# muhanzhang/IGMC

Measured on AMD Instinct MI355X. Metric: enclosing-subgraphs/sec (train step, batch=50) + test RMSE, higher is better.
Workload: dtype f32; 1 GPU; ml_1m, hop 1, max-nodes-per-hop 100, batch 50 per GPU, adj-dropout 0, dynamic-train, ARR 0.001, Adam; parallelism=dp1, global_batch=50, graphs_captured_before_timing=True, steps_per_graph_launch=100, group_steps=50

## Files before the change

igmc_amd/csrc/capi.hip:

```cpp
#include "launch.h"
#include "sortpool.h"
#include "g2_image.h"

#include <algorithm>
#include <climits>
#include <cmath>
#include <cstdio>
#include <cstring>
#include <map>
#include <string>
#include <vector>

static thread_local std::string g_err;
int g_igmc_prof_on = 0;

#define IGMC_FAIL(msg)                                                      \
  do {                                                                      \
    g_err = std::string(__func__) + ": " + (msg);                           \
    return 1;                                                               \
  } while (0)
#define HIPCHECK(expr)                                                      \
  do {                                                                      \
    hipError_t e_ = (expr);                                                 \
    if (e_ != hipSuccess) {                                                 \
// ... 706 lines not shown
      if (!told) fprintf(stderr, "[igmc] batches of more than 1024 subgraphs: no plane-exchange regions -- the dense-layer / per-layer kernels take the steps, not the subgraph kernel\n");
      told = true;
    }
  } else if (wide) {
    fail |= M.get(&d.g2_w, g2_w_words(d.R, d.L));
  }
  fail |= M.get(&d.gs_bar, 2 * Bc + 1);
  fail |= M.get(&d.gs_ts, 4);
  d.gs_err = d.gs_bar ? d.gs_bar + 2 * Bc : nullptr;
  fail |= M.get(&d.wg_part, (size_t)4 * IGMC_WG_BLOCKS * igmc_wg_stride()) |
          M.get(&d.gatt_part, (size_t)3 * IGMC_GATHER_BLOCKS * d.R * 4) |
          M.get(&d.l0_part, (size_t)IGMC_L0_BLOCKS * rows0 * 32) |
          M.get(&d.graw, (size_t)3 * igmc_wg_stride() + 3 * d.R * 4 + rows0 * 32) | M.get(&d.arr_part, 4);
  d.side = nullptr;
  d.ctrl = nullptr;
  d.dcat[0] = d.dcat[1] = d.dcat[2] = nullptr;
  fail |= M.get(&m->done_ctr, 8);
  if (fail) {
    M.release();
    delete m;
    IGMC_FAIL("hipMalloc failed (model workspace)");
  }
  {
    hipStream_t st1, st2;
    if (hipStreamCreateWithFlags(&st1, hipStreamNonBlocking) != hipSuccess ||
        hipStreamCreateWithFlags(&st2, hipStreamNonBlocking) != hipSuccess) {
      M.release();
      delete m;
      IGMC_FAIL("hipStreamCreate failed");
    }
    m->ax.s1 = st1;
    m->ax.s2 = st2;
    for (int i = 0; i < 8; ++i) {
      hipEvent_t e;
      if (hipEventCreateWithFlags(&e, hipEventDisableTiming) != hipSuccess) IGMC_FAIL("hipEventCreate failed");
      m->ax.ev[i] = e;
    }
  }
  HIPCHECK(hipMemset(m->done_ctr, 0, 8 * sizeof(int)));
  HIPCHECK(hipMemset(m->d.gs_bar, 0, (2 * (size_t)max_graphs + 1) * sizeof(int)));
  {
    const unsigned long long ts0[4] = {~0ull, 0ull, 0ull, 0ull};
    HIPCHECK(hipMemcpy(m->d.gs_ts, ts0, sizeof(ts0), hipMemcpyHostToDevice));
  }
  if (m->d.fold_w) HIPCHECK(hipMemset(m->d.fold_w, 0, (size_t)4 * 32 * IGMC_FOLD_NA * sizeof(unsigned long long)));
  if (m->d.g2_ex) {
    HIPCHECK(hipMemset(m->d.g2_ex, 0, 5 * m->d.g2_ex_stride * sizeof(unsigned long long)));
    HIPCHECK(hipMemset(m->d.g2_fx, 0, (size_t)max_graphs * 256 * sizeof(unsigned long long)));
    if (m->d.g2_px) HIPCHECK(hipMemset(m->d.g2_px, 0, 5 * m->d.g2_px_stride));
  }
  if (igmc_model_prepare(d)) {
    M.release();
    delete m;
    IGMC_FAIL("hipFuncSetAttribute failed");
  }
  *out = m;
  return 0;
}

extern "C" int igmc_debug_lin_mask(const igmc_model* m, uint8_t* h_out, int64_t n) {
  if (!m || !h_out) IGMC_FAIL("null argument");
  if (n < 0 || n > (int64_t)m->d.graph_cap * 128) IGMC_FAIL("mask size out of range");
  HIPCHECK(hipDeviceSynchronize());
  HIPCHECK(hipMemcpy(h_out, m->d.lmask, (size_t)n, hipMemcpyDeviceToHost));
  return 0;
}

extern "C" int igmc_debug_head_array(const igmc_model* m, int which, float* h_out, int64_t n) {
  if (!m || !h_out) IGMC_FAIL("null argument");
  if (which < 0 || which > 3) IGMC_FAIL("no such array");
  const float* src = which == 0 ? m->d.a1 : which == 1 ? m->d.dz : which == 2 ? m->d.feat : m->d.gfeat;
  if (n < 0 || n > (int64_t)m->d.graph_cap * (which < 2 ? 128 : m->d.D)) IGMC_FAIL("size out of range");
  HIPCHECK(hipDeviceSynchronize());
  HIPCHECK(hipMemcpy(h_out, src, (size_t)n * sizeof(float), hipMemcpyDeviceToHost));
  return 0;
}

extern "C" int igmc_debug_weight_images(const igmc_model* m, float* h_out, int64_t* n_words) {
  if (!m || !n_words) IGMC_FAIL("null argument");
  const int64_t n = m->d.g2_w ? (int64_t)g2_w_words(m->d.R, m->d.L) : 0;
  if (h_out) {
    if (*n_words < 0 || *n_words > n) IGMC_FAIL("size out of range");
    HIPCHECK(hipDeviceSynchronize());
    if (*n_words) HIPCHECK(hipMemcpy(h_out, m->d.g2_w, (size_t)*n_words * sizeof(float), hipMemcpyDeviceToHost));
  } else {
    *n_words = n;
  }
  return 0;
}

extern "C" void igmc_model_destroy(igmc_model* m) {
  if (!m) return;
  for (int i = 0; i < 8; ++i) hipEventDestroy((hipEvent_t)m->ax.ev[i]);
  hipStreamDestroy((hipStream_t)m->ax.s1);
  hipStreamDestroy((hipStream_t)m->ax.s2);
  m->mem.release();
  delete m;
}

extern "C" int64_t igmc_param_count(const igmc_model* m) { return m ? m->d.n_params : 0; }

extern "C" int64_t igmc_param_offset(const igmc_model* m, int layer, int which, int64_t* count) {
  if (!m) return -1;
  const ModelDev& d = m->d;
  const int fin = (layer == 0) ? d.L : 32;
  int64_t off = -1, n = 0;
  switch (which) {
    case IGMC_P_BASIS: off = d.off_basis[layer & 3]; n = (int64_t)4 * fin * 32; break;
    case IGMC_P_ROOT: off = d.off_root[layer & 3]; n = (int64_t)fin * 32; break;
    case IGMC_P_BIAS: off = d.off_bias[layer & 3]; n = 32; break;
    case IGMC_P_ATT: off = d.off_att[layer & 3]; n = (int64_t)d.R * 4; break;
    case IGMC_P_LIN1_W: off = d.off_l1w; n = (int64_t)128 * d.D; break;
    case IGMC_P_LIN1_B: off = d.off_l1b; n = 128; break;
    case IGMC_P_LIN2_W: off = d.off_l2w; n = 128; break;
    case IGMC_P_LIN2_B: off = d.off_l2b; n = 1; break;
  }
  if (count) *count = n;
  return off;
}

static StepPlan plan_query(const igmc_model* m, const igmc_batch* b, int B) {
  StepPlan sp;
  igmc_step_plan(m->d, b->d, B, IGMC_CALL_STEP, &sp);
  return sp;
}

extern "C" int igmc_model_dense_layers(const igmc_model* m, const igmc_batch* b, int B) {
  return (m && b) ? plan_query(m, b, B).dense_layers : 0;
}

extern "C" int igmc_model_dense_path(const igmc_model* m, const igmc_batch* b, int B) {
  return (m && b) ? plan_query(m, b, B).family == IGMC_FAM_G2 : 0;
}

extern "C" int igmc_model_step_form(const igmc_model* m, const igmc_batch* b, int B) {
  return (m && b) ? plan_query(m, b, B).step_form : 0;
}

extern "C" int igmc_model_step_geometry(const igmc_model* m, const igmc_batch* b, int B, int32_t* out, int n) {
  if (!m || !b || !out || n < 0) IGMC_FAIL("bad arguments");
  if (B < 1 || B > b->d.graph_cap) IGMC_FAIL("batch size outside the arena's capacity");
  const StepPlan sp = plan_query(m, b, B);
  const int g2 = sp.family == IGMC_FAM_G2, dense = sp.family == IGMC_FAM_DLF || sp.family == IGMC_FAM_DL;
  const int32_t v[IGMC_GEOM_N] = {sp.step_form,
                                  sp.family,
                                  g2 ? sp.cs : 0,
                                  g2 ? sp.grid : 0,
                                  sp.nqu,
                                  sp.nqv,
                                  sp.family == IGMC_FAM_ROWS ? 0 : sp.wide ? g2_groups(m->d.R, m->d.L) : 1,
                                  sp.wide && sp.gsplit,
                                  g2 || sp.dlts,
                                  g2 ? sp.lay.kp : 0,
                                  dense && sp.dlb};
  for (int i = 0; i < n && i < IGMC_GEOM_N; ++i) out[i] = v[i];
  return 0;
}

static int check_fit(igmc_model* m, const igmc_batch* b, std::string* why) {
  if (!m || !b) { *why = "null model or batch"; return 1; }
  if (b->last_B <= 0) { *why = "batch is empty (run igmc_extract_batch first)"; return 1; }
  if (b->d.node_cap > m->d.node_cap || b->d.graph_cap > m->d.graph_cap) { *why = "batch capacity exceeds the model workspace"; return 1; }
  if (b->d.num_labels != m->d.L) { *why = "num_labels mismatch (hop)"; return 1; }
  if (b->g->max_rel >= m->d.R) { *why = "graph has more relations than the model"; return 1; }
  if (m->d.S != b->n_side && m->d.S > 0) { *why = "side feature width mismatch"; return 1; }
  return 0;
}

static int check_call(igmc_model* m, const igmc_batch* b, bool buffers, std::string* why) {
  if (check_fit(m, b, why)) return 1;
  if (!buffers) { *why = "null buffer"; return 1; }
  return 0;
}
static StepPlan begin_call(igmc_model* m, const igmc_batch* b, int kind, void* stream) {
  m->d.side = b->side;
  StepPlan sp;
  igmc_step_plan(m->d, b->d, b->last_B, kind, &sp);
  if (b->lean && sp.needs_csr) ensure_csr(b, stream);
  return sp;
}
static void end_call(igmc_model* m, const igmc_batch* b, int training, int use_edge_flags) {
  m->last_B = b->last_B;
  m->last_training = training;
  m->last_flags = use_edge_flags;
}

struct AdamScalars {
  float step_size, inv_sqrt_bc2;
};
static AdamScalars adam_scalars(const int64_t* d_ctrl, int64_t t, float lr, float beta1, float beta2) {
  AdamScalars a = {0.f, 0.f};
  if (!d_ctrl) {
    const double bc1 = 1.0 - std::pow((double)beta1, (double)t);
    const double bc2 = 1.0 - std::pow((double)beta2, (double)t);
    a.step_size = (float)((double)lr / bc1);
    a.inv_sqrt_bc2 = (float)(1.0 / std::sqrt(bc2));
  }
  return a;
}

extern "C" int igmc_model_forward(igmc_model* m, const float* d_params, const igmc_batch* b, int training,
                                  int use_edge_flags, const uint8_t* d_lin_mask, uint64_t seed, uint64_t step,
                                  float multiply_by, float* d_out, void* stream) {
  std::string why;
  if (check_call(m, b, d_params && d_out, &why)) IGMC_FAIL(why);
  const StepPlan sp = begin_call(m, b, training ? IGMC_CALL_CONV : IGMC_CALL_EVAL, stream);
  ImgScope img(m, d_params);
  igmc_launch_forward(m->d, b->d, sp, d_params, b->last_B, training, use_edge_flags, d_lin_mask, seed, step, multiply_by,
                      d_out, stream);
  img.done_unchanged();
  HIPCHECK(hipGetLastError());
  end_call(m, b, training, use_edge_flags);
  return 0;
}

extern "C" int igmc_model_backward(igmc_model* m, const float* d_params, const igmc_batch* b, const float* d_gout,
                                   float multiply_by, float* d_grad, void* stream) {
  std::string why;
  if (check_fit(m, b, &why)) IGMC_FAIL(why);
  if (!m->last_training || m->last_B != b->last_B) IGMC_FAIL("backward needs a preceding training-mode forward on this batch");
  if (!d_params || !d_gout || !d_grad) IGMC_FAIL("null buffer");
  StepPlan sp;
  igmc_step_plan(m->d, b->d, b->last_B, IGMC_CALL_CONV, &sp);
  igmc_launch_backward(m->d, b->d, sp, d_params, b->last_B, m->last_flags, d_gout, 0, 0.f, multiply_by, 2.f, 0.f, d_grad,
                       stream);
  HIPCHECK(hipGetLastError());
  return 0;
}

extern "C" int igmc_model_loss_grad(igmc_model* m, const float* d_params, const igmc_batch* b, int use_edge_flags,
                                    const uint8_t* d_lin_mask, uint64_t seed, uint64_t step, float multiply_by,
                                    float ARR, float grad_scale, float arr_scale, float* d_out, float* d_grad,
                                    float* d_loss, void* stream) {
  std::string why;
  if (check_call(m, b, d_params && d_out && d_grad, &why)) IGMC_FAIL(why);
  const StepPlan sp = begin_call(m, b, IGMC_CALL_STEP, stream);
  ImgScope img(m, d_params);
  igmc_launch_loss_grad(m->d, b->d, sp, (float*)d_params, b->last_B, use_edge_flags, d_lin_mask, seed, step,
                        multiply_by, ARR, grad_scale, arr_scale, d_out, d_grad, d_loss, nullptr, stream);
  img.done_unchanged();
  HIPCHECK(hipGetLastError());
  end_call(m, b, 1, use_edge_flags);
  return 0;
}

extern "C" int igmc_adam_step(float* d_params, const float* d_grad, float* d_exp_avg, float* d_exp_avg_sq, int64_t n,
                              int64_t step, float lr, float beta1, float beta2, float eps, float weight_decay,
                              void* stream) {
  if (!d_params || !d_grad || !d_exp_avg || !d_exp_avg_sq || n <= 0 || step < 1) IGMC_FAIL("bad arguments");
  const AdamScalars as = adam_scalars(nullptr, step, lr, beta1, beta2);
  igmc_launch_adam(d_params, d_grad, d_exp_avg, d_exp_avg_sq, n, as.step_size, as.inv_sqrt_bc2, beta1, beta2, eps, weight_decay,
                   nullptr, 0, stream);
  HIPCHECK(hipGetLastError());
  return 0;
}

extern "C" int igmc_sse_accumulate(const float* d_out, const igmc_batch* b, double* d_acc, void* stream) {
  if (!d_out || !b || !d_acc) IGMC_FAIL("null argument");
  igmc_launch_sse(b->d, d_out, d_acc, nullptr, stream);
  HIPCHECK(hipGetLastError());
  return 0;
}
extern "C" int igmc_sse_accumulate_tick(const float* d_out, const igmc_batch* b, double* d_acc, int64_t* d_ctrl, void* stream) {
  if (!d_out || !b || !d_acc || !d_ctrl) IGMC_FAIL("null argument");
  igmc_launch_sse(b->d, d_out, d_acc, d_ctrl, stream);
  HIPCHECK(hipGetLastError());
  return 0;
}

extern "C" int igmc_scores_store(const float* d_out, const igmc_batch* b, double* d_acc, float* d_scores, float* d_labels,
                                 int64_t n, int64_t first_or_minus1, int64_t* d_ctrl, int32_t* d_err, void* stream) {
  if (!d_out || !b || !d_acc || !d_scores || !d_labels || !d_err) IGMC_FAIL("null argument");
  if (n < 1 || n > (int64_t)INT32_MAX) IGMC_FAIL("n must be in [1, 2^31)");
  if (first_or_minus1 < -1 || first_or_minus1 >= n) IGMC_FAIL("first must be -1 (the arena's stamp) or a position below n");
  igmc_launch_scores_store(b->d, d_out, d_acc, d_ctrl, d_scores, d_labels, n, first_or_minus1, d_err, stream);
  HIPCHECK(hipGetLastError());
  return 0;
}
static int select_grid(int64_t n, int num, int grid) {
  if (n < 1 || n > (int64_t)INT32_MAX || num < 1 || num > IGMC_SELECT_MAX_NUM || grid < 0 || grid > IGMC_SELECT_MAX_GRID) return -1;
  return grid > 0 ? grid : igmc_select_default_grid(n);
}
extern "C" int64_t igmc_select_scratch_bytes(int64_t n, int num, int grid) {
  const int g = select_grid(n, num, grid);
  if (g < 0) {
    g_err = std::string(__func__) + ": n must be in [1, 2^31), num in [1, 64], grid in [0, 1024]";
    return -1;
  }
  return (int64_t)2 * g * num * (int64_t)sizeof(uint64_t);
}
extern "C" int igmc_select_extremes(const float* d_keys, int64_t n, int num, int32_t* d_idx_low, int32_t* d_idx_high,
                                    float* d_key_low, float* d_key_high, int32_t* d_count, void* d_scratch,
                                    int64_t scratch_bytes, int grid, void* stream) {
  if (!d_keys || !d_idx_low || !d_idx_high || !d_scratch) IGMC_FAIL("null argument");
  const int g = select_grid(n, num, grid);
  if (g < 0) IGMC_FAIL("n must be in [1, 2^31), num in [1, 64], grid in [0, 1024]");
  if (scratch_bytes < (int64_t)2 * g * num * (int64_t)sizeof(uint64_t)) IGMC_FAIL("scratch too small (igmc_select_scratch_bytes)");
  if (((uintptr_t)d_scratch & 7) != 0) IGMC_FAIL("scratch must be 8-byte aligned");
  igmc_launch_select(d_keys, n, num, g, d_scratch, d_idx_low, d_idx_high, d_key_low, d_key_high, d_count, stream);
  HIPCHECK(hipGetLastError());
  return 0;
}

extern "C" int igmc_candidates_count(const igmc_graph* g, const int32_t* d_users, int nq, const uint8_t* d_item_ok,
                                     int exclude_seen, int64_t* d_counts, int32_t* d_err, void* stream) {
  if (!g || !d_users || !d_counts || !d_err) IGMC_FAIL("null argument");
  if (nq < 1) IGMC_FAIL("nq must be at least 1");
// ... 739 lines not shown
```

igmc_amd/csrc/g2_compose.h:

```cpp
#pragma once

__global__ __launch_bounds__(G2C_THREADS) void k_g2_compose(ModelDev m, const float* P, float* w) {
  __shared__ float s_att[4 * G2_NR * G2_NG_MAX];
  const int tid = threadIdx.x, R = m.R, L = m.L, RL = R * L, LF = L * 32;
  const int ng = g2_groups(R, L);
  const int tableb = 2 * 3 * ng * (G2_NR + 1);
  const int mi = (int)(blockIdx.x >> 1);
  const int l = ((int)blockIdx.x >= tableb) ? 0 : 1 + mi / (ng * (G2_NR + 1)), trans = blockIdx.x & 1;
  if ((int)blockIdx.x >= tableb) {
    const int c0 = 32 * ((int)blockIdx.x - tableb);
    const float attv = (tid < R * 4) ? P[m.off_att[0] + tid] : 0.f;
    float bv[4][4], rv[4];
#pragma unroll
    for (int q = 0; q < 4; ++q) {
      const int i = tid + q * G2C_THREADS, c = c0 + (i >> 5), f = i & 31;
      const int cf = (c < RL) ? (c % L) * 32 + f : 0;
#pragma unroll
      for (int bb = 0; bb < 4; ++bb) bv[q][bb] = (c < RL) ? P[m.off_basis[0] + bb * LF + cf] : 0.f;
      rv[q] = (c >= RL && c < RL + L) ? P[m.off_root[0] + (c - RL) * 32 + f] : ((c == RL + L) ? P[m.off_bias[0] + f] : 0.f);
    }
    if (tid < 4 * G2_NR * G2_NG_MAX) s_att[tid] = attv;
    __syncthreads();
#pragma unroll
    for (int q = 0; q < 4; ++q) {
// ... 1 lines not shown
      float sacc = rv[q];
      if (c < RL) {
        const int r = c / L;
        sacc = g2_wsum(s_att[r * 4], s_att[r * 4 + 1], s_att[r * 4 + 2], s_att[r * 4 + 3], bv[q][0], bv[q][1], bv[q][2], bv[q][3]);
      }
      w[g2_t0_off(ng) + (size_t)c0 * 32 + i] = sacc;
    }
    return;
  }
  const int grp = (mi / (G2_NR + 1)) % ng, blk = mi % (G2_NR + 1);
  uint16_t* img = (uint16_t*)(w + g2_img_off(ng, l, trans, grp));
  const int r = (blk == G2_NR) ? ((grp == 0) ? -1 : R) : G2_NR * grp + blk;
  const int n = tid & 31, kg = tid >> 5;
  float v[4] = {0.f, 0.f, 0.f, 0.f};
  if (r < 0) {
    const float* root = P + m.off_root[l];
    if (trans) {
      const float4 r4 = *(const float4*)(root + n * 32 + 4 * kg);
      v[0] = r4.x; v[1] = r4.y; v[2] = r4.z; v[3] = r4.w;
    } else {
#pragma unroll
      for (int q = 0; q < 4; ++q) v[q] = root[(4 * kg + q) * 32 + n];
    }
  } else if (r < R) {
    const float* basis = P + m.off_basis[l];
    float bq[4][4];
#pragma unroll
    for (int bb = 0; bb < 4; ++bb) {
      if (trans) {
        const float4 b4 = *(const float4*)(basis + bb * 1024 + n * 32 + 4 * kg);
        bq[bb][0] = b4.x; bq[bb][1] = b4.y; bq[bb][2] = b4.z; bq[bb][3] = b4.w;
      } else {
#pragma unroll
        for (int q = 0; q < 4; ++q) bq[bb][q] = basis[bb * 1024 + (4 * kg + q) * 32 + n];
      }
    }
    float at[4];
#pragma unroll
    for (int bb = 0; bb < 4; ++bb) at[bb] = P[m.off_att[l] + r * 4 + bb];
#pragma unroll
    for (int q = 0; q < 4; ++q) v[q] = g2_wsum(at[0], at[1], at[2], at[3], bq[0][q], bq[1][q], bq[2][q], bq[3][q]);
  }
  uint32_t h01, m01, l01, h23, m23, l23;
  g2_split2(v[0], v[1], h01, m01, l01);
  g2_split2(v[2], v[3], h23, m23, l23);
  const int lane = (kg & 3) * 16 + (n & 15), nt = n >> 4, e0 = 4 * (kg >> 2);
  const uint32_t t3[3][2] = {{h01, h23}, {m01, m23}, {l01, l23}};
#pragma unroll
  for (int t = 0; t < G2_NT; ++t)
    *(uint2*)(img + ((size_t)(((t * (G2_NR + 1) + blk) * 2 + nt) * 64 + lane)) * 8 + e0) = make_uint2(t3[t][0], t3[t][1]);
}

static int igmc_g2_layout(const ModelDev& m, const BatchDev& b, int cs, G2Layout* lay) {
  const int RL = m.R * m.L;
  if (m.S != 0 || m.D != 256 || m.R > G2_NR || m.L > 8 || RL + m.L + 1 > 32 || !m.ts_part || !m.g2_px || !m.g2_fx || !m.g2_w || !b.relm) return 0;
  const int half = 2 * cs;
  const int cmax = b.cap_u > b.cap_v ? b.cap_u : b.cap_v;
  if (cmax > 16 * half || cmax > 128) return 0;
  if (b.graph_cap > m.g2_graphs) return 0;
  const int kmax = ((cmax + 31) >> 5) << 5;
  lay->kp = kmax + 8;
  lay->nsides = (cs == 1) ? 2 : 1;
  lay->rmr = ((cmax + 15) >> 4) << 4;
  lay->rmc = kmax;
  int o = 0;
  lay->pside = ((G2_NT * 32 * lay->kp * 2 + 1023) & ~1023) >> 2;
  lay->planes = o; o += lay->nsides * lay->pside;
  lay->ohp = o; o += lay->nsides * (8 * lay->kp >> 1);
  lay->lab = o; o += 64;
  lay->xo = o; o += 2 * G2_NB * 16 * G2_XP;
  lay->hs = o; o += G2_NB * 16 * G2_XP;
  int tw = G2_NB * 16 * G2_TP;
  if (tw < (G2_THREADS / 64) * 256) tw = (G2_THREADS / 64) * 256;
  const int rw = 2 * lay->rmr * (lay->rmc + 8) / 4;
  if (rw > tw) tw = rw;
  if (tw < 1024) tw = 1024;
  lay->tile = o; o += tw;
  lay->hist = o; o += G2_NB * 16 * G2_XP;
  lay->px = o; o += G2_NB * 2 * 64 * 4;
  lay->wreg = o; o += G2_WIMG;
  lay->t0 = o; o += 1024;
  lay->att = o; o += 64;
  lay->head = o; o += 256 + 256 + 3 * 128 + 512 + 16;
  lay->words = o;
  return (size_t)o * 4 + 768 <= 160 * 1024;
}

__global__ void k_g2_xcc_probe(int* out) {
  if (threadIdx.x == 0) out[blockIdx.x] = (int)(g2_xcc_id() & 15ull);
}
int igmc_g2_xcd_ok() {
#ifdef IGMC_HIPEMU
  return 1;
#else
  static int oks[64];
  static bool init = false;
  if (!init) {
    for (int i = 0; i < 64; ++i) oks[i] = -1;
    init = true;
  }
  int dev = 0;
  if (hipGetDevice(&dev) != hipSuccess || dev < 0 || dev >= 64) dev = 0;
  int& ok = oks[dev];
  if (ok >= 0) return ok;
  ok = 0;
  int* d = nullptr;
  int h[64];
  if (hipMalloc((void**)&d, sizeof(h)) != hipSuccess) return ok;
  hipLaunchKernelGGL(k_g2_xcc_probe, dim3(64), dim3(64), 0, 0, d);
  if (hipMemcpy(h, d, sizeof(h), hipMemcpyDeviceToHost) == hipSuccess) {
    ok = 1;
    for (int b = 0; b + 8 < 64; ++b)
      if (h[b] != h[b + 8]) ok = 0;
  }
  (void)hipFree(d);
  if (!ok) fprintf(stderr, "[igmc] device %d: workgroups b and b + 8 of a launch do not share an XCD: the subgraph kernel and the one-launch dense layers are not used\n", dev);
  return ok;
#endif
}

int g_igmc_compose_count = 0;

int igmc_launch_graph_step2(const ModelDev& m, const BatchDev& b, const StepPlan& sp, const float* P, int B, int training,
                            int use_flags, const uint8_t* inj_mask, uint64_t seed, uint64_t step, float mult, float grad_scale,
                            float* out, void* stream, int nstash, const int64_t* stash_ctrl) {
  const G2Layout& lay = sp.lay;
  const int cs = sp.cs;
  G2Args a;
  memset(&a, 0, sizeof(a));
  a.n_users = b.n_users; a.n_items = b.n_items; a.B = B; a.s_lab = b.s_lab; a.relm = b.relm; a.y = b.y;
  a.cap_u = b.cap_u; a.cap_v = b.cap_v; a.slot = b.slot; a.relm_ld = b.relm_ld; a.graph_cap = b.graph_cap;
  a.R = m.R; a.L = m.L; a.D = m.D; a.ts_stride = m.ts_stride;
  for (int l = 0; l < 4; ++l) {
    a.h[l] = m.h[l];
    a.off_bias[l] = (int)m.off_bias[l];
  }
  a.ts_part = m.ts_part; a.g2_px = m.g2_px; a.g2_fx = m.g2_fx; a.g2_px_stride = m.g2_px_stride; a.g2_w = m.g2_w;
  a.gs_bar = m.gs_bar; a.gs_err = m.gs_err; a.a1 = m.a1; a.dz = m.dz; a.feat = m.feat; a.gfeat = m.gfeat; a.err = m.err;
  a.lmask = m.lmask; a.ctrl = m.ctrl;
  a.off_l1w = (int)m.off_l1w; a.off_l1b = (int)m.off_l1b; a.off_l2w = (int)m.off_l2w; a.off_l2b = (int)m.off_l2b;
  a.P = P;
  a.inj_mask = inj_mask;
  a.seed = seed;
  a.step = step;
  a.mult = mult;
  a.grad_scale = grad_scale;
  a.out = out;
  a.lay2 = lay;
  a.timing = getenv("IGMC_GS_TIMING") ? 1 : 0;
  a.ts = (g_igmc_prof_on == 2) ? m.gs_ts : nullptr;
  a.self_seq = (!training || a.ts) ? 1 : 0;
  a.cs = cs;
  a.stride = (cs > 1) ? ((B + 7) & ~7) : 1;
  if (training && nstash) {
    a.nstash = nstash;
    a.stash_ctrl = stash_ctrl;
    a.fs.R = m.R; a.fs.L = m.L;
    for (int l = 0; l < 4; ++l) {
      a.fs.off_basis[l] = m.off_basis[l];
      a.fs.off_att[l] = m.off_att[l];
    }
    a.fs.fin_stash = m.fin_stash; a.fs.adam_m1 = m.adam_m1; a.fs.adam_m2 = m.adam_m2; a.fs.arr_part = m.arr_part;
  }
  const int grid = sp.grid + a.nstash;
  const size_t sm = (size_t)lay.words * 4;
  if (!m.img_current) {
    IGMC_PLAUNCH("k_g2_compose", k_g2_compose, 2 * 3 * g2_groups(m.R, m.L) * (G2_NR + 1) + g2_t0_rows(m.R, m.L) / 32, G2C_THREADS, 0, stream, m, P, m.g2_w);
    ++g_igmc_compose_count;
  }
#ifdef IGMC_HIPEMU
  if (cs > 1) {
    hipemu::rt().co_cs = cs;
    hipemu::rt().co_stride = 8;
    hipemu::rt().co_block = 8 * cs;
  }
#endif
  if (getenv("IGMC_GS_TRACE")) fprintf(stderr, "[igmc] k_graph_step B=%d train=%d flags=%d v2 kp=%d lds=%zu cluster=%d grid=%d\n", B, training, use_flags, lay.kp, sm, cs, grid);
  igmc_dispatch([&](auto uf, auto tr, auto cl) {
    IGMC_PLAUNCH(tr() ? "k_graph_step" : "k_graph_fwd", (k_graph_step2<uf(), tr(), cl()>), grid, G2_THREADS, sm, stream, a);
  }, use_flags != 0, training != 0, cs > 1);
  return a.self_seq ? 0 : 1;
}

int igmc_dl_prepare();
int igmc_gs_prepare() { return igmc_g2_prepare(); }
int igmc_g2_prepare() {
  if (igmc_dl_prepare()) return 1;
  (void)igmc_g2_xcd_ok();
#ifndef IGMC_HIPEMU
  const int mx = 160 * 1024;
  const void* fns[8] = {(const void*)k_graph_step2<true, true, true>,   (const void*)k_graph_step2<false, true, true>,
                        (const void*)k_graph_step2<true, false, true>,  (const void*)k_graph_step2<false, false, true>,
                        (const void*)k_graph_step2<true, true, false>,  (const void*)k_graph_step2<false, true, false>,
                        (const void*)k_graph_step2<true, false, false>, (const void*)k_graph_step2<false, false, false>};
  for (const void* fn : fns) {
    hipFuncAttributes fa;
    if (hipFuncGetAttributes(&fa, fn) != hipSuccess || (int)fa.sharedSizeBytes > 768) return 1;
    if (hipFuncSetAttribute(fn, hipFuncAttributeMaxDynamicSharedMemorySize, mx - (int)fa.sharedSizeBytes) != hipSuccess) return 1;
  }
#endif
  return 0;
}
```

igmc_amd/csrc/g2_prims.h:

```cpp
#pragma once

#ifdef IGMC_HIPEMU
#define G2_STAMP(k) do { } while (0)
#else
#define G2_STAMP(k)                                                                                        \
  do {                                                                                                     \
    if (a.timing && threadIdx.x == 0) {                                                                    \
      if (blockIdx.x == 0) g_g2_clk[k] = __builtin_readcyclecounter();                                     \
      else if (a.cs > 2 && (int)blockIdx.x == 8 * (a.cs / 2) && (k) < 40) g_g2_clk[64 + (k)] = __builtin_readcyclecounter(); \
    }                                                                                                      \
  } while (0)
#endif

#ifdef IGMC_HIPEMU
#define DL_STAMP(k) do { } while (0)
#else
#define DL_STAMP(k)                                                                               \
  do {                                                                                            \
    if (a.timing && threadIdx.x == 0 && (int)blockIdx.x == a.timing - 1 && (k) < 128)             \
      g_g2_clk[k] = __builtin_readcyclecounter();                                                 \
  } while (0)
#endif

#ifdef IGMC_HIPEMU
#define G2_OPAQUE(x) do { } while (0)
#else
#define G2_OPAQUE(x) asm volatile("" : "+v"(x))
#endif

typedef uint32_t u32x4 __attribute__((ext_vector_type(4)));
#ifndef IGMC_HIPEMU
typedef __bf16 g2_bf16x8 __attribute__((ext_vector_type(8)));
#endif

__device__ __forceinline__ f32x4 g2_mfma_bf16(u32x4 a, u32x4 b, f32x4 c) {
#ifdef IGMC_HIPEMU
  return igmc_emu_mfma_16x16x32_bf16(a, b, c);
#else
  return __builtin_amdgcn_mfma_f32_16x16x32_bf16(__builtin_bit_cast(g2_bf16x8, a), __builtin_bit_cast(g2_bf16x8, b), c, 0, 0, 0);
#endif
}

template <bool FLAGS>
__device__ __forceinline__ void g2_expand4(uint32_t w, uint32_t r1, int keepbit, uint32_t& o01, uint32_t& o23) {
  uint32_t mk = w & (0x01010101u * IGMC_RELM_CODE);
  if (FLAGS) mk &= ((w >> keepbit) & 0x01010101u) * IGMC_RELM_CODE;
  const uint32_t t = mk ^ (0x01010101u * r1);
  const uint32_t eq = ~(t + 0x7F7F7F7Fu) & 0x80808080u;
  const uint32_t mask = (eq >> 7) * 0xFFu;
#ifdef IGMC_HIPEMU
  o01 = ((mask & 0xFFu) ? 0x3F80u : 0u) | ((mask & 0xFF00u) ? 0x3F800000u : 0u);
  o23 = ((mask & 0xFF0000u) ? 0x3F80u : 0u) | ((mask & 0xFF000000u) ? 0x3F800000u : 0u);
#else
  o01 = __builtin_amdgcn_perm(mask, mask, 0x01010000u) & 0x3F803F80u;
  o23 = __builtin_amdgcn_perm(mask, mask, 0x03030202u) & 0x3F803F80u;
#endif
}

template <bool FLAGS>
__device__ __forceinline__ uint32_t g2_bytemask(uint32_t w, uint32_t r1, int keepbit) {
  uint32_t mk = w & (0x01010101u * IGMC_RELM_CODE);
  if (FLAGS) mk &= ((w >> keepbit) & 0x01010101u) * IGMC_RELM_CODE;
  const uint32_t t = mk ^ (0x01010101u * r1);
  const uint32_t eq = ~(t + 0x7F7F7F7Fu) & 0x80808080u;
  return (eq >> 7) * 0xFFu;
}
__device__ __forceinline__ u32x4 g2_mask_frag(uint32_t m0, uint32_t m1) {
  u32x4 f;
#ifdef IGMC_HIPEMU
  f[0] = ((m0 & 0xFFu) ? 0x3F80u : 0u) | ((m0 & 0xFF00u) ? 0x3F800000u : 0u);
  f[1] = ((m0 & 0xFF0000u) ? 0x3F80u : 0u) | ((m0 & 0xFF000000u) ? 0x3F800000u : 0u);
  f[2] = ((m1 & 0xFFu) ? 0x3F80u : 0u) | ((m1 & 0xFF00u) ? 0x3F800000u : 0u);
  f[3] = ((m1 & 0xFF0000u) ? 0x3F80u : 0u) | ((m1 & 0xFF000000u) ? 0x3F800000u : 0u);
#else
  f[0] = __builtin_amdgcn_perm(m0, m0, 0x01010000u) & 0x3F803F80u;
  f[1] = __builtin_amdgcn_perm(m0, m0, 0x03030202u) & 0x3F803F80u;
  f[2] = __builtin_amdgcn_perm(m1, m1, 0x01010000u) & 0x3F803F80u;
  f[3] = __builtin_amdgcn_perm(m1, m1, 0x03030202u) & 0x3F803F80u;
#endif
  return f;
}

__device__ __forceinline__ float g2_tanh(float x) {
#ifdef IGMC_HIPEMU
  return tanhf(x);
#else
  return 1.f - 2.f * __builtin_amdgcn_rcpf(1.f + __expf(2.f * x));
#endif
}

template <int AUX = 0>
__device__ __forceinline__ void g2_glds16(const float4* src_wave, float4* lds_wave, int lane) {
#ifndef IGMC_HIPEMU
  __builtin_amdgcn_global_load_lds((const __attribute__((address_space(1))) void*)(src_wave + lane),
                                   (__attribute__((address_space(3))) void*)lds_wave, 16, 0, AUX);
#else
  lds_wave[lane] = src_wave[lane];
#endif
}

#include "g2_words.h"

#define G2_PX_BYTES 32768
#define G2_PX_FLAGS 28672
#define DLX_PX_BYTES 65536
#define DLX_PX_FLAGS 61440
__device__ __forceinline__ void g2_publish_planes(unsigned char* px, int kp, int f, int node0, const float (&v)[4]) {
  uint32_t h0, m0, l0, h1, m1, l1;
  g2_split2(v[0], v[1], h0, m0, l0);
  g2_split2(v[2], v[3], h1, m1, l1);
  unsigned char* p = px + ((size_t)f * kp + node0) * 2;
  const size_t ts = (size_t)32 * kp * 2;
  *(uint2*)p = make_uint2(h0, h1);
  *(uint2*)(p + ts) = make_uint2(m0, m1);
  *(uint2*)(p + 2 * ts) = make_uint2(l0, l1);
}
__device__ __forceinline__ void g2_flag_raise(unsigned char* px, int slot, uint32_t tag, int lane, int flags_off = G2_PX_FLAGS) {
#ifndef IGMC_HIPEMU
  asm volatile("s_waitcnt vmcnt(0)" ::: "memory");
  if (lane == 0) __hip_atomic_store((unsigned long long*)(px + flags_off) + slot, (unsigned long long)tag, __ATOMIC_RELAXED, __HIP_MEMORY_SCOPE_WAVEFRONT);
#else
  if (lane == 0) ((unsigned long long*)(px + flags_off))[slot] = (unsigned long long)tag;
#endif
}
__device__ __forceinline__ void g2_flags_wait(const unsigned char* px, int n, uint32_t tag, int lane, int* err, int flags_off = G2_PX_FLAGS) {
  const unsigned long long* fl = (const unsigned long long*)(px + flags_off);
  for (long it = 0;; ++it) {
#ifndef IGMC_HIPEMU
    const unsigned long long w = (lane < n) ? __hip_atomic_load(fl + lane, __ATOMIC_RELAXED, __HIP_MEMORY_SCOPE_AGENT) : (unsigned long long)tag;
#else
    const unsigned long long w = (lane < n) ? fl[lane] : (unsigned long long)tag;
#endif
    if (__ballot(w != (unsigned long long)tag) == 0ull) break;
    if (it > (1L << 20)) {
      *err = 1;
      break;
    }
#ifndef IGMC_HIPEMU
    __builtin_amdgcn_s_sleep(1);
#else
    hipemu::yield();
#endif
  }
}
__device__ __forceinline__ void g2_planes_load_exact(uint32_t* pl, const unsigned char* px, int bytes, int wave, int lane, int nwaves) {
  const int pieces = (bytes + 1023) >> 10;
  for (int c = wave; c < pieces; c += nwaves)
    if (c * 1024 + lane * 16 < bytes) g2_glds16<16>((const float4*)px + c * 64, (float4*)pl + c * 64, lane);
}
__device__ __forceinline__ void g2_planes_load(uint32_t* pl, const unsigned char* px, int kp, int wave, int lane, int nwaves) {
  const int pieces = (192 * kp + 1023) >> 10;
  for (int c = wave; c < pieces; c += nwaves) g2_glds16<16>((const float4*)px + c * 64, (float4*)pl + c * 64, lane);
}

#ifdef IGMC_HIPEMU
#define G2_SCHED_BARRIER() do { } while (0)
#else
#define G2_SCHED_BARRIER() __builtin_amdgcn_sched_barrier(0)
#endif

__device__ __forceinline__ uint32_t g2_ld_seq(const int* gs_bar) {
#ifndef IGMC_HIPEMU
  return (uint32_t)__hip_atomic_load(gs_bar + 1, __ATOMIC_RELAXED, __HIP_MEMORY_SCOPE_AGENT);
#else
  return (uint32_t)gs_bar[1];
#endif
}
__device__ __forceinline__ bool g2_last_workgroup_advances(int* gs_bar) {
#ifndef IGMC_HIPEMU
  if (__hip_atomic_fetch_add(gs_bar, 1, __ATOMIC_RELAXED, __HIP_MEMORY_SCOPE_AGENT) != (int)gridDim.x - 1) return false;
  __hip_atomic_store(gs_bar, 0, __ATOMIC_RELAXED, __HIP_MEMORY_SCOPE_AGENT);
  __hip_atomic_fetch_add(gs_bar + 1, 1, __ATOMIC_RELAXED, __HIP_MEMORY_SCOPE_AGENT);
  return true;
#else
  if (gs_bar[0]++ != (int)gridDim.x - 1) return false;
  gs_bar[0] = 0;
  gs_bar[1] += 1;
  return true;
#endif
}
__device__ __forceinline__ void g2_wait_vm0() {
#ifndef IGMC_HIPEMU
  asm volatile("s_waitcnt vmcnt(0)" ::: "memory");
#endif
}
__device__ __forceinline__ unsigned long long g2_wall_clock() {
#ifndef IGMC_HIPEMU
  return (unsigned long long)wall_clock64();
#else
  return 0ull;
#endif
}
__device__ __forceinline__ unsigned long long g2_xcc_id() {
#ifndef IGMC_HIPEMU
  return (unsigned long long)__builtin_amdgcn_s_getreg((20 << 0) | (0 << 6) | (3 << 11));
#else
  return 0ull;
#endif
}
__device__ __forceinline__ void g2_clock_open(unsigned long long* ts) {
#ifndef IGMC_HIPEMU
  atomicMin(ts, (unsigned long long)wall_clock64());
#else
  (void)ts;
#endif
}
__device__ __forceinline__ void g2_clock_close(unsigned long long* ts, unsigned long long t1) {
#ifndef IGMC_HIPEMU
  const unsigned long long t0 = __hip_atomic_load(ts, __ATOMIC_RELAXED, __HIP_MEMORY_SCOPE_AGENT);
  atomicAdd(ts + 1, t1 - t0);
  atomicAdd(ts + 2, 1ull);
  __hip_atomic_store(ts, ~0ull, __ATOMIC_RELAXED, __HIP_MEMORY_SCOPE_AGENT);
#else
  (void)ts; (void)t1;
#endif
}

#ifdef IGMC_HIPEMU
#define DL_FMAC(acc_, a_, b_) ((acc_) += (a_) * (b_))
#else
#define DL_FMAC(acc_, a_, b_) asm("v_fmac_f32 %0, %1, %2" : "+v"(acc_) : "v"(a_), "v"(b_))
#endif

#define DLX_K 256
__device__ __forceinline__ void dlx_seq_done(int* gs_bar, int self_seq) {
  if (threadIdx.x != 0 || !self_seq) return;
  (void)g2_last_workgroup_advances(gs_bar);
}
```

igmc_amd/csrc/g2_subgraph.h:

```cpp
#pragma once

struct G2Args {
  const int32_t* n_users;
  const int32_t* n_items;
  int B;
  const uint8_t* s_lab;
  const uint8_t* relm;
  const float* y;
  int cap_u, cap_v, slot, relm_ld, graph_cap;
  int R, L, D, ts_stride;
  float* h[4];
  float* ts_part;
  unsigned char* g2_px;
  unsigned long long* g2_fx;
  size_t g2_px_stride;
  const float* g2_w;
  int* gs_bar;
  int* gs_err;
  float* a1;
  float* dz;
  float* feat;
  float* gfeat;
  float* err;
  uint8_t* lmask;
  const int64_t* ctrl;
  int off_bias[4];
  int off_l1w, off_l1b, off_l2w, off_l2b;
  const float* P;
  const uint8_t* inj_mask;
  uint64_t seed, step;
  float mult, grad_scale;
  float* out;
  unsigned long long* ts;
  int timing, cs, stride, self_seq;
  G2Layout lay2;
  int nstash;
  const int64_t* stash_ctrl;
  FinStashModel fs;
};

template <bool FLAGS, bool TRAIN, bool ONCE>
__global__ __launch_bounds__(G2_THREADS) void k_graph_step2(G2Args a) {
  __builtin_amdgcn_s_setprio(3);
  const float* P = a.P;
  IGMC_DYN_SMEM(smem);
  float* S = (float*)smem;
  const G2Layout lay = a.lay2;
  const int kp = lay.kp, nsides = lay.nsides;
  uint32_t* PLN = (uint32_t*)(S + lay.planes);
  uint32_t* OHP = (uint32_t*)(S + lay.ohp);
  unsigned char* slab = (unsigned char*)(S + lay.lab);
  float* XOA = S + lay.xo;
  float* HSS = S + lay.hs;
  float* TILES = S + lay.tile;
  float* HIST = S + lay.hist;
  float* PXA = S + lay.px;
  float2* sW2 = (float2*)(S + lay.wreg);
  float* sT0 = S + lay.t0;
  float* sfeat = S + lay.head;
  float* sgf = sfeat + 256;
  float* sa1 = sgf + 256;
  float* skeep = sa1 + 128;
  float* sdz = skeep + 128;
  float* sred = sdz + 128;
  float* misc = sred + 512;
  const int R = a.R, L = a.L, RL = R * L;
  const int tid = threadIdx.x, lane = tid & 63, wave = tid >> 6;
  const int li = lane & 15, kq = lane >> 4;
  const int B = a.B;
  const int ts = a.ts_stride;
  const int cs = a.cs;
  const int cm = (cs > 1) ? (int)((blockIdx.x >> 3) % cs) : 0;
  const int half = 2 * cs;
  const uint32_t seq = g2_ld_seq(a.gs_bar);
  const uint32_t tag0 = seq * 8u + 1u;
  const uint64_t step = a.ctrl ? (uint64_t)a.ctrl[IGMC_CTRL_STEP] : a.step;
  if (a.ts && tid == 0) g2_clock_open(a.ts);
  auto xtag = [&](int x) { return tag0 + (uint32_t)x; };
  G2_STAMP(0);
  if (a.timing && tid == 0 && blockIdx.x < 1024) {
    g_g2_wg[blockIdx.x][0] = g2_wall_clock();
    g_g2_wg[blockIdx.x][2] = g2_xcc_id();
  }
  auto arrive = [&]() {
    if (tid == 0 && a.self_seq) {
      const unsigned long long t1 = a.ts ? g2_wall_clock() : 0ull;
      if (g2_last_workgroup_advances(a.gs_bar) && a.ts) g2_clock_close(a.ts, t1);
    }
  };
  const int nwork = (int)gridDim.x - (TRAIN ? a.nstash : 0);
  if (TRAIN && (int)blockIdx.x >= nwork) {
    if (tid < IGMC_BLOCK) {
      const int l = (int)blockIdx.x - nwork;
      fin_stash_body(a.fs, P, l, a.stash_ctrl);
      if (l == 0 && tid == 0) a.fs.fin_stash[IGMC_STASH_SCAL + IGMC_STASH_SEQ] = __uint_as_float(seq);
    }
    arrive();
    return;
  }

  const int g_first = (cs > 1) ? (int)(blockIdx.x / (8 * cs)) * 8 + (int)(blockIdx.x & 7) : (int)blockIdx.x;
  const int g_pre = (g_first < a.graph_cap) ? g_first : a.graph_cap - 1;
  const int pre_cu = a.n_users[g_pre], pre_cv = a.n_items[g_pre];
  const int ld = a.relm_ld;
  auto load_label = [&](int g2) {
    const int hi = (tid >> 7) & 1, t7 = tid & 127;
    const int capx = a.cap_u + hi * (a.cap_v - a.cap_u);
    return (int)a.s_lab[(size_t)g2 * a.slot + hi * a.cap_u + ((t7 < capx) ? t7 : 0)];
  };
  int labv_raw = 0;
  if (tid < 256) g2_glds16((const float4*)(a.g2_w + 6 * G2_WIMG) + (tid & ~63), (float4*)sT0 + (tid & ~63), tid & 63);
  const int tslot = (cs > 1) ? g_first + cm * a.stride : (int)blockIdx.x;
  f32x4 acc0 = (f32x4){0.f, 0.f, 0.f, 0.f};
  bool first_graph = true;
  G2_STAMP(1);

  int g = g_first;
  if (g < B) do {
    int tid_g = threadIdx.x;
    G2_OPAQUE(tid_g);
    const int tid = tid_g, lane = tid & 63, wave = tid >> 6;
    const int li = lane & 15, kq = lane >> 4;
    const int bw = wave >> 1, hf = wave & 1;
    const int gw = cm * G2_NB + bw;
    const int side = gw / half, bi = gw - side * half;
    labv_raw = load_label(g);
    uint32_t bw0[G2_KS], bw1[G2_KS];
    {
      const unsigned char* rmg = a.relm + (size_t)g * a.cap_u * ld;
      const uint32_t rrow = (uint32_t)(16 * bi + li);
#pragma unroll
      for (int s = 0; s < G2_KS; ++s) {
        const uint32_t c0 = (uint32_t)(32 * s + 8 * kq);
        if (side == 0) {
          const uint32_t* p4 = (const uint32_t*)(rmg + (rrow * (uint32_t)ld + c0));
          bw0[s] = p4[0];
          bw1[s] = p4[1];
        } else {
          const unsigned char* pc = rmg + (c0 * (uint32_t)ld + rrow);
          bw0[s] = (uint32_t)pc[0] | ((uint32_t)pc[ld] << 8) | ((uint32_t)pc[2 * ld] << 16) | ((uint32_t)pc[3 * ld] << 24);
          bw1[s] = (uint32_t)pc[4 * ld] | ((uint32_t)pc[5 * ld] << 8) | ((uint32_t)pc[6 * ld] << 16) | ((uint32_t)pc[7 * ld] << 24);
        }
      }
    }
    G2_STAMP(48);
    {
      const float4 z4 = make_float4(0.f, 0.f, 0.f, 0.f);
      for (int i = tid; i < 2 * G2_NB * 16 * G2_XP / 4; i += G2_THREADS) ((float4*)XOA)[i] = z4;
      for (int i = tid; i < G2_NB * 16 * G2_XP / 4; i += G2_THREADS) ((float4*)HIST)[i] = z4;
    }
    G2_STAMP(49);
    const int cu = first_graph ? pre_cu : a.n_users[g], cv = first_graph ? pre_cv : a.n_items[g];
    const int n_own = side ? cv : cu, n_opp = side ? cu : cv;
    const int nbs = g * a.slot + (side ? a.cap_u : 0);
    const int nbun = (n_own + 15) >> 4;
    const bool active = bi < nbun;
    const int row0 = 16 * bi;
    const int nks = (n_opp + 31) >> 5;
    const int sx = (nsides == 2) ? side : 0, so = (nsides == 2) ? 1 - side : 0;
    uint32_t* pl = PLN + so * lay.pside;
    uint32_t* ohp = OHP + so * (8 * kp >> 1);
    float* XO0 = XOA + bw * 16 * G2_XP;
    float* XO1 = XOA + (G2_NB + bw) * 16 * G2_XP;
    float* HS = HSS + bw * 16 * G2_XP;
    float* T = TILES + bw * 16 * G2_TP;
    float* HI = HIST + bw * 16 * G2_XP;
    f32x4* PXo = (f32x4*)PXA + (bw * 2 + hf) * 64 + lane;
    const f32x4* PXi = (const f32x4*)PXA + (bw * 2 + (1 - hf)) * 64 + lane;
    const size_t exs = a.g2_px_stride;
    auto px_of = [&](int x, int sd) { return a.g2_px + (size_t)x * exs + ((size_t)g * 2 + sd) * G2_PX_BYTES; };
    unsigned long long* fx = a.g2_fx + (size_t)g * 256;
    const int nbun_opp = (n_opp + 15) >> 4;

    if (tid < 256) slab[tid] = (unsigned char)(((tid & 127) < ((tid >> 7) ? cv : cu)) ? labv_raw : 255);
    G2_STAMP(50);
    __syncthreads();
    G2_STAMP(2);
    {
      for (int i = tid; i < nsides * 8 * (kp >> 1); i += G2_THREADS) {
        const int s2 = i / (8 * (kp >> 1)), rem = i - s2 * (8 * (kp >> 1));
        const int lb = rem / (kp >> 1), q = rem - lb * (kp >> 1);
        const int sd = (nsides == 2) ? s2 : 1 - side;
        const int l0 = (2 * q < 128) ? slab[sd * 128 + 2 * q] : 255, l1 = (2 * q + 1 < 128) ? slab[sd * 128 + 2 * q + 1] : 255;
        OHP[i] = ((l0 == lb) ? 0x3F80u : 0u) | ((l1 == lb) ? 0x3F800000u : 0u);
      }
    }
    __syncthreads();
    G2_STAMP(3);
    uint32_t AM[G2_NR][G2_KS][2];
    uint32_t RB[FLAGS ? G2_KS : 1][2];
    const int kb = side ? IGMC_RELM_KF : IGMC_RELM_KT;
    {
      const int kf = side ? IGMC_RELM_KT : IGMC_RELM_KF;
#pragma unroll
      for (int s = 0; s < G2_KS; ++s) {
        uint32_t w0 = 0u, w1 = 0u;
        if (active && s < nks && row0 + li < n_own) {
          w0 = bw0[s];
          w1 = bw1[s];
          {
            const int keep = n_opp - (32 * s + 8 * kq);
            if (keep < 8) {
              w1 = (keep <= 4) ? 0u : (w1 & (0xFFFFFFFFu >> (8 * (8 - keep))));
              if (keep < 4) w0 = (keep <= 0) ? 0u : (w0 & (0xFFFFFFFFu >> (8 * (4 - keep))));
            }
          }
        }
        if constexpr (FLAGS) {
          RB[s][0] = w0;
          RB[s][1] = w1;
        }
#pragma unroll
        for (int r = 0; r < G2_NR; ++r) {
          AM[r][s][0] = g2_bytemask<FLAGS>(w0, (uint32_t)(r + 1), kf);
          AM[r][s][1] = g2_bytemask<FLAGS>(w1, (uint32_t)(r + 1), kf);
        }
      }
    }
    auto frag_f = [&](int r, int s) {
      uint32_t m0 = AM[r][s][0], m1 = AM[r][s][1];
      G2_OPAQUE(m0);
      G2_OPAQUE(m1);
      return g2_mask_frag(m0, m1);
    };
    auto frag_b = [&](int r, int s) {
      uint32_t m0 = FLAGS ? RB[FLAGS ? s : 0][0] : AM[r][s][0], m1 = FLAGS ? RB[FLAGS ? s : 0][1] : AM[r][s][1];
      G2_OPAQUE(m0);
      G2_OPAQUE(m1);
      if constexpr (FLAGS) return g2_mask_frag(g2_bytemask<true>(m0, (uint32_t)(r + 1), kb), g2_bytemask<true>(m1, (uint32_t)(r + 1), kb));
      else return g2_mask_frag(m0, m1);
    };
    G2_STAMP(4);

    static_assert(G2_WIMG % 256 == 0, "an image is a whole number of 1 KB pieces");
    auto wload = [&](int l, int trans) {
      const float4* src = (const float4*)(a.g2_w + (size_t)((l - 1) * 2 + trans) * G2_WIMG);
#pragma unroll
      for (int j = 0; j < (G2_WIMG / 256 + G2_THREADS / 64 - 1) / (G2_THREADS / 64); ++j) {
        const int c = wave + j * (G2_THREADS / 64);
        if (c < G2_WIMG / 256) g2_glds16(src + c * 64, (float4*)sW2 + c * 64, lane);
      }
    };
    wload(1, 0);
    auto fwd_out = [&](int l, const f32x4& o, float bias, float* XO) {
      const int nt = hf;
      float* hrow = a.h[l] + (size_t)(nbs + row0 + 4 * kq) * 32 + li;
      float* xo = XO + 4 * kq * G2_XP + li;
      float v[4];
#pragma unroll
      for (int rr = 0; rr < 4; ++rr) {
        const float tv = g2_tanh(o[rr] + bias);
        v[rr] = (row0 + 4 * kq + rr < n_own) ? tv : 0.f;
      }
      if (l < 3) {
        g2_publish_planes(px_of(l, side), kp, 16 * nt + li, row0 + 4 * kq, v);
        g2_flag_raise(px_of(l, side), 2 * bi + hf, xtag(l), lane);
      }
#pragma unroll
      for (int rr = 0; rr < 4; ++rr) {
        xo[rr * G2_XP + 16 * nt] = v[rr];
        if (TRAIN && row0 + 4 * kq + rr < n_own) hrow[rr * 32 + 16 * nt] = v[rr];
      }
      if (bi == 0 && kq == 0) g2_pub_f32(fx + side * 128 + l * 32 + 16 * nt + li, v[0], tag0 + G2_FXTAG);
    };
    auto raise = [&](int x) { g2_flag_raise(px_of(x, side), 2 * bi + hf, xtag(x), lane); };
    auto fetch = [&](int x) {
      if (nsides == 1) {
        g2_flags_wait(px_of(x, 1 - side), 2 * nbun_opp, xtag(x), lane, a.gs_err);
        g2_planes_load(PLN, px_of(x, 1 - side), kp, wave, lane, G2_THREADS / 64);
      } else {
        for (int s2 = 0; s2 < 2; ++s2) {
          g2_flags_wait(px_of(x, s2), 2 * (((s2 ? cv : cu) + 15) >> 4), xtag(x), lane, a.gs_err);
          g2_planes_load(PLN + s2 * lay.pside, px_of(x, s2), kp, wave, lane, G2_THREADS / 64);
        }
      }
    };

    if (active) {
      f32x4 hacc[G2_NR];
#pragma unroll
      for (int r = 0; r < G2_NR; ++r) hacc[r] = (f32x4){0.f, 0.f, 0.f, 0.f};
      u32x4 pfh[G2_KS];
#pragma unroll
      for (int s = 0; s < G2_KS; ++s) {
        pfh[s] = *(const u32x4*)(ohp + ((li & 7) * kp >> 1) + 16 * s + 4 * kq);
        if (li >= 8 || s >= nks) pfh[s] = (u32x4){0u, 0u, 0u, 0u};
      }
      G2_SCHED_BARRIER();
#pragma unroll
      for (int s = 0; s < G2_KS; ++s) {
#pragma unroll
        for (int r = 0; r < G2_NR; ++r) {
          hacc[r] = g2_mfma_bf16(pfh[s], frag_f(r, s), hacc[r]);
        }
      }
      G2_STAMP(51);
#pragma unroll
      for (int r = 0; r < G2_NR; ++r)
#pragma unroll
        for (int rr = 0; rr < 4; ++rr)
          if (r < R && 4 * kq + rr < L) HI[li * G2_XP + r * L + 4 * kq + rr] = hacc[r][rr];
      if (kq == 0 && row0 + li < n_own) {
        HI[li * G2_XP + RL + slab[side * 128 + row0 + li]] = 1.f;
        HI[li * G2_XP + RL + L] = 1.f;
      }
      IGMC_WAVE_SYNC();
      f32x4 o = (f32x4){0.f, 0.f, 0.f, 0.f};
#pragma unroll
      for (int j = 0; j < 8; ++j) {
        const float av = HI[li * G2_XP + 4 * j + kq];
        o = __builtin_amdgcn_mfma_f32_16x16x4f32(av, sT0[(4 * j + kq) * 32 + 16 * hf + li], o, 0, 0, 0);
      }
      G2_STAMP(52);
      fwd_out(0, o, 0.f, XO0);
    }
    G2_STAMP(5);

#pragma unroll
    for (int l = 1; l < 4; ++l) {
      float* XOc = (l & 1) ? XO0 : XO1;
      float* XOn = (l & 1) ? XO1 : XO0;
      G2_STAMP(6 + 3 * (l - 1));
      const float bias0 = P[a.off_bias[l] + 16 * hf + li];
      fetch(l - 1);
      if (l > 1) wload(l, 0);
// ... 133 lines not shown
      wload(3, 1);
      __syncthreads();
      if (tid < 256) {
        const float v = ((TILES[tid] + TILES[256 + tid]) + (TILES[512 + tid] + TILES[768 + tid])) +
                        ((TILES[1024 + tid] + TILES[1280 + tid]) + (TILES[1536 + tid] + TILES[1792 + tid]));
        sgf[tid] = v;
        if (cm == 0) a.gfeat[(size_t)g * a.D + tid] = v;
      }
      __syncthreads();
      G2_STAMP(17);
      if (tid < 32 * nsides) {
        const int s2 = tid >> 5, f = tid & 31;
        const int sd = (nsides == 2) ? s2 : 1 - side;
        const float hv = sfeat[sd * 128 + 96 + f];
        const float d = sgf[sd * 128 + 96 + f] * (1.f - hv * hv);
        uint32_t h, mi, lo;
        g2_split2(d, 0.f, h, mi, lo);
        uint32_t* p2 = PLN + s2 * lay.pside + (f * kp >> 1);
        p2[0] = h & 0xFFFFu;
        p2[32 * kp >> 1] = mi & 0xFFFFu;
        p2[2 * (32 * kp >> 1)] = lo & 0xFFFFu;
      }
      if (hf == 0 && lane < 32) {
        const float hv = sfeat[side * 128 + 96 + lane];
        const float d = (active && bi == 0) ? sgf[side * 128 + 96 + lane] * (1.f - hv * hv) : 0.f;
        if (active && bi == 0) XO0[lane] = d;
        sred[(1 * G2_NB + bw) * 32 + lane] = d;
      }
      __syncthreads();
      G2_STAMP(18);

#pragma unroll
      for (int l = 3; l >= 1; --l) {
        float* XOc = (l & 1) ? XO0 : XO1;
        float* XOn = (l & 1) ? XO1 : XO0;
        float* wpart = a.ts_part + ((size_t)l * IGMC_TS_BLOCKS + tslot) * ts;
        G2_STAMP(19 + 5 * (3 - l));
        float hreg[4];
#pragma unroll
        for (int rr = 0; rr < 4; ++rr) hreg[rr] = 0.f;
        f32x4 o[2];
        if (active) {
          {
            const float* hrow = a.h[l - 1] + (size_t)(nbs + row0 + 4 * kq) * 32 + 16 * hf + li;
#pragma unroll
            for (int rr = 0; rr < 4; ++rr)
              if (row0 + 4 * kq + rr < n_own) hreg[rr] = hrow[rr * 32];
          }
          int lane_ = lane;
          G2_OPAQUE(lane_);
          const int li_ = lane_ & 15, kq_ = lane_ >> 4;
          f32x4 acc[G2_NR];
          if (l == 2) G2_STAMP(43);
          g2_gather_h(pl, kp, (l == 3) ? 1 : nks, frag_b, li_, kq_, hf, acc);
          if (l == 2) G2_STAMP(44);
#pragma unroll
          for (int r = 0; r < G2_NR; ++r)
            *(float4*)(T + li * G2_TP + r * 32 + 16 * hf + 4 * kq) = make_float4(acc[r][0], acc[r][1], acc[r][2], acc[r][3]);
#pragma unroll
          for (int rr = 0; rr < 4; ++rr) HS[(4 * kq + rr) * G2_XP + 16 * hf + li] = hreg[rr];
          if (l == 2) G2_STAMP(45);
          g2_transform_h(acc, XOc, (const uint32_t*)sW2, li_, kq_, hf, o);
          if (l == 2) G2_STAMP(46);
          *PXo = hf ? o[0] : o[1];
#pragma unroll
          for (int rr = 0; rr < 4; ++rr) G2_OPAQUE(hreg[rr]);
        } else if (hf == 0) {
          for (int i = lane; i < 16 * G2_TP; i += 64) T[i] = 0.f;
          for (int i = lane; i < 16 * G2_XP; i += 64) HS[i] = 0.f;
        }
        __syncthreads();
        if (l == 2) G2_STAMP(47);
        if (active) {
          const f32x4 po = *PXi;
          const int f = 16 * hf + li;
          float v[4];
#pragma unroll
          for (int rr = 0; rr < 4; ++rr) {
            const int row = 4 * kq + rr;
            float d = hf ? po[rr] + o[1][rr] : o[0][rr] + po[rr];
            if (bi == 0 && row == 0) d += sgf[side * 128 + (l - 1) * 32 + f];
            const float x = hreg[rr];
            v[rr] = (row0 + row < n_own) ? d * (1.f - x * x) : 0.f;
          }
          if (l > 1) {
            g2_publish_planes(px_of(6 - l, side), kp, f, row0 + 4 * kq, v);
            raise(6 - l);
          }
#pragma unroll
          for (int rr = 0; rr < 4; ++rr) XOn[(4 * kq + rr) * G2_XP + f] = v[rr];
          if (l > 1) {
            float cb = (v[0] + v[1]) + (v[2] + v[3]);
            cb += __shfl_xor(cb, 16);
            cb += __shfl_xor(cb, 32);
            if (kq == 0) sred[(((l - 1) & 1) * G2_NB + bw) * 32 + f] = cb;
          }
        } else if (l > 1 && lane < 16) {
          sred[(((l - 1) & 1) * G2_NB + bw) * 32 + 16 * hf + lane] = 0.f;
        }
        if (tid < 32) {
          const float* sb = sred + (l & 1) * G2_NB * 32 + tid;
          const float sv = (sb[0] + sb[32]) + (sb[64] + sb[96]);
          if (first_graph) wpart[(R * 32 + 32) * 32 + tid] = sv;
          else wpart[(R * 32 + 32) * 32 + tid] += sv;
        }
        G2_STAMP(20 + 5 * (3 - l));
        G2_STAMP(21 + 5 * (3 - l));
        if (l > 1) wload(l - 1, 1);
        {
          f32x4 w3[3];
#pragma unroll
          for (int i3 = 0; i3 < 3; ++i3) w3[i3] = (f32x4){0.f, 0.f, 0.f, 0.f};
          const int m2w = wave >> 2, wo = wave & 3;
#pragma unroll 1
          for (int wb = 0; wb < G2_NB; ++wb) {
            const float* Tb = TILES + wb * 16 * G2_TP;
            const float* Hb = HSS + wb * 16 * G2_XP;
            const float* Db = XOA + (((l & 1) ? 0 : G2_NB) + wb) * 16 * G2_XP;
            float av[4], bw3[4][3];
#pragma unroll
            for (int s4 = 0; s4 < 4; ++s4) {
              av[s4] = Hb[(4 * s4 + kq) * G2_XP + m2w * 16 + li];
              const float* tb = Tb + (4 * s4 + kq) * G2_TP + li;
              const float* db = Db + (4 * s4 + kq) * G2_XP + li;
#pragma unroll
              for (int i3 = 0; i3 < 3; ++i3) {
                const int nt = 3 * wo + i3;
                bw3[s4][i3] = (nt < 2 * G2_NR) ? tb[nt * 16] : db[(nt - 2 * G2_NR) * 16];
              }
            }
            G2_SCHED_BARRIER();
#pragma unroll
            for (int s4 = 0; s4 < 4; ++s4)
#pragma unroll
              for (int i3 = 0; i3 < 3; ++i3)
                w3[i3] = __builtin_amdgcn_mfma_f32_16x16x4f32(av[s4], bw3[s4][i3], w3[i3], 0, 0, 0);
          }
#pragma unroll
          for (int i3 = 0; i3 < 3; ++i3) {
            const int m2 = m2w, nt = 3 * wo + i3;
            const int r = nt >> 1;
            if (r >= R && r < G2_NR) continue;
            float* pp = wpart + (kq * 4) * 32 + li + (r < R ? r : R) * 1024 + m2 * 512 + (nt & 1) * 16;
            if (first_graph) {
#pragma unroll
              for (int rr = 0; rr < 4; ++rr) pp[rr * 32] = w3[i3][rr];
            } else {
#pragma unroll
              for (int rr = 0; rr < 4; ++rr) pp[rr * 32] += w3[i3][rr];
            }
          }
        }
        G2_STAMP(22 + 5 * (3 - l));
        if (l > 1) fetch(6 - l);
        __syncthreads();
        G2_STAMP(23 + 5 * (3 - l));
      }

      if (wave < 4) {
        const int m2 = wave >> 1, wn = wave & 1;
        for (int wb = 0; wb < G2_NB; ++wb) {
          const float* Hb = HIST + wb * 16 * G2_XP;
          const float* Db = XOA + (G2_NB + wb) * 16 * G2_XP;
#pragma unroll
          for (int s4 = 0; s4 < 4; ++s4)
            acc0 = __builtin_amdgcn_mfma_f32_16x16x4f32(Hb[(4 * s4 + kq) * G2_XP + m2 * 16 + li],
                                                        Db[(4 * s4 + kq) * G2_XP + wn * 16 + li], acc0, 0, 0, 0);
        }
      }
      first_graph = false;
      __syncthreads();
      G2_STAMP(34);
    }
  } while (!ONCE && (g += nwork) < B);

  if (TRAIN && wave < 4) {
    float* part0 = a.ts_part + (size_t)tslot * ts;
    const int m2 = wave >> 1, wn = wave & 1;
#pragma unroll
    for (int rr = 0; rr < 4; ++rr) {
      const int c = m2 * 16 + kq * 4 + rr;
      if (c < RL + L + 1) part0[c * 32 + wn * 16 + li] = acc0[rr];
    }
  }
  arrive();
  G2_STAMP(35);
  if (a.timing && tid == 0 && blockIdx.x < 1024) g_g2_wg[blockIdx.x][1] = g2_wall_clock();
}

extern "C" int igmc_debug_g2_wg_clocks(unsigned long long* out, int n_wg) {
#ifndef IGMC_HIPEMU
  if (n_wg > 1024) n_wg = 1024;
  if (hipDeviceSynchronize() != hipSuccess) return 1;
  if (hipMemcpyFromSymbol(out, HIP_SYMBOL(g_g2_wg), (size_t)n_wg * 3 * sizeof(unsigned long long)) != hipSuccess) return 1;
#else
  for (int i = 0; i < 3 * n_wg; ++i) out[i] = 0;
#endif
  return 0;
}

extern "C" int igmc_debug_g2_clocks(unsigned long long* out, int n) {
#ifndef IGMC_HIPEMU
  if (n > 128) n = 128;
  if (hipDeviceSynchronize() != hipSuccess) return 1;
  if (hipMemcpyFromSymbol(out, HIP_SYMBOL(g_g2_clk), (size_t)n * sizeof(unsigned long long)) != hipSuccess) return 1;
#else
  for (int i = 0; i < n; ++i) out[i] = 0;
#endif
  return 0;
}
```

igmc_amd/csrc/graphstep2.hip:

```cpp
#include "launch.h"
#include "g2_image.h"
#include "head_sub.h"
#include "fin_stash.h"
#include <stdlib.h>
#include <stdio.h>
#include <string.h>

#define G2_THREADS 512
#define G2_NB 4
#define G2C_THREADS 256
#define G2_KS 4
#define G2_TP (G2_NR * 32 + 4)
#define G2_XP 36
#define G2_FXTAG 7

__device__ unsigned long long g_g2_clk[128];
__device__ unsigned long long g_g2_wg[1024][3];
#include "g2_prims.h"

template <typename Frag>
__device__ __forceinline__ void g2_gather_h(const uint32_t* pl, int kp, int nks, Frag frag, int li, int kq, int hf, f32x4 (&acc)[G2_NR]) {
#pragma unroll
  for (int r = 0; r < G2_NR; ++r) acc[r] = (f32x4){0.f, 0.f, 0.f, 0.f};
  const int tstride = 32 * kp >> 1;
  const uint32_t* base = pl + ((16 * hf + li) * kp >> 1) + 4 * kq;
  u32x4 pf[2][G2_NT];
  auto request = [&](int s, int buf) {
#pragma unroll
    for (int sp = 0; sp < G2_NT; ++sp) pf[buf][sp] = *(const u32x4*)(base + sp * tstride + 16 * s);
  };
  request(0, 0);
#pragma unroll
  for (int s = 0; s < G2_KS; ++s) {
    if (s < nks) {
      if (s + 1 < G2_KS) request(s + 1, (s + 1) & 1);
      G2_SCHED_BARRIER();
#pragma unroll
      for (int r = 0; r < G2_NR; ++r) {
        const u32x4 fr = frag(r, s);
#pragma unroll
        for (int q = 0; q < G2_NT; ++q) acc[r] = g2_mfma_bf16(pf[s & 1][q], fr, acc[r]);
      }
      G2_SCHED_BARRIER();
    }
  }
}

__device__ __forceinline__ void g2_transform_h(const f32x4 (&acc)[G2_NR], const float* xrows, const uint32_t* sW, int li, int kq, int hf,
                                               f32x4 (&o)[2]) {
  f32x4 o0a = (f32x4){0.f, 0.f, 0.f, 0.f}, o0b = o0a, o1a = o0a, o1b = o0a;
  const float4 xv = *(const float4*)(xrows + li * G2_XP + 16 * hf + 4 * kq);
  const uint2* wf = (const uint2*)sW + 2 * (kq * 16 + li) + hf;
  uint2 bf[2][2 * G2_NT][2];
  auto request = [&](int st, int buf) {
#pragma unroll
    for (int t = 0; t < G2_NT; ++t)
#pragma unroll
      for (int nt = 0; nt < 2; ++nt)
#pragma unroll
        for (int b2 = 0; b2 < 2; ++b2) bf[buf][2 * t + nt][b2] = wf[((t * (G2_NR + 1) + 2 * st + b2) * 2 + nt) * 128];
  };
  request(0, 0);
#pragma unroll
  for (int st = 0; st < (G2_NR + 1) / 2; ++st) {
    if (st + 1 < (G2_NR + 1) / 2) request(st + 1, (st + 1) & 1);
    float v[8];
#pragma unroll
    for (int rr = 0; rr < 4; ++rr) {
      v[rr] = acc[2 * st][rr];
      v[4 + rr] = (2 * st + 1 < G2_NR) ? acc[(2 * st + 1 < G2_NR) ? 2 * st + 1 : 0][rr] : (rr == 0 ? xv.x : rr == 1 ? xv.y : rr == 2 ? xv.z : xv.w);
    }
    u32x4 ah, am, al;
#pragma unroll
    for (int q = 0; q < 4; ++q) {
      uint32_t h, mi, lo;
      g2_split2(v[2 * q], v[2 * q + 1], h, mi, lo);
      ah[q] = h;
      am[q] = mi;
      al[q] = lo;
    }
    G2_SCHED_BARRIER();
    u32x4 b[2 * G2_NT];
#pragma unroll
    for (int q = 0; q < 2 * G2_NT; ++q) b[q] = (u32x4){bf[st & 1][q][0].x, bf[st & 1][q][0].y, bf[st & 1][q][1].x, bf[st & 1][q][1].y};
    o0a = g2_mfma_bf16(ah, b[0], o0a);
    o1a = g2_mfma_bf16(ah, b[1], o1a);
    o0b = g2_mfma_bf16(ah, b[2], o0b);
    o1b = g2_mfma_bf16(ah, b[3], o1b);
    o0a = g2_mfma_bf16(am, b[0], o0a);
    o1a = g2_mfma_bf16(am, b[1], o1a);
    o0b = g2_mfma_bf16(ah, b[4], o0b);
    o1b = g2_mfma_bf16(ah, b[5], o1b);
    o0a = g2_mfma_bf16(al, b[0], o0a);
    o1a = g2_mfma_bf16(al, b[1], o1a);
    o0b = g2_mfma_bf16(am, b[2], o0b);
    o1b = g2_mfma_bf16(am, b[3], o1b);
    G2_SCHED_BARRIER();
  }
#pragma unroll
  for (int rr = 0; rr < 4; ++rr) {
    o[0][rr] = o0a[rr] + o0b[rr];
    o[1][rr] = o1a[rr] + o1b[rr];
  }
}

__device__ __forceinline__ void g2_transform(const f32x4 (&acc)[G2_NR][2], const float* xrows, const uint32_t* sW, int li, int kq,
                                             f32x4 (&o)[2]) {
  f32x4 o0a = (f32x4){0.f, 0.f, 0.f, 0.f}, o0b = o0a, o1a = o0a, o1b = o0a;
  const float4 x0 = *(const float4*)(xrows + li * G2_XP + 4 * kq), x1 = *(const float4*)(xrows + li * G2_XP + 16 + 4 * kq);
  const u32x4* wf = (const u32x4*)sW + (kq * 16 + li);
  u32x4 bf[2][2 * G2_NT];
  auto request = [&](int g, int buf) {
#pragma unroll
    for (int t = 0; t < G2_NT; ++t) {
      bf[buf][2 * t] = wf[((t * (G2_NR + 1) + g) * 2 + 0) * 64];
      bf[buf][2 * t + 1] = wf[((t * (G2_NR + 1) + g) * 2 + 1) * 64];
    }
  };
  request(0, 0);
#pragma unroll
  for (int g = 0; g <= G2_NR; ++g) {
    if (g < G2_NR) request(g + 1, (g + 1) & 1);
    float v[8];
    if (g < G2_NR) {
#pragma unroll
      for (int rr = 0; rr < 4; ++rr) {
        v[rr] = acc[g][0][rr];
        v[4 + rr] = acc[g][1][rr];
      }
    } else {
      v[0] = x0.x; v[1] = x0.y; v[2] = x0.z; v[3] = x0.w;
      v[4] = x1.x; v[5] = x1.y; v[6] = x1.z; v[7] = x1.w;
    }
    u32x4 ah, am, al;
#pragma unroll
    for (int q = 0; q < 4; ++q) {
      uint32_t h, mi, lo;
      g2_split2(v[2 * q], v[2 * q + 1], h, mi, lo);
      ah[q] = h;
      am[q] = mi;
      al[q] = lo;
    }
    G2_SCHED_BARRIER();
    const u32x4 (&b)[2 * G2_NT] = bf[g & 1];
    o0a = g2_mfma_bf16(ah, b[0], o0a);
    o1a = g2_mfma_bf16(ah, b[1], o1a);
    o0b = g2_mfma_bf16(ah, b[2], o0b);
    o1b = g2_mfma_bf16(ah, b[3], o1b);
    o0a = g2_mfma_bf16(am, b[0], o0a);
    o1a = g2_mfma_bf16(am, b[1], o1a);
    o0b = g2_mfma_bf16(ah, b[4], o0b);
    o1b = g2_mfma_bf16(ah, b[5], o1b);
    o0a = g2_mfma_bf16(al, b[0], o0a);
    o1a = g2_mfma_bf16(al, b[1], o1a);
    o0b = g2_mfma_bf16(am, b[2], o0b);
    o1b = g2_mfma_bf16(am, b[3], o1b);
    G2_SCHED_BARRIER();
  }
#pragma unroll
  for (int rr = 0; rr < 4; ++rr) {
    o[0][rr] = o0a[rr] + o0b[rr];
    o[1][rr] = o1a[rr] + o1b[rr];
  }
}

#include "g2_subgraph.h"
#include "g2_compose.h"
// ... 3 lines not shown
```

igmc_amd/csrc/launch.h:

```cpp
#pragma once
#include "model.h"
#include <string.h>
#include <type_traits>

size_t igmc_extract_smem_bytes(const GraphDev& g);
void igmc_launch_extract(const GraphDev& g, const BatchDev& b, const int32_t* link_u, const int32_t* link_v,
                         const float* link_y, const int32_t* link_idx, int first, int B, int replay,
                         double sample_ratio, uint64_t seed, uint64_t epoch, const int64_t* ctrl, int lean, void* stream);
void igmc_launch_extract_set(const GraphDev& g, const BatchDev* d_set, const BatchDev& b0, int count, const int32_t* link_u,
                             const int32_t* link_v, const float* link_y, const int32_t* link_idx, int sel0, int B,
                             double sample_ratio, uint64_t seed, const int64_t* ctrl, float drop_p, int force_undirected,
                             uint64_t drop_seed, void* stream);
void igmc_launch_emit(const BatchDev& b, int B, void* stream);
void igmc_launch_emit_nodes(const BatchDev& b, int B, void* stream);
void igmc_launch_load_nodes(const BatchDev& b, const int64_t* uoff, const int32_t* unodes, const uint8_t* udist,
                            const int64_t* voff, const int32_t* vnodes, const uint8_t* vdist, const float* link_y,
                            const int32_t* link_idx, int first, int B, const int64_t* ctrl, void* stream);
void igmc_launch_edge_flags(const BatchDev& b, float p, int force_undirected, uint64_t seed, uint64_t step,
                            const int64_t* ctrl, void* stream);
void igmc_launch_relm_flags(const BatchDev& b, void* stream);
void igmc_launch_relm_dropout(const BatchDev& b, int B, float p, int force_undirected, uint64_t seed, uint64_t step,
                              const int64_t* ctrl, void* stream);
void igmc_launch_tick(int64_t* ctrl, void* stream);
void igmc_launch_regroup(int64_t* ctrl, int M, int64_t first_cur, int64_t first_next, void* stream);
void igmc_launch_gate(int64_t* ctrl, int q, int gk_min, long long delay_ticks, int delay_always, long long timeout_ticks,
                      void* stream);
void igmc_launch_fill_u8(uint8_t* p, int64_t n, uint8_t v, void* stream);
int igmc_extract_prepare(size_t smem);

struct ModelAux {
  void* s1;
  void* s2;
  void* ev[8];
};
struct StepPlan;
void igmc_launch_forward(const ModelDev& m, const BatchDev& b, const StepPlan& sp, const float* P, int B, int training,
                         int use_flags, const uint8_t* inj_mask, uint64_t seed, uint64_t step, float mult,
                         float* out, void* stream);
void igmc_launch_conv_forward(const ModelDev& m, const BatchDev& b, const StepPlan& sp, const float* P, int B, int training,
                              int use_flags, void* stream);
void igmc_launch_conv_backward(const ModelDev& m, const BatchDev& b, const StepPlan& sp, const float* P, int B, int use_flags,
                               float arr_coef, float* grad, void* stream);
void igmc_launch_backward(const ModelDev& m, const BatchDev& b, const StepPlan& sp, const float* P, int B, int use_flags,
                          const float* gout, int from_err, float grad_scale, float mult, float drop_scale,
                          float arr_coef, float* grad, void* stream);
struct AdamTail;
struct StepExchange {
  int (*sum)(void* user, float* a, int64_t na, float* b, int64_t nb, void* stream);
  void* user;
  const int* failed;
};
int igmc_launch_loss_grad(const ModelDev& m, const BatchDev& b, const StepPlan& sp, float* P, int B, int use_flags,
                          const uint8_t* inj_mask, uint64_t seed, uint64_t step, float mult, float ARR,
                          float grad_scale, float arr_scale, float* out, float* grad, float* loss, const AdamTail* adam,
                          void* stream, const StepExchange* xch = nullptr, int* img_emitted = nullptr);
int igmc_launch_train_step(const ModelDev& m, const BatchDev& b, const StepPlan& sp, float* P, int B, int use_flags,
                           const uint8_t* inj_mask, uint64_t seed, uint64_t step, float mult, float ARR, float* out,
                           float* grad, float* m1, float* m2, float step_size, float inv_sqrt_bc2, float beta1,
                           float beta2, float eps, float wd, int64_t* ctrl, int* done, float* loss, double* total,
                           void* stream, float grad_scale = 0.f, const StepExchange* xch = nullptr, int* img_emitted = nullptr);
void igmc_launch_loss(const ModelDev& m, const BatchDev& b, float ARR, float* loss, void* stream);
void igmc_launch_sse(const BatchDev& b, const float* out, double* acc, int64_t* ctrl, void* stream);
#define IGMC_SELECT_MAX_GRID 1024
#define IGMC_SELECT_MAX_NUM 64
void igmc_launch_scores_store(const BatchDev& b, const float* out, double* acc, int64_t* ctrl, float* scores, float* labels,
                              int64_t n, int64_t first, int32_t* err, void* stream);
int igmc_select_default_grid(int64_t n);
void igmc_launch_select(const float* keys, int64_t n, int num, int grid, void* scratch, int32_t* idx_low, int32_t* idx_high,
                        float* key_low, float* key_high, int32_t* count, void* stream);
#define IGMC_CAND_TILE_ITEMS 16384
#define IGMC_SEGSEL_MAX_SPLIT 64
void igmc_launch_candidates_count(const GraphDev& g, const int32_t* users, int nq, const uint8_t* item_ok, int exclude_seen,
                                  int64_t* counts, int32_t* err, void* stream);
void igmc_launch_candidates_fill(const GraphDev& g, const int32_t* users, int nq, const uint8_t* item_ok, int exclude_seen,
                                 const int64_t* off, int32_t* link_u, int32_t* link_v, int64_t capacity, int32_t* err,
                                 void* stream);
int igmc_segsel_default_split(int ns);
void igmc_launch_select_segments(const float* keys, const int64_t* seg_off, int ns, int num, int k, void* scratch,
                                 int32_t* idx_out, float* key_out, int32_t* count, void* stream);
#define IGMC_RANK_MAX_KS 8
void igmc_launch_rank_segments(const float* keys, const int32_t* ids, int64_t n, const int64_t* seg_off, int ns,
                               const int64_t* q_off, const int32_t* q_id, int64_t nq, int k, int32_t* q_pos, int32_t* q_rank,
                               int32_t* err, void* stream);
void igmc_launch_rank_metrics(const int32_t* q_rank, const int64_t* q_off, const uint8_t* q_rel, const int32_t* ks, int nk,
                              int ns, int64_t nq, int grid, int32_t* cnt, double* dcg, int32_t* err, void* stream);
int igmc_model_prepare(const ModelDev& m);
void igmc_launch_adam(float* p, const float* g, float* m1, float* m2, int64_t n, float step_size,
                      float inv_sqrt_bc2, float beta1, float beta2, float eps, float wd, int64_t* ctrl, int tick,
                      void* stream);
void igmc_launch_finish(const ModelDev& m, const BatchDev& b, float* p, const float* g, float* m1, float* m2,
                        float step_size, float inv_sqrt_bc2, float beta1, float beta2, float eps, float wd,
                        int64_t* ctrl, float ARR, float* loss, double* total, int use_flags, void* stream);

int igmc_g2_xcd_ok();
struct G2Layout {
  int kp, nsides, rmr, rmc, pside;
  int planes, ohp, lab, xo, hs, tile, hist, px, wreg, t0, att, head, words;
};
void igmc_launch_side_gather(const float* src, int S, const int32_t* link_idx, int first, int B, const int64_t* ctrl,
                             float* dst, void* stream);
int igmc_gs_prepare();
int igmc_g2_prepare();

#define IGMC_CALL_EVAL 0
#define IGMC_CALL_CONV 1
#define IGMC_CALL_STEP 2
#define IGMC_FAM_ROWS 0
#define IGMC_FAM_G2 1
#define IGMC_FAM_DLF 2
#define IGMC_FAM_DL 3
#define IGMC_TAIL_HANDOFF 0
#define IGMC_TAIL_TS 1
#define IGMC_TAIL_BS 2
struct StepPlan {
  int kind;
  int fast_head;
  int family;
  int cs, grid;
  G2Layout lay;
  int wide, dl, dlts, dlf, dlb;
  int nqu, nqv, dl_grid;
  int gsplit;
  int self_seq;
  int head_inside;
  int bwd_dense;
  int need_y;
  int tail;
  int exchange_inside;
  int tail_fold;
  int needs_csr;
  int dense_layers;
  int step_form;
};
void igmc_step_plan(const ModelDev& m, const BatchDev& b, int B, int kind, StepPlan* p);
int igmc_dl_always();
void igmc_launch_g2_compose(const ModelDev& m, const float* P, void* stream);
void igmc_launch_dl_layer0(const ModelDev& m, const BatchDev& b, int B, int training, int use_flags, void* stream);
struct DlHead {
  const float* P;
  const uint8_t* inj_mask;
  uint64_t seed, step;
  float mult, grad_scale;
  float* out;
};
void igmc_launch_dl_bwd(const ModelDev& m, const BatchDev& b, const StepPlan& sp, int B, int use_flags, void* stream,
                        const DlHead* head = nullptr, int dense3 = 0);
void igmc_launch_dl_fwd(const ModelDev& m, const BatchDev& b, const StepPlan& sp, const float* P, int B, int training,
                        int use_flags, float* zero_out, void* stream);
void igmc_launch_head_sub(const ModelDev& m, const BatchDev& b, const float* P, int B, const uint8_t* inj_mask, uint64_t seed,
                          uint64_t step, float mult, float grad_scale, float* out, void* stream);
void igmc_launch_dl_layer(const ModelDev& m, const BatchDev& b, const float* P, int B, int l, int bwd, int use_flags,
                          float* zero_out, void* stream, int tables = 0);
int igmc_launch_graph_step2(const ModelDev& m, const BatchDev& b, const StepPlan& sp, const float* P, int B, int training,
                            int use_flags, const uint8_t* inj_mask, uint64_t seed, uint64_t step, float mult, float grad_scale,
                            float* out, void* stream, int nstash = 0, const int64_t* stash_ctrl = nullptr);

void igmc_prof_begin(const char* name, void* stream);
void igmc_prof_end(void* stream);
extern int g_igmc_prof_on;

#define IGMC_PLAUNCH(name, kern, grid, block, shmem, stream, ...)          \
  do {                                                                     \
    if (g_igmc_prof_on == 1) igmc_prof_begin(name, stream);                \
    IGMC_LAUNCH(kern, grid, block, shmem, stream, __VA_ARGS__);            \
    if (g_igmc_prof_on == 1) igmc_prof_end(stream);                        \
  } while (0)

template <typename F>
static inline void igmc_dispatch(F&& f) { f(); }
template <typename F, typename... Rest>
static inline void igmc_dispatch(F&& f, bool v, Rest... rest) {
  if (v) igmc_dispatch([&](auto... cs) { f(std::true_type{}, cs...); }, rest...);
  else igmc_dispatch([&](auto... cs) { f(std::false_type{}, cs...); }, rest...);
}
```

igmc_amd/csrc/model.hip:

```cpp
#include "model.h"
#include "g2_image.h"
#include "fin_stash.h"
#include "g2_words.h"
#include <stdlib.h>

struct XcdSeg {
  int lo, hi;
  int j, nj;
};
__device__ __forceinline__ XcdSeg igmc_xcd_segment(const BatchDev& b) {
  XcdSeg s;
  const int B = b.totals[3];
  const int x = blockIdx.x & 7;
  s.j = blockIdx.x >> 3;
  s.nj = (gridDim.x + 7 - x) >> 3;
  s.lo = b.node_off[(x * B) >> 3];
  s.hi = b.node_off[((x + 1) * B) >> 3];
  return s;
}


template <bool FLAGS, bool STORE>
__global__ __launch_bounds__(IGMC_BLOCK) void k_l0_fwd(BatchDev b, ModelDev m, const float* __restrict__ P,
                                                         float* __restrict__ out) {
// ... 1058 lines not shown
      ad[u] = 0.f;
      mk[u] = 0;
      if (extra) {
        dpv[u] = from_err ? m.err[gs] : gout[gs];
        ad[u] = m.a1[gs * 128 + j0 + li];
        mk[u] = m.lmask[gs * 128 + j0 + li];
      }
    }
#ifndef IGMC_HIPEMU
    __builtin_amdgcn_sched_barrier(0);
    asm volatile("" : "+v"(mk[0]), "+v"(mk[1]), "+v"(mk[2]), "+v"(mk[3]), "+v"(mk[4]), "+v"(mk[5]), "+v"(mk[6]), "+v"(mk[7]));
#endif
#pragma unroll
    for (int u = 0; u < 8; ++u) {
      const bool ok = g0 + 4 * u + kq < B;
      if (!ok) { av[u] = 0.f; bv[u] = 0.f; }
      if (extra) {
        dpv[u] = ok ? (from_err ? 2.f * dpv[u] * grad_scale : dpv[u]) * mult : 0.f;
        ad[u] = (ok && mk[u]) ? ad[u] * drop_scale : 0.f;
      }
    }
#pragma unroll
    for (int u = 0; u < 8; ++u) {
      acc = __builtin_amdgcn_mfma_f32_16x16x4f32(av[u], bv[u], acc, 0, 0, 0);
      if (extra) {
        accb1 = __builtin_amdgcn_mfma_f32_16x16x4f32(av[u], (g0 + 4 * u + kq < B) ? 1.f : 0.f, accb1, 0, 0, 0);
        accw2 = __builtin_amdgcn_mfma_f32_16x16x4f32(ad[u], dpv[u], accw2, 0, 0, 0);
        accb2 = __builtin_amdgcn_mfma_f32_16x16x4f32(1.f, dpv[u], accb2, 0, 0, 0);
      }
    }
  }
#pragma unroll
  for (int rr = 0; rr < 4; ++rr) grad[m.off_l1w + (int64_t)(j0 + kq * 4 + rr) * D + n0 + li] = acc[rr];
  if (extra && li == 0) {
#pragma unroll
    for (int rr = 0; rr < 4; ++rr) {
      grad[m.off_l1b + j0 + kq * 4 + rr] = accb1[rr];
      grad[m.off_l2w + j0 + kq * 4 + rr] = accw2[rr];
    }
    if (bx == 0 && kq == 0) grad[m.off_l2b] = accb2[0];
  }
}

__global__ __launch_bounds__(IGMC_BLOCK) void k_head_bwd_w_mfma(BatchDev b, ModelDev m, const float* __restrict__ P,
                                                                  const float* __restrict__ gout, int from_err,
                                                                  float grad_scale, float mult, float drop_scale,
                                                                  float* __restrict__ grad) {
  igmc_kernarg_warm<sizeof(BatchDev) + sizeof(ModelDev) + 32>();
  head_bwd_w_body(b, m, P, gout, from_err, grad_scale, mult, drop_scale, grad, blockIdx.x, blockIdx.y);
}

__global__ __launch_bounds__(IGMC_BLOCK) void k_wgrad_head(BatchDev b, ModelDev m, const float* __restrict__ P,
                                                             const float* __restrict__ gout, int from_err,
                                                             float grad_scale, float mult, float drop_scale,
                                                             float* __restrict__ grad, int nsl) {
  igmc_kernarg_warm<sizeof(BatchDev) + sizeof(ModelDev) + 32>();
  if ((int)blockIdx.y < nsl) {
    wgrad_body(b, m, blockIdx.y);
  } else {
    const int ny = (m.D / 16 + 3) / 4;
    if ((int)blockIdx.x < 8 * ny)
      head_bwd_w_body(b, m, P, gout, from_err, grad_scale, mult, drop_scale, grad, blockIdx.x & 7, blockIdx.x >> 3);
  }
}


__global__ __launch_bounds__(IGMC_BLOCK) void k_reduce_partials(ModelDev m, int n_gatt_parts, int l0_mfma,
                                                                  int n_wg_parts, const float* __restrict__ P,
                                                                  const int64_t* ctrl, int nstash) {
  igmc_kernarg_warm<sizeof(ModelDev) + 32>();
  __shared__ float sred[4][64];
  if (nstash && (int)blockIdx.x >= (int)gridDim.x - nstash) {
    fin_stash_body(m, P, (int)blockIdx.x - ((int)gridDim.x - nstash), ctrl);
    return;
  }
  const int wgs = 32 * IGMC_KCAT + 32, na = m.R * 4, rows0 = m.R * m.L + m.L + 1, n0 = rows0 * 32;
  const int nlay = l0_mfma ? 4 : 3;
  const int nblkA = (nlay * wgs + 63) / 64, nblkB = (3 * na + 3) / 4, nblkC = l0_mfma ? 0 : (n0 + 63) / 64;
  const int lane = threadIdx.x & 63, wave = threadIdx.x >> 6;
  int blk = blockIdx.x;
  if (blk < nblkA + nblkC) {
    const bool secA = blk < nblkA;
    const int o = (secA ? blk : blk - nblkA) * 64 + lane;
    const int nout = secA ? nlay * wgs : n0;
    float s = 0.f;
    if (o < nout) {
      if (secA) {
        const int l = o / wgs, i = o % wgs;
        const float* p = m.wg_part + (size_t)l * IGMC_WG_BLOCKS * wgs + i;
        for (int k0 = wave; k0 < n_wg_parts; k0 += 64) {
          float v[16];
#pragma unroll
          for (int u = 0; u < 16; ++u) {
            const int k = k0 + 4 * u;
            v[u] = p[(size_t)(k < n_wg_parts ? k : n_wg_parts - 1) * wgs];
          }
#pragma unroll
          for (int u = 0; u < 16; ++u)
            if (k0 + 4 * u < n_wg_parts) s += v[u];
        }
      } else {
        const float* p = m.l0_part + o;
        for (int k0 = wave; k0 < IGMC_L0_BLOCKS; k0 += 64) {
          float v[16];
#pragma unroll
          for (int u = 0; u < 16; ++u) {
            const int k = k0 + 4 * u;
            v[u] = p[(size_t)(k < IGMC_L0_BLOCKS ? k : IGMC_L0_BLOCKS - 1) * n0];
          }
#pragma unroll
          for (int u = 0; u < 16; ++u)
            if (k0 + 4 * u < IGMC_L0_BLOCKS) s += v[u];
        }
      }
    }
    sred[wave][lane] = s;
    __syncthreads();
    if (wave == 0 && o < nout) {
      const float tot = (sred[0][lane] + sred[1][lane]) + (sred[2][lane] + sred[3][lane]);
      if (secA && o >= 3 * wgs) {
        const int i = o - 3 * wgs, c = i / IGMC_KCAT, col = i % IGMC_KCAT;
        if (i < 32 * IGMC_KCAT && c < rows0 && col >= 128) m.graw[3 * wgs + 3 * na + c * 32 + (col - 128)] = tot;
      } else {
        m.graw[secA ? o : 3 * wgs + 3 * na + o] = tot;
      }
    }
  } else {
    blk -= nblkA + nblkC;
    const int o = blk * 4 + wave;
    if (o < 3 * na && blk < nblkB) {
      const int l = o / na, i = o % na;
      const float* p = m.gatt_part + (size_t)l * IGMC_GATHER_BLOCKS * na + i;
      float s = 0.f;
      for (int k0 = lane; k0 < n_gatt_parts; k0 += 64 * 8) {
        float v[8];
#pragma unroll
        for (int u = 0; u < 8; ++u) {
          const int k = k0 + 64 * u;
          v[u] = p[(size_t)(k < n_gatt_parts ? k : n_gatt_parts - 1) * na];
        }
#pragma unroll
        for (int u = 0; u < 8; ++u)
          if (k0 + 64 * u < n_gatt_parts) s += v[u];
      }
      s = igmc_wave_sum_f(s);
      if (lane == 0) m.graw[3 * wgs + o] = s;
    }
  }
}

struct TsSlots {
  int ng, nq, stride;
};
__device__ __forceinline__ TsSlots ts_slots(int nparts, int stride, int B) {
  TsSlots s;
  s.ng = (nparts < stride) ? nparts : ((B < stride) ? B : stride);
  s.nq = ((nparts + stride - 1) / stride) * s.ng;
  s.stride = stride;
  return s;
}
__device__ __forceinline__ int ts_slot(const TsSlots& s, int q) {
  const int qc = q < s.nq ? q : s.nq - 1;
  const int c = qc / s.ng, g = qc - c * s.ng;
  return c * s.stride + g;
}

__device__ __forceinline__ void reduce_ts_body(const ModelDev& m, int nparts, int stride, int B, int blk,
                                               const float* __restrict__ Pold = nullptr) {
  __shared__ float4 sred4[16][16];
  const int ts = m.ts_stride, rows0 = m.R * m.L + m.L + 1;
  const int lane = threadIdx.x & 63, wave = threadIdx.x >> 6;
  const int o4 = lane & 15, pg = wave * 4 + (lane >> 4);
  const int o0 = blk * 64 + 4 * o4;
  const int l = o0 / ts, i0 = o0 % ts;
  const bool ok4 = l < 4 && (l > 0 || i0 < rows0 * 32);
  float pbv[4] = {0.f, 0.f, 0.f, 0.f};
  if (Pold && wave == 0) {
    const int o = blk * 64 + lane, lo_ = o / ts, i = o % ts;
    if (lo_ < 4) {
      const int nE = ((lo_ == 0) ? m.L : 32) * 32;
      if (i < m.R * nE) {
        const float* basis = Pold + m.off_basis[lo_] + i % nE;
#pragma unroll
        for (int bb = 0; bb < 4; ++bb) pbv[bb] = basis[bb * nE];
      }
    }
  }
  float4 s4 = make_float4(0.f, 0.f, 0.f, 0.f);
  if (ok4) {
    const float* p = m.ts_part + (size_t)l * IGMC_TS_BLOCKS * ts + i0;
    const TsSlots sl = ts_slots(nparts, stride, B);
    const int nq = sl.nq;
    for (int q0 = pg; q0 < nq; q0 += 16 * 14) {
      float4 v[14];
#pragma unroll
      for (int u = 0; u < 14; ++u) v[u] = *(const float4*)(p + (size_t)ts_slot(sl, q0 + 16 * u) * ts);
#pragma unroll
      for (int u = 0; u < 14; ++u)
        if (q0 + 16 * u < nq) {
          s4.x += v[u].x; s4.y += v[u].y; s4.z += v[u].z; s4.w += v[u].w;
        }
    }
  }
  sred4[pg][o4] = s4;
  __syncthreads();
  if (wave == 0) {
    const float* sr = (const float*)sred4;
    float tot = 0.f;
#pragma unroll
    for (int g16 = 0; g16 < 16; ++g16) tot += sr[(g16 * 16 + (lane >> 2)) * 4 + (lane & 3)];
    const int o = blk * 64 + lane;
    const int lo_ = o / ts, i = o % ts;
    const bool ok = lo_ < 4 && (lo_ > 0 || i < rows0 * 32);
    if (!ok) tot = 0.f;
    if (ok) m.ts_raw[o] = tot;
    if (Pold) {
      float pb[4];
#pragma unroll
      for (int bb = 0; bb < 4; ++bb) pb[bb] = tot * pbv[bb];
#pragma unroll
      for (int bb = 0; bb < 4; ++bb)
#pragma unroll
        for (int d = 16; d >= 1; d >>= 1) pb[bb] += __shfl_xor(pb[bb], d, 64);
      if ((lane & 31) == 0 && lo_ < 4) *(float4*)(m.datt_part + (size_t)(o >> 5) * 4) = make_float4(pb[0], pb[1], pb[2], pb[3]);
    }
  }
}


__global__ __launch_bounds__(IGMC_BLOCK) void k_tail_ts(BatchDev b, ModelDev m, const float* __restrict__ P,
                                                          float grad_scale, float mult, float drop_scale,
                                                          float* __restrict__ grad, int nlin, int nparts, int stride,
                                                          int B, int nstash, const int64_t* ctrl, int bump_seq) {
  __builtin_amdgcn_s_setprio(3);
  igmc_kernarg_warm<sizeof(BatchDev) + sizeof(ModelDev) + 64>();
  const int nred = (int)gridDim.x - nlin - nstash;
  if (bump_seq && blockIdx.x == 0 && threadIdx.x == 0) m.gs_bar[1] += 1;
  if ((int)blockIdx.x < nlin)
    head_bwd_w_body(b, m, P, nullptr, 1, grad_scale, mult, drop_scale, grad, blockIdx.x & 7, blockIdx.x >> 3, B);
  else if ((int)blockIdx.x < nlin + nred)
    reduce_ts_body(m, nparts, stride, B, blockIdx.x - nlin, nstash ? P : nullptr);
  else
    fin_stash_body(m, P, blockIdx.x - nlin - nred, ctrl);
}

struct FinishArgs {
  int enabled;
  int use_flags;
  BatchDev b;
  ModelDev m;
  float ARR;
  float* loss;
  double* total;
};

__device__ __forceinline__ void ctrl_check_and_advance(int64_t* ctrl, const BatchDev& b, int use_flags) {
  const int64_t gq = ctrl[IGMC_CTRL_GQ] & 1;
  const int64_t want = ctrl[gq ? IGMC_CTRL_FIRST_ODD : IGMC_CTRL_FIRST] + ctrl[IGMC_CTRL_GK] * ctrl[IGMC_CTRL_BATCH];
  const int64_t got = b.stamp[0];
  int bad = 0;
  if (got >= 0 && got != want) bad |= 2;
  if (use_flags && got >= 0 && b.stamp[1] >= 0 && (uint64_t)b.stamp[1] != igmc_ctrl_drop_key(ctrl, (int)want)) bad |= 4;
  if (bad) atomicOr((unsigned long long*)(ctrl + IGMC_CTRL_SYNC_ERR), (unsigned long long)bad);
  ctrl_advance(ctrl);
}

__device__ __forceinline__ void loss_body(const BatchDev& b, const ModelDev& m, float ARR, float* loss,
                                          double* total, float* smf) {
  const int B = b.totals[3];
  float s = 0.f;
  for (int g = threadIdx.x; g < B; g += IGMC_BLOCK) s += m.err[g] * m.err[g];
  s = igmc_block_sum_f(s, smf);
  if (threadIdx.x == 0) {
    const float reg = m.arr_part[0] + m.arr_part[1] + m.arr_part[2] + m.arr_part[3];
    const float l0 = s / (float)B + ARR * reg;
    loss[0] = l0;
    loss[1] = s;
    if (total) total[0] += (double)l0 * (double)B;
  }
}

__device__ __forceinline__ void adam_elem(float* __restrict__ p, const float* __restrict__ g, float* __restrict__ m1,
                                          float* __restrict__ m2, int64_t i, float step_size, float inv_sqrt_bc2,
                                          float beta1, float beta2, float eps, float wd) {
  float gi = g[i];
  const float pi = p[i];
  if (wd != 0.f) gi += wd * pi;
  const float a = beta1 * m1[i] + (1.f - beta1) * gi;
  const float v = beta2 * m2[i] + (1.f - beta2) * gi * gi;
  m1[i] = a;
  m2[i] = v;
  p[i] = pi - step_size * a / (sqrtf(v) * inv_sqrt_bc2 + eps);
}

__device__ __forceinline__ void adam_store(float* p, float* m1, float* m2, int64_t i, float gi, float pv, float av, float vv,
                                           float step_size, float inv_sqrt_bc2, float beta1, float beta2, float eps, float wd) {
  if (wd != 0.f) gi += wd * pv;
  const float a = beta1 * av + (1.f - beta1) * gi;
  const float v = beta2 * vv + (1.f - beta2) * gi * gi;
  m1[i] = a;
  m2[i] = v;
  p[i] = pv - step_size * a / (sqrtf(v) * inv_sqrt_bc2 + eps);
}

__device__ __forceinline__ void adam_store_sep(float* p, float* m1, float* m2, int64_t i, float gi, float pv, float av, float vv,
                                               float step_size, float inv_sqrt_bc2, float beta1, float beta2, float eps, float wd) {
  if (wd != 0.f) gi += wd * pv;
  float a, v;
  {
#pragma clang fp contract(off)
    a = beta1 * av + (1.f - beta1) * gi;
    v = beta2 * vv + (1.f - beta2) * gi * gi;
  }
  m1[i] = a;
  m2[i] = v;
  p[i] = pv - step_size * a / (sqrtf(v) * inv_sqrt_bc2 + eps);
}

template <int NB>
__device__ __forceinline__ void adam_range(float* p, const float* g, float* m1, float* m2, int64_t lo, int64_t hi,
                                           float step_size, float inv_sqrt_bc2, float beta1, float beta2, float eps,
                                           float wd) {
  for (int64_t i0 = lo + threadIdx.x; i0 < hi; i0 += (int64_t)NB * IGMC_BLOCK) {
    float gv[NB], pv[NB], av[NB], vv[NB];
#pragma unroll
    for (int k = 0; k < NB; ++k) {
      const int64_t i = i0 + (int64_t)k * IGMC_BLOCK;
      const int64_t ic = i < hi ? i : hi - 1;
      gv[k] = g[ic];
      pv[k] = p[ic];
      av[k] = m1[ic];
      vv[k] = m2[ic];
    }
#pragma unroll
    for (int k = 0; k < NB; ++k) {
      const int64_t i = i0 + (int64_t)k * IGMC_BLOCK;
      if (i < hi) adam_store_sep(p, m1, m2, i, gv[k], pv[k], av[k], vv[k], step_size, inv_sqrt_bc2, beta1, beta2, eps, wd);
    }
  }
}

struct AdamTail {
  int enabled;
  float* p;
  float* m1;
  float* m2;
  float step_size, inv_sqrt_bc2, beta1, beta2, eps, wd;
  int64_t* ctrl;
  int* done;
  BatchDev b;
  float ARR;
  float* loss;
  double* total;
  int use_flags;
  const int* skip;
};

#define IGMC_FIN_NB 8
__global__ __launch_bounds__(IGMC_BLOCK) void k_finalize(ModelDev m, const float* P, float* __restrict__ grad,
                                                           float arr_coef, AdamTail at, int ts_mode) {
  igmc_kernarg_warm<sizeof(ModelDev) + sizeof(AdamTail) + 32>();
  if (at.skip && *at.skip) return;
  __shared__ float smf[8];
  __shared__ float sG[16], sM[16];
  __shared__ int s_lastl;
  __shared__ float sg10[4][10];
  __shared__ int s_last;
  if (at.enabled && at.ctrl) {
    const double* d = (const double*)at.ctrl;
    at.step_size = (float)d[IGMC_CTRL_STEP_SIZE];
    at.inv_sqrt_bc2 = (float)d[IGMC_CTRL_INV_SQRT_BC2];
    at.beta1 = (float)d[IGMC_CTRL_BETA1];
    at.beta2 = (float)d[IGMC_CTRL_BETA2];
    at.eps = (float)d[IGMC_CTRL_EPS];
    at.wd = (float)d[IGMC_CTRL_WD];
  }
  auto finish = [&](int64_t i, float g) { grad[i] = g; };
  if (blockIdx.x >= 4 * IGMC_FIN_NB) {
    const int64_t n_lin = m.n_params - m.off_l1w;
    const int nb = gridDim.x - 4 * IGMC_FIN_NB;
    const int64_t chunk = (n_lin + nb - 1) / nb;
    const int64_t lo = m.off_l1w + (int64_t)(blockIdx.x - 4 * IGMC_FIN_NB) * chunk;
    const int64_t hi = (lo + chunk < m.n_params) ? lo + chunk : m.n_params;
    adam_range<8>(at.p, grad, at.m1, at.m2, lo, hi, at.step_size, at.inv_sqrt_bc2, at.beta1, at.beta2, at.eps, at.wd);
  } else {
    const int l = blockIdx.x / IGMC_FIN_NB, part = blockIdx.x % IGMC_FIN_NB, tid = threadIdx.x;
    const int lane = tid & 63, wave = tid >> 6;
    const int fin = (l == 0) ? m.L : 32;
    const int nE = fin * 32;
    const int wgs = 32 * IGMC_KCAT + 32, na = m.R * 4, R = m.R;
    const float* basis = P + m.off_basis[l];
    const float* att = P + m.off_att[l];
    const int e0 = part * IGMC_BLOCK + tid, estep = IGMC_FIN_NB * IGMC_BLOCK;
    float gp[10];
// ... 276 lines not shown
#pragma unroll
            for (int i = 0; i < 32; ++i) t[i] = __shfl_xor(acc[i], d, 64);
#pragma unroll
            for (int i = 0; i < 32; ++i) acc[i] += t[i];
          }
          if (lane == 0) {
#pragma unroll
            for (int i = 0; i < 32; ++i) s_gpart[wave][i] = acc[i];
          }
          __syncthreads();
          if (tid < na) {
            float sacc = 0.f;
#pragma unroll
            for (int w = 0; w < IGMC_BLOCK / 64; ++w) sacc += s_gpart[w][tid];
            s_gatt0[tid] = sacc;
          }
        } else {
          for (int rb = wave; rb < na; rb += IGMC_BLOCK / 64) {
            const int r = rb >> 2, bb = rb & 3;
            float sacc = 0.f;
            for (int e = lane; e < nE; e += 64) sacc += t0[(size_t)r * nE + e] * P[m.off_basis[0] + (int64_t)bb * nE + e];
            sacc = igmc_wave_sum_f(sacc);
            if (lane == 0) s_gatt0[rb] = sacc;
          }
        }
      }
      __syncthreads();
    }
    __shared__ float s_attn[64];
    float pn[5] = {0.f, 0.f, 0.f, 0.f, 0.f};
    int e_img = -1;
    const bool emit = img && at.enabled && m.g2_w && R <= G2_NR * G2_NG_MAX && fin <= 32;
    const int ng = g2_groups(R, m.L);
    const int e = part * IGMC_BLOCK + tid;
    const bool has = e < nE;
    int64_t idx[5];
    float pv[5], m1v[5], m2v[5], g[5], tv[8];
#pragma unroll
    for (int q = 0; q < 5; ++q) {
      idx[q] = (q < 4) ? m.off_basis[l] + (int64_t)q * nE + (has ? e : 0) : m.off_root[l] + (has ? e : 0);
      pv[q] = has ? P[idx[q]] : 0.f;
      m1v[q] = (has && at.enabled) ? at.m1[idx[q]] : 0.f;
      m2v[q] = (has && at.enabled) ? at.m2[idx[q]] : 0.f;
      g[q] = 0.f;
    }
#pragma unroll
    for (int r = 0; r < 8; ++r) tv[r] = 0.f;
    if (has) {
      if (table) {
#pragma unroll
        for (int r = 0; r < 8; ++r) tv[r] = (r < R) ? t0[(size_t)r * nE + e] : 0.f;
        g[4] = t0[(size_t)R * nE + e];
      } else {
#pragma unroll
        for (int bb = 0; bb < 4; ++bb) g[bb] = raw[(e >> 5) * IGMC_KCAT + bb * 32 + (e & 31)];
        g[4] = raw[(e >> 5) * IGMC_KCAT + 128 + (e & 31)];
      }
    }
    const bool roles = part == 0 || emit;
    const bool bias_role = roles && tid < 32 && part == 0;
    const bool att_role = roles && !bias_role && tid >= 64 && tid - 64 < na;
    float bq[4] = {0.f, 0.f, 0.f, 0.f};
    if (bias_role) {
      const int64_t i = m.off_bias[l] + tid;
      bq[0] = table ? t0[(size_t)(R * fin + fin) * 32 + tid] : raw[32 * IGMC_KCAT + tid];
      bq[1] = P[i];
      bq[2] = at.enabled ? at.m1[i] : 0.f;
      bq[3] = at.enabled ? at.m2[i] : 0.f;
    }
    float dpre[32], am1 = 0.f, am2 = 0.f, ag = 0.f;
#pragma unroll
    for (int k = 0; k < 32; ++k) dpre[k] = 0.f;
    if (att_role) {
      const int rb = tid - 64, r = rb >> 2, bb = rb & 3;
      const int64_t i = m.off_att[l] + rb;
      if (at.enabled && !emit) {
        am1 = at.m1[i];
        am2 = at.m2[i];
      }
      if (bs) {
        if (l > 0) ag = m.graw[3 * wgs + (size_t)(l - 1) * na + rb];
      } else {
        const float* dp = m.datt_part + ((size_t)l * m.ts_stride + (size_t)r * nE) / 32 * 4 + bb;
#pragma unroll
        for (int k = 0; k < 32; ++k) dpre[k] = (k < fin) ? dp[(size_t)k * 4] : 0.f;
      }
    }
#pragma unroll
    for (int u = 0; u < (IGMC_STASH_LAYER + IGMC_BLOCK - 1) / IGMC_BLOCK; ++u) {
      const int i = tid + u * IGMC_BLOCK;
      if (i < IGMC_STASH_LAYER) s_st[i] = stq[u];
    }
    __syncthreads();
    if (roles) {
      if (bias_role) {
        fts_bias(m, grad, at, ng, l, R, fin, tid, bq, emit);
      } else if (tid >= 64) {
       for (int rb = tid - 64; rb < na; rb += IGMC_BLOCK - 64) {
        const int r = rb >> 2, bb = rb & 3;
        const bool first = rb == tid - 64;
        const int64_t i = m.off_att[l] + rb;
        const float pold = st[IGMC_STASH_ATT + rb];
        const float m1o = !at.enabled ? 0.f : emit ? st[IGMC_STASH_ATTM1 + rb] : first ? am1 : at.m1[i];
        const float m2o = !at.enabled ? 0.f : emit ? st[IGMC_STASH_ATTM2 + rb] : first ? am2 : at.m2[i];
        float g = 0.f;
        if (bs) {
          g = (l == 0) ? s_gatt0[rb] : first ? ag : m.graw[3 * wgs + (size_t)(l - 1) * na + rb];
        } else if (first && fin <= 32) {
#pragma unroll
          for (int k = 0; k < 32; ++k) g += dpre[k];
        } else {
          const float* dp = m.datt_part + ((size_t)l * m.ts_stride + (size_t)r * nE) / 32 * 4 + bb;
          for (int k0 = 0; k0 < fin; k0 += 32) {
            float v[32];
#pragma unroll
            for (int k = 0; k < 32; ++k) v[k] = (k0 + k < fin) ? dp[(size_t)(k0 + k) * 4] : 0.f;
#pragma unroll
            for (int k = 0; k < 32; ++k) g += v[k];
          }
        }
        const float anew = fts_att_entry(grad, at, st, R, rb, g, arr_coef, i, pold, m1o, m2o, part == 0);
        if (emit) s_attn[rb] = anew;
       }
      }
    }
    if (has) {
      if (table) {
        fts_col_table8(g, st, tv, R);
        for (int r = 8; r < R; ++r) {
          const float tvr = t0[(size_t)r * nE + e];
#pragma unroll
          for (int bb = 0; bb < 4; ++bb) g[bb] += st[IGMC_STASH_ATT + r * 4 + bb] * tvr;
        }
      }
      fts_col_emit(grad, at, st, arr_coef, idx, g, pv, m1v, m2v, pn);
      e_img = e;
    }
    if (emit) {
      __syncthreads();
      if (e_img >= 0) fts_image_col(m, ng, l, R, fin, e_img >> 5, e_img & 31, s_attn, pn, 0, 1);
    }
  } else if ((int)blockIdx.x < 4 * IGMC_FTS_NB + nlin) {
    const int64_t n_lin = m.n_params - m.off_l1w;
    const int64_t chunk = (n_lin + nlin - 1) / nlin;
    const int64_t lo = m.off_l1w + (int64_t)(blockIdx.x - 4 * IGMC_FTS_NB) * chunk;
    const int64_t hi = (lo + chunk < m.n_params) ? lo + chunk : m.n_params;
    adam_range<8>(at.p, grad, at.m1, at.m2, lo, hi, at.step_size, at.inv_sqrt_bc2, at.beta1, at.beta2, at.eps, at.wd);
  } else {
    loss_body(at.b, m, at.ARR, at.loss, at.total, smf);
    if (tid == 0 && at.ctrl) ctrl_check_and_advance(at.ctrl, at.b, at.use_flags);
  }
}

#define IGMC_TF_SETS 3
#define IGMC_TF_ROWS 384
#define IGMC_TF_O_ROWS (IGMC_TF_SETS * 1024)
#define IGMC_TF_O_ST (IGMC_TF_O_ROWS + IGMC_TF_ROWS)
#define IGMC_TF_O_DATT (IGMC_TF_O_ST + IGMC_STASH_LAYER)
#define IGMC_TF_O_ATTN (IGMC_TF_O_DATT + 32 * IGMC_FOLD_NA)
#define IGMC_TF_O_PN (IGMC_TF_O_ATTN + 64)
#define IGMC_TF_O_SMF (IGMC_TF_O_PN + 5 * 32)
#define IGMC_TF_WORDS (IGMC_TF_O_SMF + 16)
#define IGMC_TF_POLL ((32 * IGMC_FOLD_NA + IGMC_BLOCK - 1) / IGMC_BLOCK)
#define IGMC_TF_TIMEOUT_TICKS 20000000ll
#define IGMC_SYNC_ERR_FOLD 8

#if defined(IGMC_FIN_CLOCKS) && !defined(IGMC_HIPEMU)
__device__ unsigned long long g_fin_clk[64];
extern "C" int igmc_debug_fin_clocks(unsigned long long* out) {
  return hipMemcpyFromSymbol(out, HIP_SYMBOL(g_fin_clk), sizeof(g_fin_clk)) != hipSuccess;
}
#define TF_STAMP(on, k) do { if ((on) && threadIdx.x == 0) g_fin_clk[k] = __builtin_readcyclecounter(); } while (0)
#else
#define TF_STAMP(on, k) do { } while (0)
#endif

__global__ __launch_bounds__(IGMC_BLOCK) void k_tail_fin(BatchDev b, ModelDev m, const float* P, float grad_scale, float mult,
                                                           float drop_scale, float* grad, float arr_coef, AdamTail at, int nlin,
                                                           int nparts, int stride, int B, int bump_seq, int mute_layer) {
  __builtin_amdgcn_s_setprio(3);
  igmc_kernarg_warm<sizeof(BatchDev) + sizeof(ModelDev) + sizeof(AdamTail) + 64>();
  IGMC_DYN_SMEM(smem);
  float* S = (float*)smem;
  const int tid = threadIdx.x, lane = tid & 63, wave = tid >> 6;
  const float* stash = m.fin_stash;
  if (at.ctrl) {
    at.step_size = stash[IGMC_STASH_SCAL + 0];
    at.inv_sqrt_bc2 = stash[IGMC_STASH_SCAL + 1];
    at.beta1 = stash[IGMC_STASH_SCAL + 2];
    at.beta2 = stash[IGMC_STASH_SCAL + 3];
    at.eps = stash[IGMC_STASH_SCAL + 4];
    at.wd = stash[IGMC_STASH_SCAL + 5];
  }
  const int R = m.R, L = m.L, na = R * 4;
  const int nconv = 96 + L;
  const int blk = blockIdx.x;
  TF_STAMP(blk == 0, 0);
  TF_STAMP(blk == nconv, 16);
  TF_STAMP(blk == nconv + nlin, 32);
  if (blk < nconv) {
    const int l = blk < 96 ? 1 + (blk >> 5) : 0, c = blk < 96 ? (blk & 31) : blk - 96;
    const int fin = (l == 0) ? L : 32, nE = fin * 32, ts = m.ts_stride;
    const uint32_t tag = __float_as_uint(stash[IGMC_STASH_SCAL + IGMC_STASH_SEQ]) * 2u + 1u;
    float4* sred4 = (float4*)S;
    float* rows = S + IGMC_TF_O_ROWS;
    float* s_st = S + IGMC_TF_O_ST;
    float* s_datt = S + IGMC_TF_O_DATT;
    float* s_attn = S + IGMC_TF_O_ATTN;
    float* s_pn = S + IGMC_TF_O_PN;
    int* s_flag = (int*)(S + IGMC_TF_O_SMF + 8);
    const int ng = g2_groups(R, L);
    const int o4 = lane & 15, pg = wave * 4 + (lane >> 4);
    float stq[(IGMC_STASH_LAYER + IGMC_BLOCK - 1) / IGMC_BLOCK];
#pragma unroll
    for (int u = 0; u < (IGMC_STASH_LAYER + IGMC_BLOCK - 1) / IGMC_BLOCK; ++u) {
      const int i = tid + u * IGMC_BLOCK;
      stq[u] = stash[l * IGMC_STASH_LAYER + (i < IGMC_STASH_LAYER ? i : IGMC_STASH_LAYER - 1)];
    }
    const int f = tid & 31, e = c * 32 + f;
    const bool col = tid < 32, bias_role = c == 0 && tid >= 32 && tid < 64;
    int64_t idx[5];
    float pv[5], m1v[5], m2v[5], pvb[4] = {0.f, 0.f, 0.f, 0.f}, bq[4] = {0.f, 0.f, 0.f, 0.f};
#pragma unroll
    for (int q = 0; q < 5; ++q) {
      idx[q] = (q < 4) ? m.off_basis[l] + (int64_t)q * nE + e : m.off_root[l] + e;
      pv[q] = col ? P[idx[q]] : 0.f;
      m1v[q] = col ? at.m1[idx[q]] : 0.f;
      m2v[q] = col ? at.m2[idx[q]] : 0.f;
    }
    if (wave == 0) {
#pragma unroll
      for (int bb = 0; bb < 4; ++bb) pvb[bb] = P[idx[bb]];
    }
    if (bias_role) {
      const int64_t i = m.off_bias[l] + f;
      bq[1] = P[i];
      bq[2] = at.m1[i];
      bq[3] = at.m2[i];
    }
    if (tid == 0) *s_flag = 0;
    TF_STAMP(blk == 0, 1);
    const float* pl = m.ts_part + (size_t)l * IGMC_TS_BLOCKS * ts;
    const TsSlots sl = ts_slots(nparts, stride, B);
    const int nq = sl.nq;
    bool first_round = true;
    auto sum_columns = [&](int k0, int k1) {
      const int nsets = (k1 - k0 + 15) >> 4;
      int i0[IGMC_TF_SETS];
      float4 s4[IGMC_TF_SETS];
#pragma unroll
      for (int s = 0; s < IGMC_TF_SETS; ++s) {
        const int k = k0 + 16 * s + o4, kc = k < k1 ? k : k1 - 1, j = kc >> 3;
        const int row = j < R ? j * fin + c : j == R ? R * fin + c : R * fin + fin;
        i0[s] = row * 32 + 4 * (kc & 7);
        s4[s] = make_float4(0.f, 0.f, 0.f, 0.f);
      }
      for (int q0 = pg; q0 < nq; q0 += 16 * 14) {
        float4 v[IGMC_TF_SETS][14];
        size_t so[14];
#pragma unroll
        for (int u = 0; u < 14; ++u) so[u] = (size_t)ts_slot(sl, q0 + 16 * u) * ts;
#pragma unroll
        for (int s = 0; s < IGMC_TF_SETS; ++s)
          if (s < nsets) {
#pragma unroll
            for (int u = 0; u < 14; ++u) v[s][u] = *(const float4*)(pl + so[u] + i0[s]);
          }
#pragma unroll
        for (int s = 0; s < IGMC_TF_SETS; ++s)
          if (s < nsets) {
#pragma unroll
            for (int u = 0; u < 14; ++u)
              if (q0 + 16 * u < nq) {
                s4[s].x += v[s][u].x; s4[s].y += v[s][u].y; s4[s].z += v[s][u].z; s4[s].w += v[s][u].w;
              }
          }
      }
      if (!first_round) __syncthreads();
#pragma unroll
      for (int s = 0; s < IGMC_TF_SETS; ++s)
        if (s < nsets) sred4[(s * 16 + pg) * 16 + o4] = s4[s];
      if (first_round) {
#pragma unroll
        for (int u = 0; u < (IGMC_STASH_LAYER + IGMC_BLOCK - 1) / IGMC_BLOCK; ++u) {
          const int i = tid + u * IGMC_BLOCK;
          if (i < IGMC_STASH_LAYER) s_st[i] = stq[u];
        }
      }
      first_round = false;
      __syncthreads();
      if (wave < nsets) {
        const float* sr = (const float*)sred4;
        float tot = 0.f;
#pragma unroll
        for (int g16 = 0; g16 < 16; ++g16) tot += sr[((wave * 16 + g16) * 16 + (lane >> 2)) * 4 + (lane & 3)];
        const int k = k0 + 16 * wave + (lane >> 2);
        if (k < k1) rows[k * 4 + (lane & 3)] = tot;
      }
    };
    const int ncol_a = 8 * (R + 1);
    for (int k0 = 0; k0 < ncol_a; k0 += 16 * IGMC_TF_SETS) sum_columns(k0, k0 + 16 * IGMC_TF_SETS < ncol_a ? k0 + 16 * IGMC_TF_SETS : ncol_a);
    __syncthreads();
    TF_STAMP(blk == 0, 2);
    unsigned long long* words = m.fold_w + (size_t)l * 32 * IGMC_FOLD_NA;
    if (wave == 0) {
      const int h = lane >> 5;
      for (int r2 = 0; r2 < R; r2 += 2) {
        const int r = r2 + h;
        const float tot = r < R ? rows[r * 32 + f] : 0.f;
        float pb[4];
#pragma unroll
        for (int bb = 0; bb < 4; ++bb) pb[bb] = tot * pvb[bb];
#pragma unroll
        for (int bb = 0; bb < 4; ++bb)
#pragma unroll
          for (int d = 16; d >= 1; d >>= 1) pb[bb] += __shfl_xor(pb[bb], d, 64);
#ifdef IGMC_HIPEMU
        if (l == mute_layer) continue;
#endif
        if (f == 0 && r < R) {
#pragma unroll
          for (int bb = 0; bb < 4; ++bb) g2_pub_f32_agent(words + c * IGMC_FOLD_NA + r * 4 + bb, pb[bb], tag);
        }
      }
    }
    TF_STAMP(blk == 0, 3);
    if (c == 0) sum_columns(ncol_a, ncol_a + 8);
    TF_STAMP(blk == 0, 4);
    {
      const int nw = fin * na;
      const unsigned long long* wp[IGMC_TF_POLL];
      int wi[IGMC_TF_POLL];
#pragma unroll
      for (int u = 0; u < IGMC_TF_POLL; ++u) {
        const int w = tid + u * IGMC_BLOCK, wc = w < nw ? w : nw - 1;
        wi[u] = (wc / na) * IGMC_FOLD_NA + wc % na;
        wp[u] = words + wi[u];
      }
      bool ok = false;
#ifndef IGMC_HIPEMU
      const long long t0 = (long long)wall_clock64();
#endif
      for (long it = 0;; ++it) {
        unsigned long long w[IGMC_TF_POLL];
        bool all = true;
#pragma unroll
        for (int u = 0; u < IGMC_TF_POLL; ++u) w[u] = g2_ld_word(wp[u]);
#pragma unroll
        for (int u = 0; u < IGMC_TF_POLL; ++u) all = all && (uint32_t)(w[u] >> 32) == tag;
        if (all) {
#pragma unroll
          for (int u = 0; u < IGMC_TF_POLL; ++u) s_datt[wi[u]] = __uint_as_float((uint32_t)w[u]);
          ok = true;
          break;
        }
#ifndef IGMC_HIPEMU
        if ((it & 15) == 15 && (long long)wall_clock64() - t0 > IGMC_TF_TIMEOUT_TICKS) break;
        __builtin_amdgcn_s_sleep(2);
#else
        if (it > (1L << 12)) break;
        hipemu::yield();
#endif
      }
      if (!ok) *s_flag = 1;
    }
    __syncthreads();
    TF_STAMP(blk == 0, 5);
    if (*s_flag) {
      if (tid == 0) {
        *m.gs_err = 1;
        if (at.ctrl) atomicOr((unsigned long long*)(at.ctrl + IGMC_CTRL_SYNC_ERR), (unsigned long long)IGMC_SYNC_ERR_FOLD);
      }
      return;
    }
    const float* st = s_st;
    if (tid >= 64 && tid - 64 < na) {
      const int rb = tid - 64;
      float g = 0.f;
#pragma unroll
      for (int k = 0; k < 32; ++k) g += (k < fin) ? s_datt[k * IGMC_FOLD_NA + rb] : 0.f;
      s_attn[rb] = fts_att_entry(grad, at, st, R, rb, g, arr_coef, m.off_att[l] + rb, st[IGMC_STASH_ATT + rb],
                                 st[IGMC_STASH_ATTM1 + rb], st[IGMC_STASH_ATTM2 + rb], c == 0);
    }
    if (bias_role) {
      bq[0] = rows[(R + 1) * 32 + f];
      fts_bias(m, grad, at, ng, l, R, fin, f, bq, true);
    }
    if (col) {
      float g[5] = {0.f, 0.f, 0.f, 0.f, 0.f}, tv[8], pn[5];
#pragma unroll
      for (int r = 0; r < 8; ++r) tv[r] = (r < R) ? rows[r * 32 + f] : 0.f;
      g[4] = rows[R * 32 + f];
      fts_col_table8(g, st, tv, R);
      fts_col_emit(grad, at, st, arr_coef, idx, g, pv, m1v, m2v, pn);
#pragma unroll
      for (int q = 0; q < 5; ++q) s_pn[q * 32 + f] = pn[q];
    }
    TF_STAMP(blk == 0, 6);
    __syncthreads();
    {
      float pn[5];
#pragma unroll
      for (int q = 0; q < 5; ++q) pn[q] = s_pn[q * 32 + f];
      fts_image_col(m, ng, l, R, fin, c, f, s_attn, pn, tid >> 5, IGMC_BLOCK / 32);
    }
    TF_STAMP(blk == 0, 7);
  } else if (blk < nconv + nlin) {
    const int bx = (blk - nconv) & 7, by = (blk - nconv) >> 3, D = m.D;
    head_bwd_w_body(b, m, P, nullptr, 1, grad_scale, mult, drop_scale, grad, bx, by, B);
    __syncthreads();
    TF_STAMP(blk == nconv, 17);
    int64_t ix[5];
    bool okx[5];
    float gv[5], pv[5], av[5], vv[5];
#pragma unroll
    for (int k = 0; k < 4; ++k) {
      const int el = tid + k * IGMC_BLOCK, colx = by * 64 + (el & 63);
      okx[k] = colx < D;
      ix[k] = m.off_l1w + (int64_t)(bx * 16 + (el >> 6)) * D + (okx[k] ? colx : 0);
    }
    okx[4] = by == 0 && (tid < 32 || (tid == 32 && bx == 0));
    ix[4] = tid < 16 ? m.off_l1b + bx * 16 + tid : tid < 32 ? m.off_l2w + bx * 16 + tid - 16 : m.off_l2b;
    const float* gsrc = grad;
#pragma unroll
    for (int k = 0; k < 5; ++k) {
      const int64_t i = okx[k] ? ix[k] : m.off_l1w;
      gv[k] = gsrc[i];
      pv[k] = at.p[i];
      av[k] = at.m1[i];
      vv[k] = at.m2[i];
    }
#pragma unroll
    for (int k = 0; k < 5; ++k)
      if (okx[k]) adam_store_sep(at.p, at.m1, at.m2, ix[k], gv[k], pv[k], av[k], vv[k], at.step_size, at.inv_sqrt_bc2, at.beta1,
                                 at.beta2, at.eps, at.wd);
    TF_STAMP(blk == nconv, 18);
  } else {
    if (bump_seq && tid == 0) m.gs_bar[1] += 1;
    loss_body(at.b, m, at.ARR, at.loss, at.total, S + IGMC_TF_O_SMF);
    TF_STAMP(true, 33);
    if (tid == 0 && at.ctrl) ctrl_check_and_advance(at.ctrl, at.b, at.use_flags);
    TF_STAMP(true, 34);
  }
}

__global__ __launch_bounds__(IGMC_BLOCK) void k_loss(BatchDev b, ModelDev m, float ARR, float* __restrict__ loss) {
  igmc_kernarg_warm<sizeof(BatchDev) + sizeof(ModelDev) + 32>();
  __shared__ float smf[8];
  loss_body(b, m, ARR, loss, nullptr, smf);
}

__global__ __launch_bounds__(IGMC_BLOCK) void k_sse_acc(BatchDev b, const float* __restrict__ out, double* acc, int64_t* ctrl) {
  igmc_kernarg_warm<sizeof(BatchDev) + 32>();
  __shared__ float smf[8];
  const int B = b.totals[3];
  float s = 0.f;
  for (int g = threadIdx.x; g < B; g += IGMC_BLOCK) {
    const float d = out[g] - b.y[g];
    s += d * d;
  }
  s = igmc_block_sum_f(s, smf);
  if (threadIdx.x == 0) {
    acc[0] += (double)s;
    acc[1] += (double)B;
    if (ctrl) ctrl_advance(ctrl);
  }
}

__global__ void k_tick(int64_t* ctrl) {
  if (threadIdx.x == 0 && blockIdx.x == 0) ctrl_advance(ctrl);
}
__global__ void k_regroup(int64_t* ctrl, int M, int64_t first_cur, int64_t first_next) {
  if (threadIdx.x != 0 || blockIdx.x != 0) return;
  ctrl[IGMC_CTRL_GROUP] = M > 0 ? M : 1;
  ctrl[IGMC_CTRL_GK] = 0;
  ctrl[IGMC_CTRL_GQ] = 0;
  ctrl[IGMC_CTRL_FIRST] = first_cur;
  ctrl[IGMC_CTRL_FIRST_ODD] = first_next;
}

__global__ void k_step_gate(int64_t* ctrl, int q, int gk_min, long long delay_ticks, int delay_always,
                            long long timeout_ticks) {
#ifndef IGMC_HIPEMU
  if (threadIdx.x != 0 || blockIdx.x != 0) return;
  const long long t0 = wall_clock64();
  bool waited = false;
  for (;;) {
    if ((igmc_ctrl_ld(ctrl + IGMC_CTRL_GQ) & 1) != (int64_t)(q & 1)) return;
    if (igmc_ctrl_ld(ctrl + IGMC_CTRL_GK) >= (int64_t)gk_min) break;
    if (wall_clock64() - t0 > timeout_ticks) {
      atomicAdd((unsigned long long*)(ctrl + IGMC_CTRL_GATE_TIMEOUTS), 1ull);
      return;
    }
    waited = true;
    __builtin_amdgcn_s_sleep(16);
  }
  if (waited || delay_always) {
    const long long t1 = wall_clock64();
    while (wall_clock64() - t1 < delay_ticks) __builtin_amdgcn_s_sleep(8);
  }
#endif
}

__global__ __launch_bounds__(IGMC_BLOCK) void k_adam(float* __restrict__ p, const float* __restrict__ g,
                                                       float* __restrict__ m1, float* __restrict__ m2, int64_t n,
                                                       float step_size, float inv_sqrt_bc2, float beta1, float beta2,
                                                       float eps, float wd, int64_t* ctrl, int tick, FinishArgs fin) {
  __shared__ float smf[8];
  if (ctrl) {
    const double* d = (const double*)ctrl;
    step_size = (float)d[IGMC_CTRL_STEP_SIZE];
    inv_sqrt_bc2 = (float)d[IGMC_CTRL_INV_SQRT_BC2];
    beta1 = (float)d[IGMC_CTRL_BETA1];
    beta2 = (float)d[IGMC_CTRL_BETA2];
    eps = (float)d[IGMC_CTRL_EPS];
    wd = (float)d[IGMC_CTRL_WD];
  }
  {
    const int64_t chunk = ((n + gridDim.x - 1) / gridDim.x + IGMC_BLOCK - 1) / IGMC_BLOCK * IGMC_BLOCK;
    const int64_t lo = (int64_t)blockIdx.x * chunk, hi = (lo + chunk < n) ? lo + chunk : n;
    if (lo < n) adam_range<8>(p, g, m1, m2, lo, hi, step_size, inv_sqrt_bc2, beta1, beta2, eps, wd);
  }
  if (fin.enabled && blockIdx.x == 0) loss_body(fin.b, fin.m, fin.ARR, fin.loss, fin.total, smf);
  if (ctrl && tick) {
    __syncthreads();
    if (threadIdx.x == 0) {
      __threadfence();
      int* done = (int*)&ctrl[IGMC_CTRL_DONE];
      if (atomicAdd(done, 1) == (int)gridDim.x - 1) {
        *done = 0;
        if (fin.enabled) ctrl_check_and_advance(ctrl, fin.b, fin.use_flags);
        else ctrl_advance(ctrl);
      }
    }
  }
}

#include "launch.h"

static inline int igmc_rows_grid(int cap_rows, int rows_per_block, int max_blocks) {
  int g = (cap_rows + rows_per_block - 1) / rows_per_block;
  if (g > max_blocks) g = max_blocks;
  g = (g + 7) & ~7;
  return g < 8 ? 8 : g;
}
static inline int igmc_xcd_grid(const ModelDev& m, int B, int rows_per_block, int max_blocks) {
  const int slot = (m.node_cap + m.graph_cap - 1) / m.graph_cap;
  const long rows = (long)((B + 7) / 8) * slot;
  long per = (rows + rows_per_block - 1) / rows_per_block;
  if (per < 1) per = 1;
  long g = 8 * per;
  if (g > max_blocks) g = max_blocks & ~7;
  return (int)(g < 8 ? 8 : g);
}

static inline int igmc_l0_grid(const ModelDev& m, int B) {
  int rows = 4;
  if (m.R * m.L > 32) rows = (m.R * m.L) / 8;
  return igmc_xcd_grid(m, B, rows, IGMC_GATHER_BLOCKS);
}


static void launch_conv_fwd(const ModelDev& m, const BatchDev& b, const StepPlan& sp, const float* P, int B, int training,
                            int use_flags, void* stream) {
  if (sp.dl) igmc_launch_g2_compose(m, P, stream);
  if (sp.dlf) {
    igmc_launch_dl_fwd(m, b, sp, P, B, training, use_flags, training ? m.dpre[3] : nullptr, stream);
  } else if (sp.dl) {
    igmc_launch_dl_layer0(m, b, B, training, use_flags, stream);
  } else {
    const size_t l0s = (size_t)(m.R * m.L * 32 + m.L * 32 + 32) * sizeof(float) + (size_t)4 * m.R * m.L * sizeof(int);
    igmc_dispatch([&](auto uf, auto tr) {
      IGMC_PLAUNCH("k_l0_fwd", (k_l0_fwd<uf(), tr()>), igmc_l0_grid(m, B), IGMC_BLOCK, l0s, stream, b, m, P, m.h[0]);
    }, use_flags != 0, training != 0);
  }
  const int gt = igmc_xcd_grid(m, B, 16, 2048);
  const size_t fsm4 = (size_t)(16 * IGMC_TP + 1024 + m.R * 4) * sizeof(float);
  for (int l = 1; l < 4 && !sp.dlf; ++l) {
    float* zo = (training && l == 3) ? m.dpre[3] : nullptr;
    if (sp.dl) igmc_launch_dl_layer(m, b, P, B, l, 0, use_flags, zo, stream);
    else igmc_dispatch([&](auto uf) {
      IGMC_PLAUNCH("k_rgcn_layer_fwd", (k_rgcn_layer4<uf(), false>), gt, IGMC_BLOCK, fsm4, stream, b, m, P, l, zo);
    }, use_flags != 0);
  }
  if (training && sp.need_y)
    IGMC_PLAUNCH("k_dense_y_all", k_dense_y_all, dim3(igmc_rows_grid(m.node_cap, 64, 512), 3), IGMC_BLOCK,
                 (size_t)32 * (128 + 4) * sizeof(float), stream, b, m, P);
}

static void launch_layers_bwd(const ModelDev& m, const BatchDev& b, const StepPlan& sp, const float* P, int B, int use_flags,
                              int tables, void* stream) {
  const int gt = igmc_xcd_grid(m, B, 16, 2048);
  const size_t bsm4 = (size_t)(16 * IGMC_TP + 1024 + m.R * 4 + 16 * m.R * 4) * sizeof(float);
  for (int l = 3; l >= 1; --l) {
    if (sp.bwd_dense) igmc_launch_dl_layer(m, b, P, B, l, 1, use_flags, nullptr, stream, tables);
    else igmc_dispatch([&](auto uf) {
      IGMC_PLAUNCH("k_rgcn_layer_bwd", (k_rgcn_layer4<uf(), true>), gt, IGMC_BLOCK, bsm4, stream, b, m, P, l, (float*)nullptr);
    }, use_flags != 0);
  }
}

static void launch_reduce(const ModelDev& m, const BatchDev& b, const StepPlan& sp, const float* P, int B, const int64_t* ctrl,
                          int nstash, void* stream) {
  const int rows0 = m.R * m.L + m.L + 1, l0_mfma = rows0 <= 32;
  const float* d0 = m.dpre[0];
  if (l0_mfma) {
  } else if (rows0 <= 64) IGMC_PLAUNCH("k_l0_bwd", (k_l0_bwd<8>), IGMC_L0_BLOCKS, IGMC_BLOCK, 0, stream, b, m, d0, m.l0_part);
  else IGMC_PLAUNCH("k_l0_bwd", (k_l0_bwd<40>), IGMC_L0_BLOCKS, IGMC_BLOCK, 0, stream, b, m, d0, m.l0_part);
  const int nblk = ((l0_mfma ? 4 : 3) * igmc_wg_stride() + 63) / 64 + (l0_mfma ? 0 : (rows0 * 32 + 63) / 64) + (3 * m.R * 4 + 3) / 4;
  IGMC_PLAUNCH("k_reduce_partials", k_reduce_partials, nblk + nstash, IGMC_BLOCK, 0, stream, m,
               sp.bwd_dense ? sp.dl_grid : igmc_xcd_grid(m, B, 16, 2048), l0_mfma, IGMC_WG_BLOCKS, P, ctrl, nstash);
}

static void launch_tail_ts(const ModelDev& m, const BatchDev& b, const float* P, int B, float grad_scale, float mult, float* grad,
                           int nlin, int nparts, int stride, int nstash, const int64_t* ctrl, int bump_seq, void* stream) {
  IGMC_PLAUNCH("k_tail_ts", k_tail_ts, nlin + (4 * m.ts_stride + 63) / 64 + nstash, IGMC_BLOCK, 0, stream, b, m, P, grad_scale,
               mult, 2.f, grad, nlin, nparts, stride, B, nstash, ctrl, bump_seq);
}

static void launch_tail_fin(const ModelDev& m, const BatchDev& b, const float* P, int B, float grad_scale, float mult, float* grad,
                            float arr_coef, const AdamTail& at, int nlin, int nparts, int stride, int bump_seq, void* stream) {
  int mute = -1;
#ifdef IGMC_HIPEMU
  if (const char* e = getenv("IGMC_EMU_FOLD_MUTE")) mute = atoi(e);
  hipemu::rt().co_cs = 32;
  hipemu::rt().co_stride = -1;
  hipemu::rt().co_block = 0;
#endif
  IGMC_PLAUNCH("k_tail_fin", k_tail_fin, 96 + m.L + nlin + 1, IGMC_BLOCK, (size_t)IGMC_TF_WORDS * sizeof(float), stream, b, m, P,
               grad_scale, mult, 2.f, grad, arr_coef, at, nlin, nparts, stride, B, bump_seq, mute);
}

static int launch_exchange(const ModelDev& m, int tail, const StepExchange* xch, float* grad, void* stream) {
  if (!xch || tail == IGMC_TAIL_HANDOFF) return 0;
  const int rows0 = m.R * m.L + m.L + 1;
  const int64_t n = tail == IGMC_TAIL_TS ? (int64_t)4 * m.ts_stride + (int64_t)4 * m.ts_stride / 32 * 4
                                         : (int64_t)3 * igmc_wg_stride() + 3 * m.R * 4 + rows0 * 32;
  return xch->sum(xch->user, tail == IGMC_TAIL_TS ? m.ts_raw : m.graw, n, grad + m.off_l1w, m.n_params - m.off_l1w, stream);
}

static void launch_finalize(const ModelDev& m, const BatchDev& b, const float* P, float* grad, float arr_coef, int tail,
                            int ts_mode, const AdamTail& at, int img, float ARR, float* loss, int* img_emitted, void* stream) {
  const int bs = tail == IGMC_TAIL_BS;
  if (tail == IGMC_TAIL_HANDOFF) {
    if (at.enabled) IGMC_PLAUNCH("k_finalize_adam", k_finalize, 4 * IGMC_FIN_NB + 32, IGMC_BLOCK, 0, stream, m, P, grad, arr_coef, at, ts_mode);
    else IGMC_PLAUNCH("k_finalize", k_finalize, 4 * IGMC_FIN_NB, IGMC_BLOCK, 0, stream, m, P, grad, arr_coef, at, ts_mode);
  } else if (at.enabled) {
    IGMC_PLAUNCH("k_finalize_adam", k_finalize_ts, 4 * IGMC_FTS_NB + 32 + 1, IGMC_BLOCK, 0, stream, m, P, grad, arr_coef, at, 32, bs, img);
    if (img_emitted) *img_emitted = img;
  } else {
    IGMC_PLAUNCH("k_finalize", k_finalize_ts, 4 * IGMC_FTS_NB, IGMC_BLOCK, 0, stream, m, P, grad, arr_coef, at, 0, bs, 0);
  }
  if (!at.enabled && loss) igmc_launch_loss(m, b, ARR, loss, stream);
}


void igmc_launch_forward(const ModelDev& m, const BatchDev& b, const StepPlan& sp, const float* P, int B, int training,
                         int use_flags, const uint8_t* inj_mask, uint64_t seed, uint64_t step, float mult,
                         float* out, void* stream) {
  if (sp.family == IGMC_FAM_G2) {
    igmc_launch_graph_step2(m, b, sp, P, B, 0, use_flags, nullptr, seed, step, mult, 0.f, out, stream);
    return;
  }
  launch_conv_fwd(m, b, sp, P, B, training, use_flags, stream);
  const int hgrid = (B + IGMC_HG - 1) / IGMC_HG;
  const size_t fs = (size_t)IGMC_HG * m.D * sizeof(float);
  if (m.D % 16 == 0)
    IGMC_PLAUNCH("k_head_fwd", k_head_fwd_mfma, (B + 15) / 16, 512, 0, stream, b, m, P, training, inj_mask, seed, step,
                 mult, out);
  else if (fs <= 48 * 1024)
    IGMC_PLAUNCH("k_head_fwd", (k_head_fwd<true>), hgrid, 512, fs, stream, b, m, P, training, inj_mask, seed, step,
                 mult, out);
  else
    IGMC_PLAUNCH("k_head_fwd", (k_head_fwd<false>), hgrid, 512, 0, stream, b, m, P, training, inj_mask, seed, step,
                 mult, out);
}

void igmc_launch_conv_forward(const ModelDev& m, const BatchDev& b, const StepPlan& sp, const float* P, int B, int training,
                              int use_flags, void* stream) {
  launch_conv_fwd(m, b, sp, P, B, training, use_flags, stream);
}

void igmc_launch_backward(const ModelDev& m, const BatchDev& b, const StepPlan& sp, const float* P, int B, int use_flags,
                          const float* gout, int from_err, float grad_scale, float mult, float drop_scale,
                          float arr_coef, float* grad, void* stream) {
  const int hgrid = (B + IGMC_HG - 1) / IGMC_HG;
  if (m.D % 16 == 0)
    IGMC_PLAUNCH("k_head_bwd_a", k_head_bwd_a_mfma, dim3((B + 15) / 16, (m.D / 16 + 7) / 8), 512, 0, stream, b, m, P,
                 gout, from_err, grad_scale, mult, drop_scale, m.dpre[3]);
  else
    IGMC_PLAUNCH("k_head_bwd_a", k_head_bwd_a, hgrid, 1024, 0, stream, b, m, P, gout, from_err, grad_scale, mult,
                 drop_scale, m.dpre[3]);
  if (m.D % 16 == 0)
    IGMC_PLAUNCH("k_head_bwd_w", k_head_bwd_w_mfma, dim3(8, (m.D / 16 + 3) / 4), IGMC_BLOCK, 0, stream, b, m, P, gout,
                 from_err, grad_scale, mult, drop_scale, grad);
  else
    IGMC_PLAUNCH("k_head_bwd_w", k_head_bwd_w, dim3(17, (m.D + 255) / 256), IGMC_BLOCK, 0, stream, b, m, P, gout, from_err,
                 grad_scale, mult, drop_scale, grad);
  igmc_launch_conv_backward(m, b, sp, P, B, use_flags, arr_coef, grad, stream);
}

void igmc_launch_conv_backward(const ModelDev& m, const BatchDev& b, const StepPlan& sp, const float* P, int B, int use_flags,
                               float arr_coef, float* grad, void* stream) {
  AdamTail none;
  memset(&none, 0, sizeof(none));
  if (sp.dlb) {
    const int gstride = (B + 7) & ~7;
    igmc_launch_dl_bwd(m, b, sp, B, use_flags, stream, nullptr, 1);
    launch_tail_ts(m, b, P, B, 0.f, 1.f, grad, 0, (sp.nqu + sp.nqv) * gstride, gstride, 4, nullptr, 1, stream);
  } else {
    const int l0_mfma = m.R * m.L + m.L + 1 <= 32;
    launch_layers_bwd(m, b, sp, P, B, use_flags, 0, stream);
    IGMC_PLAUNCH("k_wgrad", k_wgrad, dim3(IGMC_WG_BLOCKS, l0_mfma ? 4 : 3), IGMC_BLOCK, 0, stream, b, m, 0);
    launch_reduce(m, b, sp, nullptr, B, nullptr, 0, stream);
  }
  launch_finalize(m, b, P, grad, arr_coef, sp.tail, 0, none, 0, 0.f, nullptr, nullptr, stream);
}

int igmc_launch_loss_grad(const ModelDev& m_in, const BatchDev& b, const StepPlan& sp, float* P, int B, int use_flags,
                          const uint8_t* inj_mask, uint64_t seed, uint64_t step, float mult, float ARR,
                          float grad_scale, float arr_scale, float* out, float* grad, float* loss, const AdamTail* adam,
                          void* stream, const StepExchange* xch, int* img_emitted) {
  ModelDev m = m_in;
  m.adam_m1 = adam ? adam->m1 : nullptr;
  m.adam_m2 = adam ? adam->m2 : nullptr;
  if (img_emitted) *img_emitted = 0;
  const int rows0 = m.R * m.L + m.L + 1;
  const int img = adam && m.g2_w && m.R <= G2_NR * G2_NG_MAX && rows0 <= (g2_t0_rows(m.R, m.L) == 32 ? 32 : 48);
  const int ny = (m.D / 16 + 3) / 4;
  const float* Pc = P;
  AdamTail at;
  memset(&at, 0, sizeof(at));
  if (adam) {
    at = *adam;
    at.enabled = sp.fast_head;
    at.b = b;
    at.ARR = ARR;
  }
  at.use_flags = use_flags;
  at.skip = xch ? xch->failed : nullptr;
  const int64_t* ctrl = adam ? at.ctrl : nullptr;
  if (!sp.fast_head) {
    igmc_launch_forward(m, b, sp, Pc, B, 1, use_flags, inj_mask, seed, step, mult, out, stream);
    igmc_launch_backward(m, b, sp, Pc, B, use_flags, nullptr, 1, grad_scale, mult, 2.f, ARR * arr_scale, grad, stream);
    if (adam) {
      igmc_launch_finish(m, b, at.p, grad, at.m1, at.m2, at.step_size, at.inv_sqrt_bc2, at.beta1, at.beta2, at.eps, at.wd,
                         at.ctrl, ARR, at.loss, at.total, use_flags, stream);
    } else if (loss) {
      igmc_launch_loss(m, b, ARR, loss, stream);
    }
    return 0;
  }
  const int tables = sp.tail == IGMC_TAIL_TS;
  if (sp.family == IGMC_FAM_G2) {
    const int fold = sp.tail_fold && tables && adam && at.enabled && img && !xch;
    const int stride = (sp.cs > 1) ? ((B + 7) & ~7) : IGMC_TS_BLOCKS;
    const int bump_seq = igmc_launch_graph_step2(m, b, sp, Pc, B, 1, use_flags, inj_mask, seed, step, mult, grad_scale, out, stream,
                                                 fold ? 4 : 0, ctrl);
    if (fold) {
      launch_tail_fin(m, b, Pc, B, grad_scale, mult, grad, ARR * arr_scale, at, 8 * ny, sp.grid, stride, bump_seq, stream);
      if (img_emitted) *img_emitted = 1;
      return 0;
    }
    launch_tail_ts(m, b, Pc, B, grad_scale, mult, grad, 8 * ny, sp.grid, (sp.cs > 1) ? ((B + 7) & ~7) : IGMC_TS_BLOCKS,
                   tables ? 4 : 0, ctrl, bump_seq, stream);
  } else {
    launch_conv_fwd(m, b, sp, Pc, B, 1, use_flags, stream);
    if (sp.dlts) {
      const DlHead hd = {Pc, inj_mask, seed, step, mult, grad_scale, out};
      const int inside = sp.dlb && sp.head_inside;
      if (!inside) igmc_launch_head_sub(m, b, Pc, B, inj_mask, seed, step, mult, grad_scale, out, stream);
      if (sp.dlb) igmc_launch_dl_bwd(m, b, sp, B, use_flags, stream, inside ? &hd : nullptr);
      else launch_layers_bwd(m, b, sp, Pc, B, use_flags, 1, stream);
      const int gstride = (B + 7) & ~7;
      launch_tail_ts(m, b, Pc, B, grad_scale, mult, grad, 8 * ny, (sp.nqu + sp.nqv) * gstride, gstride, 4, ctrl, sp.dlf ? 1 : 0, stream);
    } else {
      const int gy = igmc_rows_grid(m.node_cap, 128, 512), hb = (B + 15) / 16, nsl = rows0 <= 32 ? 4 : 3;
      IGMC_PLAUNCH("k_head_train", k_head_train, dim3(hb > gy ? hb : gy, 4), 512, (size_t)32 * (128 + 4) * sizeof(float), stream,
                   b, m, Pc, inj_mask, seed, step, mult, grad_scale, out);
      launch_layers_bwd(m, b, sp, Pc, B, use_flags, 0, stream);
      IGMC_PLAUNCH("k_wgrad_head", k_wgrad_head, dim3(IGMC_WG_BLOCKS, nsl + 1), IGMC_BLOCK, 0, stream, b, m, Pc,
                   (const float*)nullptr, 1, grad_scale, mult, 2.f, grad, nsl);
      launch_reduce(m, b, sp, Pc, B, ctrl, sp.tail == IGMC_TAIL_BS ? 4 : 0, stream);
    }
  }
  if (const int rc = launch_exchange(m, sp.tail, xch, grad, stream)) return rc;
  launch_finalize(m, b, Pc, grad, ARR * arr_scale, sp.tail, sp.family == IGMC_FAM_G2, at, img, ARR, loss, img_emitted, stream);
  return 0;
}

int igmc_launch_train_step(const ModelDev& m, const BatchDev& b, const StepPlan& sp, float* P, int B, int use_flags,
                           const uint8_t* inj_mask, uint64_t seed, uint64_t step, float mult, float ARR, float* out,
                           float* grad, float* m1, float* m2, float step_size, float inv_sqrt_bc2, float beta1,
                           float beta2, float eps, float wd, int64_t* ctrl, int* done, float* loss, double* total,
                           void* stream, float grad_scale, const StepExchange* xch, int* img_emitted) {
  AdamTail at;
  memset(&at, 0, sizeof(at));
  at.p = P; at.m1 = m1; at.m2 = m2;
  at.step_size = step_size; at.inv_sqrt_bc2 = inv_sqrt_bc2; at.beta1 = beta1; at.beta2 = beta2; at.eps = eps; at.wd = wd;
  at.ctrl = ctrl; at.done = done; at.loss = loss; at.total = total;
  return igmc_launch_loss_grad(m, b, sp, P, B, use_flags, inj_mask, seed, step, mult, ARR,
                               grad_scale != 0.f ? grad_scale : 1.0f / (float)B, 1.0f, out, grad, nullptr, &at, stream, xch,
                               img_emitted);
}

void igmc_launch_loss(const ModelDev& m, const BatchDev& b, float ARR, float* loss, void* stream) {
  IGMC_PLAUNCH("k_loss", k_loss, 1, IGMC_BLOCK, 0, stream, b, m, ARR, loss);
}

void igmc_launch_sse(const BatchDev& b, const float* out, double* acc, int64_t* ctrl, void* stream) {
  IGMC_PLAUNCH("k_sse_acc", k_sse_acc, 1, IGMC_BLOCK, 0, stream, b, out, acc, ctrl);
}

void igmc_launch_tick(int64_t* ctrl, void* stream) { IGMC_PLAUNCH("k_tick", k_tick, 1, 64, 0, stream, ctrl); }
void igmc_launch_regroup(int64_t* ctrl, int M, int64_t first_cur, int64_t first_next, void* stream) {
  IGMC_PLAUNCH("k_regroup", k_regroup, 1, 64, 0, stream, ctrl, M, first_cur, first_next);
}
void igmc_launch_gate(int64_t* ctrl, int q, int gk_min, long long delay_ticks, int delay_always, long long timeout_ticks,
                      void* stream) {
  IGMC_PLAUNCH("k_step_gate", k_step_gate, 1, 64, 0, stream, ctrl, q, gk_min, delay_ticks, delay_always, timeout_ticks);
}

static int adam_grid(int64_t n) {
  int grid = (int)((n + 8 * IGMC_BLOCK - 1) / (8 * IGMC_BLOCK));
  if (grid > 256) grid = 256;
  return grid < 1 ? 1 : grid;
}

void igmc_launch_adam(float* p, const float* g, float* m1, float* m2, int64_t n, float step_size,
                      float inv_sqrt_bc2, float beta1, float beta2, float eps, float wd, int64_t* ctrl, int tick,
                      void* stream) {
  FinishArgs fin;
  memset(&fin, 0, sizeof(fin));
  IGMC_PLAUNCH("k_adam", k_adam, adam_grid(n), IGMC_BLOCK, 0, stream, p, g, m1, m2, n, step_size, inv_sqrt_bc2, beta1,
               beta2, eps, wd, ctrl, tick, fin);
}

void igmc_launch_finish(const ModelDev& m, const BatchDev& b, float* p, const float* g, float* m1, float* m2,
                        float step_size, float inv_sqrt_bc2, float beta1, float beta2, float eps, float wd,
                        int64_t* ctrl, float ARR, float* loss, double* total, int use_flags, void* stream) {
  FinishArgs fin;
  fin.enabled = 1;
  fin.use_flags = use_flags;
  fin.b = b;
  fin.m = m;
  fin.ARR = ARR;
  fin.loss = loss;
  fin.total = total;
  IGMC_PLAUNCH("k_step_finish", k_adam, adam_grid(m.n_params), IGMC_BLOCK, 0, stream, p, g, m1, m2,
               (int64_t)m.n_params, step_size, inv_sqrt_bc2, beta1, beta2, eps, wd, ctrl, ctrl ? 1 : 0, fin);
}

int igmc_model_prepare(const ModelDev& m) {
#ifndef IGMC_HIPEMU
  const int bsm4 = (int)((size_t)(16 * IGMC_TP + 1024 + m.R * 4 + 16 * m.R * 4) * sizeof(float));
  if (bsm4 > 48 * 1024) {
    if (bsm4 > 150 * 1024) return 1;
    if (hipFuncSetAttribute((const void*)k_rgcn_layer4<true, true>, hipFuncAttributeMaxDynamicSharedMemorySize, bsm4) != hipSuccess) return 1;
    if (hipFuncSetAttribute((const void*)k_rgcn_layer4<false, true>, hipFuncAttributeMaxDynamicSharedMemorySize, bsm4) != hipSuccess) return 1;
  }
#endif
  (void)m;
  return igmc_gs_prepare();
}
```

igmc_amd/csrc/step_plan.h:

```cpp
#include <limits.h>

#define IGMC_HOOK_UNSET INT_MIN
struct StepHooks {
  int graph_step;
  int gs_cluster;
  int gs_grid;
  int dl;
  int dl_fused;
  int dl_ts;
  int dl_gsplit;
  int dl_head;
  int fin_mode;
  int tail_fold;
};
static int step_hook(const char* name, int unset) {
  const char* e = getenv(name);
  return e ? atoi(e) : unset;
}
static StepHooks step_hooks() {
  StepHooks hk;
  hk.graph_step = step_hook("IGMC_GRAPH_STEP", 1);
  hk.gs_cluster = step_hook("IGMC_GS_CLUSTER", IGMC_HOOK_UNSET);
  hk.gs_grid = step_hook("IGMC_GS_GRID", 0);
  hk.dl = step_hook("IGMC_DL", 1);
  hk.dl_fused = step_hook("IGMC_DL_FUSED", IGMC_HOOK_UNSET);
  hk.dl_ts = step_hook("IGMC_DL_TS", 1);
  hk.dl_gsplit = step_hook("IGMC_DL_GSPLIT", 1);
  hk.dl_head = step_hook("IGMC_DL_HEAD", 1);
  hk.fin_mode = step_hook("IGMC_FIN_MODE", 1);
  hk.tail_fold = step_hook("IGMC_TAIL_FOLD", 1);
  return hk;
}
int igmc_dl_always() { return step_hook("IGMC_DL_ALWAYS", 0) == 1; }

static int gs_cluster(const StepHooks& hk, int B) {
#ifdef IGMC_HIPEMU
  int want = 1;
#else
  static int cus = -1;
  if (cus < 0) {
    hipDeviceProp_t prop;
    int dev = 0;
    cus = (hipGetDevice(&dev) == hipSuccess && hipGetDeviceProperties(&prop, dev) == hipSuccess) ? prop.multiProcessorCount : 0;
  }
  int want = (cus >= 240) ? 4 : 1;
#endif
  if (hk.gs_cluster != IGMC_HOOK_UNSET) want = hk.gs_cluster;
  const int stride = (B + 7) & ~7;
  if (want >= 4 && 4 * stride <= 224) return 4;
  if (want >= 2 && 2 * stride <= 224) return 2;
  return 1;
}
static int gs_grid(const StepHooks& hk, int B) {
  int cap = IGMC_WG_BLOCKS;
  if (hk.gs_grid > 0 && hk.gs_grid < cap) cap = hk.gs_grid;
  return B < cap ? B : cap;
}
static int g2_eligible(const StepHooks& hk, const ModelDev& m, const BatchDev& b, int B, G2Layout* lay, int* cs_out) {
  if (hk.graph_step == 0 || !igmc_g2_xcd_ok()) return 0;
  const int cs = gs_cluster(hk, B);
  if (!igmc_g2_layout(m, b, cs, lay)) return 0;
  *cs_out = cs;
  return 1;
}

static int dl_kp(const BatchDev& b) {
  const int cmax = b.cap_u > b.cap_v ? b.cap_u : b.cap_v;
  return 32 * ((cmax + 31) >> 5) + 8;
}
static int dl_base_ok(const StepHooks& hk, const ModelDev& m, const BatchDev& b, int B, int wide) {
  if (hk.dl == 0) return 0;
  if (!b.relm || !b.relmT || !m.g2_w || m.L > 8) return 0;
  const int rows0 = m.R * m.L + m.L + 1;
  if (wide ? (g2_groups(m.R, m.L) == 1 || m.R > G2_NR * G2_NG_MAX || rows0 > 48) : (m.R > G2_NR || rows0 > 32)) return 0;
  const int cmax = b.cap_u > b.cap_v ? b.cap_u : b.cap_v;
  const DlSplit sq = dl_split(b.cap_u, b.cap_v, B);
  return cmax <= 256 && B * (sq.nqu + sq.nqv) <= IGMC_GATHER_BLOCKS;
}
static int dl_eligible(const StepHooks& hk, const ModelDev& m, const BatchDev& b, int B) {
  return dl_base_ok(hk, m, b, B, 0) && dl_lds(dl_kp(b)) <= (size_t)160 * 1024;
}
static int dl_ts_eligible(const StepHooks& hk, const ModelDev& m, const BatchDev& b, int B) {
  if (hk.dl_ts == 0 || !dl_eligible(hk, m, b, B) || !m.ts_part || !m.cnt0) return 0;
  const DlSplit sq = dl_split(b.cap_u, b.cap_v, B);
  const int stride = (B + 7) & ~7;
  if ((sq.nqu + sq.nqv) * stride > IGMC_TS_BLOCKS || m.R * m.L > 20) return 0;
  return dl_lds(dl_kp(b), true) <= (size_t)160 * 1024;
}
static int dl_fwd_eligible(const StepHooks& hk, const ModelDev& m, const BatchDev& b, int B) {
  if (!igmc_g2_xcd_ok() || hk.dl_fused == 0) return 0;
  if (!dl_eligible(hk, m, b, B) || !m.g2_ex || m.ex_nodes < DLX_K || b.graph_cap > m.g2_graphs) return 0;
  const DlSplit sq = dl_split(b.cap_u, b.cap_v, B);
  if (B * (sq.nqu + sq.nqv) > 224) return 0;
  return (size_t)dlf_words(dl_kp(b)) * 4 <= (size_t)160 * 1024;
}
static int dl_bwd_eligible(const StepHooks& hk, const ModelDev& m, const BatchDev& b, int B) {
  if (!dl_fwd_eligible(hk, m, b, B) || !dl_ts_eligible(hk, m, b, B) || hk.dl_fused == 1) return 0;
  return (size_t)dlb_words(dl_kp(b)) * 4 <= (size_t)160 * 1024;
}
static int dl_wide(const StepHooks& hk, const ModelDev& m, const BatchDev& b, int B, int tables_tail) {
  if (!igmc_g2_xcd_ok() || !dl_base_ok(hk, m, b, B, 1)) return 0;
  if ((hk.dl_fused != IGMC_HOOK_UNSET && hk.dl_fused != 2) || hk.dl_ts == 0 || !tables_tail) return 0;
  if (!m.g2_ex || m.ex_nodes < DLX_K || b.graph_cap > m.g2_graphs || !m.ts_part || !m.cnt0) return 0;
  const DlSplit sq = dl_split(b.cap_u, b.cap_v, B);
  const int stride = (B + 7) & ~7, kp = dl_kp(b);
  if (B * (sq.nqu + sq.nqv) > 224 || (sq.nqu + sq.nqv) * stride > IGMC_TS_BLOCKS) return 0;
  const int ng = g2_groups(m.R, m.L);
  return (size_t)dlf_words(kp, ng) * 4 <= (size_t)160 * 1024 && (size_t)dlb_words(kp, ng) * 4 <= (size_t)160 * 1024;
}
static int dl_gsplit(const StepHooks& hk, const ModelDev& m, const BatchDev& b, int B) {
  if (g2_groups(m.R, m.L) != 2 || g2_rel_groups(m.R) != 2 || hk.dl_gsplit == 0) return 0;
  const DlSplit sq = dl_split(b.cap_u, b.cap_v, B);
  const int nbu = (b.cap_u + 15) >> 4, nbv = (b.cap_v + 15) >> 4;
  if ((nbu + sq.nqu - 1) / sq.nqu > DL_GB || (nbv + sq.nqv - 1) / sq.nqv > DL_GB) return 0;
  const int kp = dl_kp(b);
  return (size_t)dlf_words_gs(kp) * 4 <= 160 * 1024 && (size_t)dlb_words_gs(kp) * 4 <= 160 * 1024;
}

void igmc_step_plan(const ModelDev& m, const BatchDev& b, int B, int kind, StepPlan* p) {
  memset(p, 0, sizeof(*p));
  const StepHooks hk = step_hooks();
  const int ny = (m.D / 16 + 3) / 4;
  const int l0_mfma = m.R * m.L + m.L + 1 <= 32;
  const int fin = hk.fin_mode && m.fin_stash;
  const int tables_tail = fin && m.datt_part;
  const int fts = tables_tail && m.R <= 8;
  p->kind = kind;
  p->fast_head = (m.D % 16 == 0) && 8 * ny <= IGMC_WG_BLOCKS;
  const int fused = kind == IGMC_CALL_STEP && p->fast_head;
  const int g2 = l0_mfma && g2_eligible(hk, m, b, B, &p->lay, &p->cs);
  const int narrow = dl_eligible(hk, m, b, B), wide = dl_wide(hk, m, b, B, tables_tail);
  p->dense_layers = narrow || wide;
  p->needs_csr = !(narrow || (kind != IGMC_CALL_CONV && (g2 || wide)));
  if (g2 && (fused || kind == IGMC_CALL_EVAL)) {
    p->family = IGMC_FAM_G2;
    p->grid = (p->cs > 1) ? p->cs * ((B + 7) & ~7) : gs_grid(hk, B);
    p->tail = fts ? IGMC_TAIL_TS : IGMC_TAIL_HANDOFF;
    p->exchange_inside = fused && fts;
    p->tail_fold = fused && fts && hk.tail_fold != 0 && m.fold_w && m.L <= 32 && 4 * m.R <= IGMC_FOLD_NA;
    p->step_form = 1;
    return;
  }
  const int dlf1 = narrow && dl_fwd_eligible(hk, m, b, B), dlb1 = dlf1 && dl_bwd_eligible(hk, m, b, B);
  p->wide = wide;
  p->dl = wide || narrow;
  p->dlf = wide || dlf1;
  if (fused) {
    p->dlts = wide || (narrow && l0_mfma && fts && dl_ts_eligible(hk, m, b, B));
    p->dlb = p->dlts && (wide || dlb1);
    p->self_seq = !p->dlts;
    p->head_inside = hk.dl_head != 0;
    p->bwd_dense = p->dl;
    p->exchange_inside = fin && m.R <= IGMC_FBS_MAX_R;
    p->tail = p->dlts ? IGMC_TAIL_TS : p->exchange_inside ? IGMC_TAIL_BS : IGMC_TAIL_HANDOFF;
  } else {
    p->dlts = p->dlb = fts && l0_mfma && m.dcat[0] && dlb1;
    p->self_seq = 1;
    p->bwd_dense = narrow;
    p->need_y = kind != IGMC_CALL_EVAL && !p->dlts;
    p->tail = p->dlts ? IGMC_TAIL_TS : IGMC_TAIL_HANDOFF;
  }
  p->gsplit = p->dlf && dl_gsplit(hk, m, b, B);
  p->family = p->dlf ? IGMC_FAM_DLF : p->dl ? IGMC_FAM_DL : IGMC_FAM_ROWS;
  if (p->dl) {
    const DlSplit sq = dl_split(b.cap_u, b.cap_v, B);
    p->nqu = sq.nqu;
    p->nqv = sq.nqv;
    p->dl_grid = B * (sq.nqu + sq.nqv);
  }
  p->step_form = (wide && p->gsplit) ? 3 : p->dlf ? 2 : 0;
}
```

igmc_amd/engine.py:

```python
import ctypes as C

import numpy as np

from . import _lib


def _p(x):
    if x is None:
        return None
    if isinstance(x, np.ndarray):
        return C.c_void_p(x.ctypes.data)
    return C.c_void_p(int(x))


class Graph(object):

    def __init__(self, A, device=0, lib=None):
        self.lib = lib or _lib.load()
        A = A.tocsr()
        A.sum_duplicates()
        A.sort_indices()
        self.n_users, self.n_items = A.shape
        indptr = np.ascontiguousarray(A.indptr, dtype=np.int32)
        indices = np.ascontiguousarray(A.indices, dtype=np.int32)
# ... 81 lines not shown
    def set_side_features(self, ptr, n_side):
        self.lib.call('igmc_batch_set_side_features', self.handle, _p(ptr), int(n_side))

    def bind_side_source(self, ptr, n_side):
        self.lib.call('igmc_batch_bind_side_source', self.handle, _p(ptr), int(n_side))

    def dense_layers(self, ws):
        return bool(self.lib.cdll.igmc_model_dense_layers(ws.handle, self.handle, int(self.B or self.max_graphs)))

    def want_transposed(self):
        self.lib.call('igmc_batch_want_transposed', self.handle)

    def set_lean(self, lean=True):
        self.lib.call('igmc_batch_set_lean', self.handle, int(bool(lean)))

    def assume_size(self, B):
        self.lib.call('igmc_batch_assume_size', self.handle, int(B))
        self.B = int(B)

    def info(self, stream=None):
        info = _lib.BatchInfo()
        self.lib.call('igmc_batch_get_info', self.handle, C.byref(info), _p(stream))
        return info

    def device_ptr(self, name):
        return self.lib.igmc_batch_device_ptr(self.handle, _lib.BUF[name])

    def download(self, stream=None):
        info = self.info(stream)
        if info.overflow:
            raise RuntimeError('batch arena overflow: N=%d E=%d exceed the capacity (%d, %d)' % (
                info.num_nodes, info.num_edges, info.node_capacity, info.edge_capacity))
        B, N, E = info.num_graphs, info.num_nodes, info.num_edges
        out = dict(
            node_off=np.zeros(B + 1, np.int32), n_users=np.zeros(B, np.int32),
            node_label=np.zeros(N, np.uint8), node_gid=np.zeros(N, np.int32), node_graph=np.zeros(N, np.int32),
            row_ptr=np.zeros(N + 1, np.int32), col=np.zeros(E, np.int32), erel=np.zeros(E, np.uint8),
            elab=np.zeros(E, np.uint8), eflag=np.zeros(E, np.uint8), y=np.zeros(B, np.float32))
        self.lib.call('igmc_batch_download', self.handle, _p(out['node_off']), _p(out['n_users']),
                      _p(out['node_label']), _p(out['node_gid']), _p(out['node_graph']), _p(out['row_ptr']),
                      _p(out['col']), _p(out['erel']), _p(out['elab']), _p(out['eflag']), _p(out['y']), _p(stream))
        out['B'], out['N'], out['E'] = B, N, E
        return out

    def close(self):
        if getattr(self, 'handle', None):
            self.lib.igmc_batch_destroy(self.handle)
            self.handle = None

    def __del__(self):
        try:
            self.close()
        except Exception:
            pass


class BatchSet(object):

    def __init__(self, arenas):
        self.arenas = list(arenas)
        self.lib = self.arenas[0].lib
        hs = (C.c_void_p * len(self.arenas))(*[a.handle for a in self.arenas])
        h = C.c_void_p()
        self.lib.call('igmc_batch_set_create', C.cast(hs, C.c_void_p), len(self.arenas), C.byref(h))
        self.handle = h

    def extract(self, count, link_u, link_v, link_y, link_idx, sel0, B, sample_ratio=1.0, seed=0, drop_p=0.0,
                force_undirected=False, drop_seed=0, stream=None):
        self.lib.call('igmc_extract_group', self.arenas[0].graph.handle, self.handle, int(count), _p(link_u), _p(link_v),
                      _p(link_y), _p(link_idx), int(sel0), int(B), float(sample_ratio), int(seed) & (2 ** 64 - 1),
                      float(drop_p), int(bool(force_undirected)), int(drop_seed) & (2 ** 64 - 1), _p(stream))
        for a in self.arenas[:count]:
            a.B = int(B)

    def close(self):
        if getattr(self, 'handle', None):
            self.lib.cdll.igmc_batch_set_destroy(self.handle)
            self.handle = None

    def __del__(self):
        try:
            self.close()
        except Exception:
            pass


class ModelWorkspace(object):

    PARAM_KINDS = ('BASIS', 'ROOT', 'BIAS', 'ATT')

    def __init__(self, lib, device, num_relations, num_bases, num_labels, n_side, max_nodes, max_edges, max_graphs):
        self.lib = lib
        self.R, self.Bs, self.L, self.S = int(num_relations), int(num_bases), int(num_labels), int(n_side)
        self.max_nodes, self.max_edges, self.max_graphs = int(max_nodes), int(max_edges), int(max_graphs)
        h = C.c_void_p()
        lib.call('igmc_model_create', int(device), self.R, self.Bs, self.L, self.S, self.max_nodes,
                 self.max_edges, self.max_graphs, C.byref(h))
        self.handle = h
        self.n_params = int(lib.igmc_param_count(h))

    def layout(self):
        out = []
        for l in range(4):
            fin = self.L if l == 0 else 32
            shapes = dict(BASIS=(self.Bs, fin, 32), ROOT=(fin, 32), BIAS=(32,), ATT=(self.R, self.Bs))
            for kind, key in (('BASIS', 'basis'), ('ROOT', 'root'), ('BIAS', 'bias'), ('ATT', 'att')):
                cnt = C.c_int64()
                off = self.lib.igmc_param_offset(self.handle, l, _lib.P[kind], C.byref(cnt))
                assert cnt.value == int(np.prod(shapes[kind]))
                out.append(('convs.%d.%s' % (l, key), int(off), shapes[kind]))
        D = 256 + self.S
        for kind, key, shape in (('LIN1_W', 'lin1.weight', (128, D)), ('LIN1_B', 'lin1.bias', (128,)),
                                 ('LIN2_W', 'lin2.weight', (1, 128)), ('LIN2_B', 'lin2.bias', (1,))):
            cnt = C.c_int64()
            off = self.lib.igmc_param_offset(self.handle, 0, _lib.P[kind], C.byref(cnt))
            assert cnt.value == int(np.prod(shape))
            out.append((key, int(off), shape))
        return out

    def forward(self, params, batch, out, training=False, use_edge_flags=False, lin_mask=None, seed=0, step=0,
                multiply_by=1.0, stream=None):
        self.lib.call('igmc_model_forward', self.handle, _p(params), batch.handle, int(bool(training)),
                      int(bool(use_edge_flags)), _p(lin_mask), int(seed) & (2 ** 64 - 1), int(step) & (2 ** 64 - 1),
                      float(multiply_by), _p(out), _p(stream))

    def backward(self, params, batch, gout, grad, multiply_by=1.0, stream=None):
        self.lib.call('igmc_model_backward', self.handle, _p(params), batch.handle, _p(gout), float(multiply_by),
                      _p(grad), _p(stream))

    def loss_grad(self, params, batch, out, grad, loss, use_edge_flags=False, lin_mask=None, seed=0, step=0,
                  multiply_by=1.0, ARR=0.0, grad_scale=None, arr_scale=1.0, stream=None):
        if grad_scale is None:
            grad_scale = 1.0 / batch.B
        self.lib.call('igmc_model_loss_grad', self.handle, _p(params), batch.handle, int(bool(use_edge_flags)),
                      _p(lin_mask), int(seed) & (2 ** 64 - 1), int(step) & (2 ** 64 - 1), float(multiply_by),
                      float(ARR), float(grad_scale), float(arr_scale), _p(out), _p(grad), _p(loss), _p(stream))

    def dense_path(self, batch, B):
        return bool(self.lib.igmc_model_dense_path(self.handle, batch.handle, int(B)))

    def step_form(self, batch, B):
        return int(self.lib.igmc_model_step_form(self.handle, batch.handle, int(B)))

    GEOMETRY_KEYS = ('form', 'family', 'wg_per_graph', 'grid', 'nqu', 'nqv', 'groups', 'gsplit', 'tables', 'kp', 'dl_bwd')
    FAMILIES = ('rows', 'subgraph', 'dense_fused', 'dense_layer')

    def step_geometry(self, batch, B):
        n = len(self.GEOMETRY_KEYS)
        out = (C.c_int32 * n)()
        self.lib.call('igmc_model_step_geometry', self.handle, batch.handle, int(B), C.cast(out, C.c_void_p), n)
        g = dict(zip(self.GEOMETRY_KEYS, [int(x) for x in out]))
        g['family'] = self.FAMILIES[g['family']]
        return g

    def adam_step(self, params, grad, exp_avg, exp_avg_sq, step, lr, beta1=0.9, beta2=0.999, eps=1e-8,
                  weight_decay=0.0, stream=None):
        self.lib.call('igmc_adam_step', _p(params), _p(grad), _p(exp_avg), _p(exp_avg_sq), self.n_params, int(step),
                      float(lr), float(beta1), float(beta2), float(eps), float(weight_decay), _p(stream))

    def sse_accumulate(self, out, batch, acc, stream=None, ctrl=None):
        if ctrl is not None:
            self.lib.call('igmc_sse_accumulate_tick', _p(out), batch.handle, _p(acc), _p(ctrl), _p(stream))
        else:
            self.lib.call('igmc_sse_accumulate', _p(out), batch.handle, _p(acc), _p(stream))

    def scores_store(self, out, batch, acc, scores, labels, n, err, first=-1, stream=None, ctrl=None):
        self.lib.call('igmc_scores_store', _p(out), batch.handle, _p(acc), _p(scores), _p(labels), int(n), int(first),
                      _p(ctrl), _p(err), _p(stream))

    def close(self):
        if getattr(self, 'handle', None):
            self.lib.igmc_model_destroy(self.handle)
            self.handle = None

    def __del__(self):
        try:
            self.close()
        except Exception:
            pass


def adam_step(lib, params, grad, exp_avg, exp_avg_sq, n, step, lr, beta1=0.9, beta2=0.999, eps=1e-8,
              weight_decay=0.0, stream=None):
    lib.call('igmc_adam_step', _p(params), _p(grad), _p(exp_avg), _p(exp_avg_sq), int(n), int(step), float(lr),
             float(beta1), float(beta2), float(eps), float(weight_decay), _p(stream))


def select_extremes(keys, num, grid=0, lib=None, stream=None):
    import torch
    lib = lib or _lib.load()
    if keys.dtype != torch.float32 or keys.dim() != 1 or not keys.is_cuda or not keys.is_contiguous():
        raise ValueError('keys: a contiguous 1-D float32 device tensor')
    n, num = keys.numel(), int(num)
    nbytes = lib.igmc_select_scratch_bytes(n, num, int(grid))
    if nbytes < 0:
        raise RuntimeError('igmc_select_scratch_bytes failed: %s' % lib.cdll.igmc_last_error().decode())
    scratch = torch.empty(nbytes // 8, dtype=torch.int64, device=keys.device)
    idx = torch.empty(2, num, dtype=torch.int32, device=keys.device)
    key = torch.empty(2, num, dtype=torch.float32, device=keys.device)
    count = torch.zeros(1, dtype=torch.int32, device=keys.device)
    st = torch.cuda.current_stream().cuda_stream if stream is None else stream
    lib.call('igmc_select_extremes', _p(keys.data_ptr()), n, num, _p(idx[0].data_ptr()), _p(idx[1].data_ptr()),
             _p(key[0].data_ptr()), _p(key[1].data_ptr()), _p(count.data_ptr()), _p(scratch.data_ptr()), nbytes, int(grid),
             _p(st))
    c = min(n, num)
    return idx[0, :c], idx[1, :c], key[0, :c], key[1, :c]


def select_segments(keys, seg_off, num, geometry=0, lib=None, stream=None):
    import torch
    lib = lib or _lib.load()
    if keys.dtype != torch.float32 or keys.dim() != 1 or not keys.is_cuda or not keys.is_contiguous():
        raise ValueError('keys: a contiguous 1-D float32 device tensor')
    if seg_off.dtype != torch.int64 or seg_off.dim() != 1 or not seg_off.is_cuda or not seg_off.is_contiguous():
        raise ValueError('seg_off: a contiguous 1-D int64 device tensor')
    ns, num = seg_off.numel() - 1, int(num)
    nbytes = lib.igmc_select_segments_scratch_bytes(ns, num, int(geometry))
    if nbytes < 0:
        raise RuntimeError('igmc_select_segments_scratch_bytes failed: %s' % lib.cdll.igmc_last_error().decode())
    idx = torch.full((ns, num), -1, dtype=torch.int32, device=keys.device)
    key = torch.zeros(ns, num, dtype=torch.float32, device=keys.device)
    count = torch.zeros(ns, dtype=torch.int32, device=keys.device)
    if keys.numel() == 0:
        return idx, key, count
    scratch = torch.empty(nbytes // 8, dtype=torch.int64, device=keys.device)
    st = torch.cuda.current_stream().cuda_stream if stream is None else stream
    lib.call('igmc_select_segments', _p(keys.data_ptr()), _p(seg_off.data_ptr()), ns, num, _p(idx.data_ptr()),
             _p(key.data_ptr()), _p(count.data_ptr()), _p(scratch.data_ptr()), nbytes, int(geometry), _p(st))
    return idx, key, count


RANK_ERRORS = ((1, 'query offsets that are not 0 = q_off[0] <= ... <= q_off[ns] = the number of queries'),
               (2, 'a segment outside the keys'))


def _dev_vector(t, dtype, what):
    if t.dtype != dtype or t.dim() != 1 or not t.is_cuda or not t.is_contiguous():
        raise ValueError('%s: a contiguous 1-D %s device tensor' % (what, str(dtype).replace('torch.', '')))


def rank_segments(keys, ids, seg_off, q_off, q_id, geometry=0, err=None, lib=None, stream=None):
    import torch
    lib = lib or _lib.load()
    _dev_vector(keys, torch.float32, 'keys')
    _dev_vector(ids, torch.int32, 'ids')
    _dev_vector(seg_off, torch.int64, 'seg_off')
    _dev_vector(q_off, torch.int64, 'q_off')
    _dev_vector(q_id, torch.int32, 'q_id')
    if ids.numel() != keys.numel() or q_off.numel() != seg_off.numel():
        raise ValueError('one id per key and one query range per segment')
    ns, n, nq = seg_off.numel() - 1, keys.numel(), q_id.numel()
    pos = torch.full((nq,), -1, dtype=torch.int32, device=keys.device)
    rank = torch.full((nq,), -1, dtype=torch.int32, device=keys.device)
    if n == 0 or nq == 0:
        return pos, rank
    own = err is None
    if own:
        err = torch.zeros(1, dtype=torch.int32, device=keys.device)
    st = torch.cuda.current_stream().cuda_stream if stream is None else stream
    lib.call('igmc_rank_segments', _p(keys.data_ptr()), _p(ids.data_ptr()), n, _p(seg_off.data_ptr()), ns,
             _p(q_off.data_ptr()), _p(q_id.data_ptr()), nq, _p(pos.data_ptr()), _p(rank.data_ptr()), _p(err.data_ptr()),
             int(geometry), _p(st))
    if own:
        _raise_rank_errors(err, 'igmc_rank_segments')
    return pos, rank


def rank_metrics(rank, q_off, ks, relevant=None, grid=0, err=None, lib=None, stream=None):
    import torch
    lib = lib or _lib.load()
    _dev_vector(rank, torch.int32, 'rank')
    _dev_vector(q_off, torch.int64, 'q_off')
    if relevant is not None:
        _dev_vector(relevant, torch.uint8, 'relevant')
        if relevant.numel() != rank.numel():
            raise ValueError('one relevance flag per query')
    ks = [int(k) for k in ks]
    if not 1 <= len(ks) <= 8 or min(ks) < 1 or max(ks) > 2 ** 31 - 1:
        raise ValueError('ks: 1 to 8 cut-offs K in [1, 2^31)')
    ns, nk = q_off.numel() - 1, len(ks)
    d_ks = torch.tensor(ks, dtype=torch.int32, device=rank.device)
    cnt = torch.zeros(ns, 2 + nk, dtype=torch.int32, device=rank.device)
    dcg = torch.zeros(ns, 2 * nk, dtype=torch.float64, device=rank.device)
    own = err is None
    if own:
        err = torch.zeros(1, dtype=torch.int32, device=rank.device)
    st = torch.cuda.current_stream().cuda_stream if stream is None else stream
    lib.call('igmc_rank_metrics', _p(rank.data_ptr() if rank.numel() else None), _p(q_off.data_ptr()),
             _p(None if relevant is None else relevant.data_ptr()), rank.numel(), ns, _p(d_ks.data_ptr()), nk,
             _p(cnt.data_ptr()), _p(dcg.data_ptr()), _p(err.data_ptr()), int(grid), _p(st))
    if own:
        _raise_rank_errors(err, 'igmc_rank_metrics')
    return cnt, dcg


def _raise_rank_errors(err, what):
    e = int(err.item())
    if e:
        raise RuntimeError('%s: %s (err=%d)' % (what, '; '.join(w for b, w in RANK_ERRORS if e & b), e))


def profile_enable(lib, on):
    lib.igmc_profile_enable(int(bool(on)))


def profile_fetch(lib, cap=64):
# ... 42 lines not shown
```

include/igmc_hip.h:

```cpp
#ifndef IGMC_HIP_H
#define IGMC_HIP_H
#include <stddef.h>
#include <stdint.h>

#ifdef __cplusplus
extern "C" {
#endif

typedef struct igmc_graph igmc_graph;
typedef struct igmc_batch igmc_batch;
typedef struct igmc_model igmc_model;

#define IGMC_HIDDEN 32
#define IGMC_NUM_LAYERS 4
#define IGMC_LIN1_OUT 128

const char* igmc_last_error(void);
int igmc_version(void);

int igmc_graph_create(int n_users, int n_items, int64_t nnz,
                      const int32_t* h_indptr, const int32_t* h_indices, const uint8_t* h_rating,
                      int device, igmc_graph** out);
void igmc_graph_destroy(igmc_graph* g);
int64_t igmc_graph_hbm_bytes(const igmc_graph* g);

int igmc_batch_create(const igmc_graph* g, int max_graphs, int hop, int max_nodes_per_hop,
                      igmc_batch** out);
void igmc_batch_destroy(igmc_batch* b);

int igmc_extract_batch(const igmc_graph* g, igmc_batch* b,
                       const int32_t* d_link_u, const int32_t* d_link_v, const float* d_link_y,
                       const int32_t* d_link_idx, int first, int B,
                       double sample_ratio, uint64_t seed, uint64_t epoch, void* stream);

int igmc_extract_batch_replay(const igmc_graph* g, igmc_batch* b, int B,
                              const int32_t* h_unodes, const uint8_t* h_udist, const int32_t* h_uoff,
                              const int32_t* h_vnodes, const uint8_t* h_vdist, const int32_t* h_voff,
                              const float* h_y, void* stream);

int igmc_extract_batch_cached(const igmc_graph* g, igmc_batch* b,
                              const int64_t* d_uoff, const int32_t* d_unodes, const uint8_t* d_udist,
                              const int64_t* d_voff, const int32_t* d_vnodes, const uint8_t* d_vdist,
                              const float* d_link_y, const int32_t* d_link_idx, int first, int B, void* stream);

typedef struct igmc_batch_set igmc_batch_set;
int igmc_batch_set_create(igmc_batch* const* batches, int count, igmc_batch_set** out);
void igmc_batch_set_destroy(igmc_batch_set* s);
int igmc_extract_group(const igmc_graph* g, igmc_batch_set* s, int count,
                       const int32_t* d_link_u, const int32_t* d_link_v, const float* d_link_y,
                       const int32_t* d_link_idx, int sel0, int B, double sample_ratio, uint64_t seed,
                       float drop_p, int force_undirected, uint64_t drop_seed, void* stream);

int igmc_batch_edge_dropout(igmc_batch* b, float p, int force_undirected,
                            uint64_t seed, uint64_t step, void* stream);
int igmc_batch_set_edge_flags(igmc_batch* b, const uint8_t* h_flags, int64_t n);
int igmc_batch_clear_edge_flags(igmc_batch* b);

typedef struct igmc_batch_info {
  int32_t num_graphs, num_nodes, num_edges, overflow;
  int32_t node_capacity, edge_capacity, num_labels, hop;
} igmc_batch_info;
int igmc_batch_get_info(const igmc_batch* b, igmc_batch_info* out, void* stream);
int igmc_batch_download(const igmc_batch* b, int32_t* node_off, int32_t* n_users, uint8_t* node_label,
                        int32_t* node_gid, int32_t* node_graph, int32_t* row_ptr, int32_t* col,
                        uint8_t* erel, uint8_t* elab, uint8_t* eflag, float* y, void* stream);
enum { IGMC_BUF_NODE_OFF = 0, IGMC_BUF_N_USERS, IGMC_BUF_NODE_LABEL, IGMC_BUF_NODE_GID,
       IGMC_BUF_NODE_GRAPH, IGMC_BUF_ROW_PTR, IGMC_BUF_ECR, IGMC_BUF_ECODE,
       IGMC_BUF_EFLAG, IGMC_BUF_Y, IGMC_BUF_TOTALS, IGMC_BUF_COUNT };
void* igmc_batch_device_ptr(const igmc_batch* b, int which);
int igmc_batch_set_side_features(igmc_batch* b, const float* d_feat, int n_side);
int igmc_batch_bind_side_source(igmc_batch* b, const float* d_side_all, int n_side);
int igmc_batch_set_lean(igmc_batch* b, int lean);
int igmc_batch_assume_size(igmc_batch* b, int B);
int igmc_batch_want_transposed(igmc_batch* b);

enum { IGMC_P_BASIS = 0, IGMC_P_ROOT, IGMC_P_BIAS, IGMC_P_ATT,
       IGMC_P_LIN1_W, IGMC_P_LIN1_B, IGMC_P_LIN2_W, IGMC_P_LIN2_B };
int igmc_model_create(int device, int num_relations, int num_bases, int num_labels ,
                      int n_side_features, int max_nodes, int max_edges, int max_graphs,
                      igmc_model** out);
void igmc_model_destroy(igmc_model* m);
int64_t igmc_param_count(const igmc_model* m);
int64_t igmc_param_offset(const igmc_model* m, int layer, int which, int64_t* count);

int igmc_model_forward(igmc_model* m, const float* d_params, const igmc_batch* b,
                       int training, int use_edge_flags, const uint8_t* d_lin_mask,
                       uint64_t seed, uint64_t step, float multiply_by,
                       float* d_out, void* stream);
int igmc_model_backward(igmc_model* m, const float* d_params, const igmc_batch* b,
                        const float* d_gout, float multiply_by, float* d_grad, void* stream);

int igmc_model_loss_grad(igmc_model* m, const float* d_params, const igmc_batch* b,
                         int use_edge_flags, const uint8_t* d_lin_mask, uint64_t seed, uint64_t step,
                         float multiply_by, float ARR, float grad_scale, float arr_scale,
                         float* d_out, float* d_grad, float* d_loss, void* stream);

int igmc_adam_step(float* d_params, const float* d_grad, float* d_exp_avg, float* d_exp_avg_sq,
                   int64_t n, int64_t step, float lr, float beta1, float beta2, float eps,
                   float weight_decay, void* stream);

enum { IGMC_CTRL_STEP = 0, IGMC_CTRL_FIRST = 1, IGMC_CTRL_EPOCH = 2, IGMC_CTRL_ADAM_T = 3, IGMC_CTRL_BATCH = 4,
       IGMC_CTRL_DONE = 5, IGMC_CTRL_FIRST_ODD = 6, IGMC_CTRL_K = 7,
       IGMC_CTRL_LR = 8, IGMC_CTRL_BETA1 = 9, IGMC_CTRL_BETA2 = 10, IGMC_CTRL_EPS = 11, IGMC_CTRL_WD = 12,
       IGMC_CTRL_STEP_SIZE = 13, IGMC_CTRL_INV_SQRT_BC2 = 14, IGMC_CTRL_GROUP = 15, IGMC_CTRL_GK = 16,
       IGMC_CTRL_GQ = 17, IGMC_CTRL_SYNC_ERR = 18, IGMC_CTRL_GATE_TIMEOUTS = 19, IGMC_CTRL_WORDS = 24 };
int igmc_ctrl_tick(int64_t* d_ctrl, void* stream);
int igmc_ctrl_regroup(int64_t* d_ctrl, int M, int64_t first_cur, int64_t first_next, void* stream);
int igmc_ctrl_gate(int64_t* d_ctrl, int q, int gk_min, double delay_us, int delay_always, double timeout_us, void* stream);
int igmc_batch_set_ctrl(igmc_batch* b, const int64_t* d_ctrl);
int igmc_model_set_ctrl(igmc_model* m, const int64_t* d_ctrl);
int igmc_step_finish(igmc_model* m, const igmc_batch* b, float* d_params, const float* d_grad,
                     float* d_exp_avg, float* d_exp_avg_sq, float ARR, float* d_loss, double* d_total,
                     int64_t* d_ctrl, int64_t step, float lr, float beta1, float beta2, float eps,
                     float weight_decay, void* stream);
int igmc_train_step(igmc_model* m, float* d_params, const igmc_batch* b, int use_edge_flags,
                    const uint8_t* d_lin_mask, uint64_t seed, uint64_t step, float multiply_by, float ARR,
                    float* d_out, float* d_grad, float* d_exp_avg, float* d_exp_avg_sq, float* d_loss,
                    double* d_total, int64_t* d_ctrl, int64_t adam_t, float lr, float beta1, float beta2,
                    float eps, float weight_decay, void* stream);

int igmc_model_weights_unchanged(igmc_model* m, int on);
int igmc_adam_step_ctrl(float* d_params, const float* d_grad, float* d_exp_avg, float* d_exp_avg_sq,
                        int64_t n, const int64_t* d_ctrl, void* stream);

typedef struct igmc_comm igmc_comm;
typedef int (*igmc_allreduce_fn)(void* user, float* d_buf, int64_t n, void* stream);
int igmc_comm_unique_id(uint8_t* h_id128);
int igmc_comm_create(const uint8_t* h_id128, int rank, int world, int device, igmc_comm** out);
int igmc_comm_create_host(igmc_allreduce_fn fn, void* user, int rank, int world, igmc_comm** out);
int igmc_comm_peer_alloc(int rank, int world, int device, int64_t max_floats, igmc_comm** out, uint8_t* h_handle64);
int igmc_comm_peer_connect(igmc_comm* c, const uint8_t* h_handles);
int igmc_comm_check(igmc_comm* c, void* stream);
int igmc_comm_kind(const igmc_comm* c);
void igmc_comm_destroy(igmc_comm* c);
int igmc_comm_info(const igmc_comm* c, int* rank, int* world);
int igmc_allreduce_grads(igmc_comm* c, float* d_flat_grad, int64_t n, float scale, void* stream);
int igmc_train_step_dp(igmc_model* m, igmc_comm* comm, float* d_params, const igmc_batch* b, int use_edge_flags,
                       const uint8_t* d_lin_mask, uint64_t seed, uint64_t step, float multiply_by, float ARR, float* d_out,
                       float* d_grad, float* d_exp_avg, float* d_exp_avg_sq, float* d_loss, double* d_total,
                       int64_t* d_ctrl, int64_t adam_t, float lr, float beta1, float beta2, float eps, float weight_decay,
                       void* stream);

int igmc_sse_accumulate(const float* d_out, const igmc_batch* b, double* d_acc, void* stream);
int igmc_sse_accumulate_tick(const float* d_out, const igmc_batch* b, double* d_acc, int64_t* d_ctrl, void* stream);

int igmc_scores_store(const float* d_out, const igmc_batch* b, double* d_acc, float* d_scores, float* d_labels, int64_t n,
                      int64_t first_or_minus1, int64_t* d_ctrl , int32_t* d_err, void* stream);
int64_t igmc_select_scratch_bytes(int64_t n, int num, int grid);
int igmc_select_extremes(const float* d_keys, int64_t n, int num, int32_t* d_idx_low, int32_t* d_idx_high, float* d_key_low,
                         float* d_key_high, int32_t* d_count, void* d_scratch, int64_t scratch_bytes, int grid, void* stream);

int igmc_candidates_count(const igmc_graph* g, const int32_t* d_users, int nq, const uint8_t* d_item_ok ,
                          int exclude_seen, int64_t* d_counts, int32_t* d_err, void* stream);
int igmc_candidates_fill(const igmc_graph* g, const int32_t* d_users, int nq, const uint8_t* d_item_ok ,
                         int exclude_seen, const int64_t* d_offsets, int32_t* d_link_u, int32_t* d_link_v, int64_t capacity,
                         int32_t* d_err, void* stream);
int64_t igmc_select_segments_scratch_bytes(int ns, int num, int geometry);
int igmc_select_segments(const float* d_keys, const int64_t* d_seg_off, int ns, int num, int32_t* d_idx_out, float* d_key_out,
                         int32_t* d_count, void* d_scratch, int64_t scratch_bytes, int geometry, void* stream);

int igmc_rank_segments(const float* d_keys, const int32_t* d_ids, int64_t n, const int64_t* d_seg_off, int ns,
                       const int64_t* d_q_off, const int32_t* d_q_id, int64_t nq, int32_t* d_q_pos, int32_t* d_q_rank,
                       int32_t* d_err, int geometry, void* stream);
int igmc_rank_metrics(const int32_t* d_q_rank, const int64_t* d_q_off, const uint8_t* d_q_rel , int64_t nq,
                      int ns, const int32_t* d_ks, int nk, int32_t* d_cnt, double* d_dcg, int32_t* d_err, int grid,
                      void* stream);

int igmc_profile_enable(int on);
int igmc_profile_fetch(char names[][48], float* ms, int* calls, int cap);
int igmc_profile_gs_clock(const igmc_model* m, int64_t* launches, double* mean_us, int reset);

int igmc_model_check(igmc_model* m, void* stream);
int igmc_model_dense_path(const igmc_model* m, const igmc_batch* b, int B);
int igmc_model_step_form(const igmc_model* m, const igmc_batch* b, int B);
#define IGMC_GEOM_N 11
int igmc_model_step_geometry(const igmc_model* m, const igmc_batch* b, int B, int32_t* out, int n);
int igmc_model_reset_exchange(igmc_model* m, void* stream);

int igmc_model_dense_layers(const igmc_model* m, const igmc_batch* b, int B);

typedef struct igmc_sortpool igmc_sortpool;
int igmc_sortpool_create(igmc_model* m, int k, int max_nodes_per_graph, igmc_sortpool** out);
void igmc_sortpool_destroy(igmc_sortpool* sp);
int igmc_sortpool_layout(const igmc_sortpool* sp, int64_t* out27);
int igmc_sortpool_forward(igmc_sortpool* sp, const float* d_params, const igmc_batch* b, int training,
                          int use_edge_flags, const uint8_t* d_lin_mask, uint64_t seed, uint64_t step,
                          float* d_out, void* stream);
int igmc_sortpool_loss_grad(igmc_sortpool* sp, const float* d_params, const igmc_batch* b, int use_edge_flags,
                            const uint8_t* d_lin_mask, uint64_t seed, uint64_t step, float ARR, float grad_scale,
                            float arr_scale, float* d_out, float* d_grad, float* d_loss, void* stream);

int igmc_sortpool_step_finish(igmc_sortpool* sp, const igmc_batch* b, float* d_params, const float* d_grad,
                              float* d_exp_avg, float* d_exp_avg_sq, float ARR, float* d_loss, double* d_total,
                              int64_t* d_ctrl, int64_t step, float lr, float beta1, float beta2, float eps,
                              float weight_decay, void* stream);

#ifdef __cplusplus
}
#endif
#endif
```

Before: 824,700 subgraphs/s.

## Sum cluster members' weight-grad tables in-kernel, shrinking tail reduction slots

Adds an optional mode (IGMC_GS_TSUM) in which the cluster members of the fused graph-step kernel sum their per-member weight-gradient tables inside the kernel. The summing is interleaved with the backward layers and synchronised through flag barriers, so the tail kernels only reduce one table per graph instead of one per member. The tail reduce kernels are templated on an in-flight unroll count and use a smaller unroll and an extra set when few slots remain. The mode is off by default (hook default 0), so ts_tables equals cs and the old reduction sizes are mostly kept. The templated tail kernels may still select the small-unroll variant depending on the slot count. It risks extra spin-waits and agent-scope atomic loads inside the main kernel.

```diff
diff --git a/igmc_amd/csrc/capi.hip b/igmc_amd/csrc/capi.hip
--- a/igmc_amd/csrc/capi.hip
+++ b/igmc_amd/csrc/capi.hip
@@ -882,7 +882,8 @@
                                   sp.wide && sp.gsplit,
                                   g2 || sp.dlts,
                                   g2 ? sp.lay.kp : 0,
-                                  dense && sp.dlb};
+                                  dense && sp.dlb,
+                                  g2 ? (sp.cs > 1 ? sp.ts_tables * B : sp.grid) : 0};
   for (int i = 0; i < n && i < IGMC_GEOM_N; ++i) out[i] = v[i];
   return 0;
 }
diff --git a/igmc_amd/csrc/g2_compose.h b/igmc_amd/csrc/g2_compose.h
--- a/igmc_amd/csrc/g2_compose.h
+++ b/igmc_amd/csrc/g2_compose.h
@@ -177,6 +177,11 @@
   a.self_seq = (!training || a.ts) ? 1 : 0;
   a.cs = cs;
   a.stride = (cs > 1) ? ((B + 7) & ~7) : 1;
+  a.tsum = (training && cs > 1 && sp.ts_tables == 1) ? 1 : 0;
+  a.mute_member = -1;
+#ifdef IGMC_HIPEMU
+  if (const char* e = getenv("IGMC_EMU_TSUM_MUTE")) a.mute_member = atoi(e);
+#endif
   if (training && nstash) {
     a.nstash = nstash;
     a.stash_ctrl = stash_ctrl;
diff --git a/igmc_amd/csrc/g2_prims.h b/igmc_amd/csrc/g2_prims.h
--- a/igmc_amd/csrc/g2_prims.h
+++ b/igmc_amd/csrc/g2_prims.h
@@ -123,7 +123,8 @@
   if (lane == 0) ((unsigned long long*)(px + flags_off))[slot] = (unsigned long long)tag;
 #endif
 }
-__device__ __forceinline__ void g2_flags_wait(const unsigned char* px, int n, uint32_t tag, int lane, int* err, int flags_off = G2_PX_FLAGS) {
+__device__ __forceinline__ void g2_flags_wait(const unsigned char* px, int n, uint32_t tag, int lane, int* err, int flags_off = G2_PX_FLAGS,
+                                              long max_polls = 1L << 20) {
   const unsigned long long* fl = (const unsigned long long*)(px + flags_off);
   for (long it = 0;; ++it) {
 #ifndef IGMC_HIPEMU
@@ -132,7 +133,7 @@
     const unsigned long long w = (lane < n) ? fl[lane] : (unsigned long long)tag;
 #endif
     if (__ballot(w != (unsigned long long)tag) == 0ull) break;
-    if (it > (1L << 20)) {
+    if (it > max_polls) {
       *err = 1;
       break;
     }
@@ -143,6 +144,21 @@
 #endif
   }
 }
+__device__ __forceinline__ float4 g2_ld_f4_l2(const float4* p) {
+#ifndef IGMC_HIPEMU
+  const unsigned long long lo = __hip_atomic_load((const unsigned long long*)p, __ATOMIC_RELAXED, __HIP_MEMORY_SCOPE_AGENT);
+  const unsigned long long hi = __hip_atomic_load((const unsigned long long*)p + 1, __ATOMIC_RELAXED, __HIP_MEMORY_SCOPE_AGENT);
+  return make_float4(__uint_as_float((uint32_t)lo), __uint_as_float((uint32_t)(lo >> 32)), __uint_as_float((uint32_t)hi),
+                     __uint_as_float((uint32_t)(hi >> 32)));
+#else
+  return *p;
+#endif
+}
+#ifdef IGMC_HIPEMU
+#define G2_TB_POLLS (1L << 12)
+#else
+#define G2_TB_POLLS (1L << 20)
+#endif
 __device__ __forceinline__ void g2_planes_load_exact(uint32_t* pl, const unsigned char* px, int bytes, int wave, int lane, int nwaves) {
   const int pieces = (bytes + 1023) >> 10;
   for (int c = wave; c < pieces; c += nwaves)
diff --git a/igmc_amd/csrc/g2_subgraph.h b/igmc_amd/csrc/g2_subgraph.h
--- a/igmc_amd/csrc/g2_subgraph.h
+++ b/igmc_amd/csrc/g2_subgraph.h
@@ -33,6 +33,8 @@
   float* out;
   unsigned long long* ts;
   int timing, cs, stride, self_seq;
+  int tsum;
+  int mute_member;
   G2Layout lay2;
   int nstash;
   const int64_t* stash_ctrl;
@@ -171,6 +173,36 @@
     auto px_of = [&](int x, int sd) { return a.g2_px + (size_t)x * exs + ((size_t)g * 2 + sd) * G2_PX_BYTES; };
     unsigned long long* fx = a.g2_fx + (size_t)g * 256;
     const int nbun_opp = (n_opp + 15) >> 4;
+    const bool tsum = ONCE && TRAIN && a.tsum != 0;
+    auto tbl_raise = [&](int x) {
+#ifdef IGMC_HIPEMU
+      if (cm == a.mute_member) return;
+#endif
+      g2_flag_raise(px_of(x, 0), cm * (G2_THREADS / 64) + wave, tag0 + G2_TBTAG, lane, G2_PX_FLAGS + 16 * 8);
+    };
+    auto tbl_wait = [&](int x) {
+      g2_flags_wait(px_of(x, 0), cs * (G2_THREADS / 64), tag0 + G2_TBTAG, lane, a.gs_err, G2_PX_FLAGS + 16 * 8, G2_TB_POLLS);
+    };
+    auto tbl_sum = [&](float* t0, int nf4) {
+      const int sh = (nf4 + cs - 1) / cs;
+      for (int i = tid; i < sh && cm * sh + i < nf4; i += G2_THREADS) {
+        float4* p = (float4*)t0 + cm * sh + i;
+        const size_t ms = (size_t)a.stride * ts / 4;
+        float4 v[4];
+#pragma unroll
+        for (int k = 0; k < 4; ++k)
+          if (k < cs) v[k] = g2_ld_f4_l2(p + k * ms);
+        float4 s4 = v[0];
+#pragma unroll
+        for (int k = 1; k < 4; ++k)
+          if (k < cs) {
+            s4.x += v[k].x; s4.y += v[k].y; s4.z += v[k].z; s4.w += v[k].w;
+          }
+        *p = s4;
+      }
+    };
+    const int tbl_nf4 = (R + 1) * 256 + 8;
+    auto tbl_of = [&](int l) { return a.ts_part + ((size_t)l * IGMC_TS_BLOCKS + g) * ts; };
 
     if (tid < 256) slab[tid] = (unsigned char)(((tid & 127) < ((tid >> 7) ? cv : cu)) ? labv_raw : 255);
     G2_STAMP(50);
@@ -610,8 +642,14 @@
           }
         }
         G2_STAMP(22 + 5 * (3 - l));
+        if (tsum && l < 3) {
+          tbl_wait(3 - (l + 1));
+          tbl_sum(tbl_of(l + 1), tbl_nf4);
+          G2_STAMP(58 + (2 - l));
+        }
         if (l > 1) fetch(6 - l);
         __syncthreads();
+        if (tsum && l > 1) tbl_raise(3 - l);
         G2_STAMP(23 + 5 * (3 - l));
       }
 
@@ -640,6 +678,44 @@
       const int c = m2 * 16 + kq * 4 + rr;
       if (c < RL + L + 1) part0[c * 32 + wn * 16 + li] = acc0[rr];
     }
+  }
+  if (ONCE && TRAIN && a.tsum && g_first < B) {
+    const int g = g_first;
+    unsigned char* px2 = a.g2_px + (size_t)2 * a.g2_px_stride + ((size_t)g * 2) * G2_PX_BYTES;
+    const int nw = G2_THREADS / 64;
+#ifdef IGMC_HIPEMU
+    if (cm != a.mute_member)
+#endif
+    g2_flag_raise(px2, cm * nw + wave, tag0 + G2_TBTAG, lane, G2_PX_FLAGS + 16 * 8);
+    g2_flags_wait(px2, cs * nw, tag0 + G2_TBTAG, lane, a.gs_err, G2_PX_FLAGS + 16 * 8, G2_TB_POLLS);
+    const size_t ms = (size_t)a.stride * ts / 4;
+    const int nf4[2] = {(R + 1) * 256 + 8, (RL + L + 1) * 8};
+    float4* p[2];
+    float4 v[2][4];
+    bool on[2];
+    for (int i0 = 0; i0 < (nf4[0] + cs - 1) / cs; i0 += G2_THREADS) {
+#pragma unroll
+    for (int t = 0; t < 2; ++t) {
+      const int sh = (nf4[t] + cs - 1) / cs, e = cm * sh + i0 + tid;
+      on[t] = i0 + tid < sh && e < nf4[t];
+      p[t] = (float4*)(a.ts_part + ((size_t)(1 - t) * IGMC_TS_BLOCKS + g) * ts) + (on[t] ? e : 0);
+#pragma unroll
+      for (int k = 0; k < 4; ++k)
+        if (k < cs && on[t]) v[t][k] = g2_ld_f4_l2(p[t] + k * ms);
+    }
+#pragma unroll
+    for (int t = 0; t < 2; ++t)
+      if (on[t]) {
+        float4 s4 = v[t][0];
+#pragma unroll
+        for (int k = 1; k < 4; ++k)
+          if (k < cs) {
+            s4.x += v[t][k].x; s4.y += v[t][k].y; s4.z += v[t][k].z; s4.w += v[t][k].w;
+          }
+        *p[t] = s4;
+      }
+    }
+    G2_STAMP(60);
   }
   arrive();
   G2_STAMP(35);
diff --git a/igmc_amd/csrc/graphstep2.hip b/igmc_amd/csrc/graphstep2.hip
--- a/igmc_amd/csrc/graphstep2.hip
+++ b/igmc_amd/csrc/graphstep2.hip
@@ -13,6 +13,7 @@
 #define G2_TP (G2_NR * 32 + 4)
 #define G2_XP 36
 #define G2_FXTAG 7
+#define G2_TBTAG 5
 
 __device__ unsigned long long g_g2_clk[128];
 __device__ unsigned long long g_g2_wg[1024][3];
diff --git a/igmc_amd/csrc/launch.h b/igmc_amd/csrc/launch.h
--- a/igmc_amd/csrc/launch.h
+++ b/igmc_amd/csrc/launch.h
@@ -131,7 +131,10 @@
   int needs_csr;
   int dense_layers;
   int step_form;
+  int ts_tables;
 };
+static inline int gs_ts_stride(const StepPlan& sp, int B) { return (sp.cs > 1) ? ((B + 7) & ~7) : IGMC_TS_BLOCKS; }
+static inline int gs_ts_nparts(const StepPlan& sp, int B) { return (sp.cs > 1) ? sp.ts_tables * ((B + 7) & ~7) : sp.grid; }
 void igmc_step_plan(const ModelDev& m, const BatchDev& b, int B, int kind, StepPlan* p);
 int igmc_dl_always();
 void igmc_launch_g2_compose(const ModelDev& m, const float* P, void* stream);
diff --git a/igmc_amd/csrc/model.hip b/igmc_amd/csrc/model.hip
--- a/igmc_amd/csrc/model.hip
+++ b/igmc_amd/csrc/model.hip
@@ -1234,7 +1234,7 @@
 struct TsSlots {
   int ng, nq, stride;
 };
-__device__ __forceinline__ TsSlots ts_slots(int nparts, int stride, int B) {
+__host__ __device__ __forceinline__ TsSlots ts_slots(int nparts, int stride, int B) {
   TsSlots s;
   s.ng = (nparts < stride) ? nparts : ((B < stride) ? B : stride);
   s.nq = ((nparts + stride - 1) / stride) * s.ng;
@@ -1247,6 +1247,10 @@
   return c * s.stride + g;
 }
 
+#define IGMC_TS_NU_MIN 4
+#define IGMC_TS_NU_MAX 14
+static inline int ts_inflight(int nparts, int stride, int B) { return ts_slots(nparts, stride, B).nq <= 16 * IGMC_TS_NU_MIN ? IGMC_TS_NU_MIN : IGMC_TS_NU_MAX; }
+template <int NU>
 __device__ __forceinline__ void reduce_ts_body(const ModelDev& m, int nparts, int stride, int B, int blk,
                                                const float* __restrict__ Pold = nullptr) {
   __shared__ float4 sred4[16][16];
@@ -1273,12 +1277,12 @@
     const float* p = m.ts_part + (size_t)l * IGMC_TS_BLOCKS * ts + i0;
     const TsSlots sl = ts_slots(nparts, stride, B);
     const int nq = sl.nq;
-    for (int q0 = pg; q0 < nq; q0 += 16 * 14) {
-      float4 v[14];
-#pragma unroll
-      for (int u = 0; u < 14; ++u) v[u] = *(const float4*)(p + (size_t)ts_slot(sl, q0 + 16 * u) * ts);
-#pragma unroll
-      for (int u = 0; u < 14; ++u)
+    for (int q0 = pg; q0 < nq; q0 += 16 * NU) {
+      float4 v[NU];
+#pragma unroll
+      for (int u = 0; u < NU; ++u) v[u] = *(const float4*)(p + (size_t)ts_slot(sl, q0 + 16 * u) * ts);
+#pragma unroll
+      for (int u = 0; u < NU; ++u)
         if (q0 + 16 * u < nq) {
           s4.x += v[u].x; s4.y += v[u].y; s4.z += v[u].z; s4.w += v[u].w;
         }
@@ -1310,6 +1314,7 @@
 }
 
 
+template <int NU>
 __global__ __launch_bounds__(IGMC_BLOCK) void k_tail_ts(BatchDev b, ModelDev m, const float* __restrict__ P,
                                                           float grad_scale, float mult, float drop_scale,
                                                           float* __restrict__ grad, int nlin, int nparts, int stride,
@@ -1321,7 +1326,7 @@
   if ((int)blockIdx.x < nlin)
     head_bwd_w_body(b, m, P, nullptr, 1, grad_scale, mult, drop_scale, grad, blockIdx.x & 7, blockIdx.x >> 3, B);
   else if ((int)blockIdx.x < nlin + nred)
-    reduce_ts_body(m, nparts, stride, B, blockIdx.x - nlin, nstash ? P : nullptr);
+    reduce_ts_body<NU>(m, nparts, stride, B, blockIdx.x - nlin, nstash ? P : nullptr);
   else
     fin_stash_body(m, P, blockIdx.x - nlin - nred, ctrl);
 }
@@ -1904,7 +1909,7 @@
   }
 }
 
-#define IGMC_TF_SETS 3
+#define IGMC_TF_SETS 4
 #define IGMC_TF_ROWS 384
 #define IGMC_TF_O_ROWS (IGMC_TF_SETS * 1024)
 #define IGMC_TF_O_ST (IGMC_TF_O_ROWS + IGMC_TF_ROWS)
@@ -1927,6 +1932,7 @@
 #define TF_STAMP(on, k) do { } while (0)
 #endif
 
+template <int NU>
 __global__ __launch_bounds__(IGMC_BLOCK) void k_tail_fin(BatchDev b, ModelDev m, const float* P, float grad_scale, float mult,
                                                            float drop_scale, float* grad, float arr_coef, AdamTail at, int nlin,
                                                            int nparts, int stride, int B, int bump_seq, int mute_layer) {
@@ -1992,37 +1998,39 @@
     }
     if (tid == 0) *s_flag = 0;
     TF_STAMP(blk == 0, 1);
+    constexpr int SETS = (NU == IGMC_TS_NU_MIN) ? 4 : 3;
+    static_assert(SETS <= IGMC_TF_SETS && SETS <= IGMC_BLOCK / 64, "a wave per set of the round, LDS for every set");
     const float* pl = m.ts_part + (size_t)l * IGMC_TS_BLOCKS * ts;
     const TsSlots sl = ts_slots(nparts, stride, B);
     const int nq = sl.nq;
     bool first_round = true;
     auto sum_columns = [&](int k0, int k1) {
       const int nsets = (k1 - k0 + 15) >> 4;
-      int i0[IGMC_TF_SETS];
-      float4 s4[IGMC_TF_SETS];
-#pragma unroll
-      for (int s = 0; s < IGMC_TF_SETS; ++s) {
+      int i0[SETS];
+      float4 s4[SETS];
+#pragma unroll
+      for (int s = 0; s < SETS; ++s) {
         const int k = k0 + 16 * s + o4, kc = k < k1 ? k : k1 - 1, j = kc >> 3;
         const int row = j < R ? j * fin + c : j == R ? R * fin + c : R * fin + fin;
         i0[s] = row * 32 + 4 * (kc & 7);
         s4[s] = make_float4(0.f, 0.f, 0.f, 0.f);
       }
-      for (int q0 = pg; q0 < nq; q0 += 16 * 14) {
-        float4 v[IGMC_TF_SETS][14];
-        size_t so[14];
-#pragma unroll
-        for (int u = 0; u < 14; ++u) so[u] = (size_t)ts_slot(sl, q0 + 16 * u) * ts;
-#pragma unroll
-        for (int s = 0; s < IGMC_TF_SETS; ++s)
+      for (int q0 = pg; q0 < nq; q0 += 16 * NU) {
+        float4 v[SETS][NU];
+        size_t so[NU];
+#pragma unroll
+        for (int u = 0; u < NU; ++u) so[u] = (size_t)ts_slot(sl, q0 + 16 * u) * ts;
+#pragma unroll
+        for (int s = 0; s < SETS; ++s)
           if (s < nsets) {
 #pragma unroll
-            for (int u = 0; u < 14; ++u) v[s][u] = *(const float4*)(pl + so[u] + i0[s]);
+            for (int u = 0; u < NU; ++u) v[s][u] = *(const float4*)(pl + so[u] + i0[s]);
           }
 #pragma unroll
-        for (int s = 0; s < IGMC_TF_SETS; ++s)
+        for (int s = 0; s < SETS; ++s)
           if (s < nsets) {
 #pragma unroll
-            for (int u = 0; u < 14; ++u)
+            for (int u = 0; u < NU; ++u)
               if (q0 + 16 * u < nq) {
                 s4[s].x += v[s][u].x; s4[s].y += v[s][u].y; s4[s].z += v[s][u].z; s4[s].w += v[s][u].w;
               }
@@ -2030,7 +2038,7 @@
       }
       if (!first_round) __syncthreads();
 #pragma unroll
-      for (int s = 0; s < IGMC_TF_SETS; ++s)
+      for (int s = 0; s < SETS; ++s)
         if (s < nsets) sred4[(s * 16 + pg) * 16 + o4] = s4[s];
       if (first_round) {
 #pragma unroll
@@ -2050,8 +2058,9 @@
         if (k < k1) rows[k * 4 + (lane & 3)] = tot;
       }
     };
-    const int ncol_a = 8 * (R + 1);
-    for (int k0 = 0; k0 < ncol_a; k0 += 16 * IGMC_TF_SETS) sum_columns(k0, k0 + 16 * IGMC_TF_SETS < ncol_a ? k0 + 16 * IGMC_TF_SETS : ncol_a);
+    const bool bias_first = NU == IGMC_TS_NU_MIN && c == 0;
+    const int ncol_a = 8 * (R + 1) + (bias_first ? 8 : 0);
+    for (int k0 = 0; k0 < ncol_a; k0 += 16 * SETS) sum_columns(k0, k0 + 16 * SETS < ncol_a ? k0 + 16 * SETS : ncol_a);
     __syncthreads();
     TF_STAMP(blk == 0, 2);
     unsigned long long* words = m.fold_w + (size_t)l * 32 * IGMC_FOLD_NA;
@@ -2077,7 +2086,7 @@
       }
     }
     TF_STAMP(blk == 0, 3);
-    if (c == 0) sum_columns(ncol_a, ncol_a + 8);
+    if (c == 0 && !bias_first) sum_columns(ncol_a, ncol_a + 8);
     TF_STAMP(blk == 0, 4);
     {
       const int nw = fin * na;
@@ -2366,8 +2375,12 @@
 
 static void launch_tail_ts(const ModelDev& m, const BatchDev& b, const float* P, int B, float grad_scale, float mult, float* grad,
                            int nlin, int nparts, int stride, int nstash, const int64_t* ctrl, int bump_seq, void* stream) {
-  IGMC_PLAUNCH("k_tail_ts", k_tail_ts, nlin + (4 * m.ts_stride + 63) / 64 + nstash, IGMC_BLOCK, 0, stream, b, m, P, grad_scale,
-               mult, 2.f, grad, nlin, nparts, stride, B, nstash, ctrl, bump_seq);
+  if (ts_inflight(nparts, stride, B) == IGMC_TS_NU_MIN)
+    IGMC_PLAUNCH("k_tail_ts", k_tail_ts<IGMC_TS_NU_MIN>, nlin + (4 * m.ts_stride + 63) / 64 + nstash, IGMC_BLOCK, 0, stream, b, m, P,
+                 grad_scale, mult, 2.f, grad, nlin, nparts, stride, B, nstash, ctrl, bump_seq);
+  else
+    IGMC_PLAUNCH("k_tail_ts", k_tail_ts<IGMC_TS_NU_MAX>, nlin + (4 * m.ts_stride + 63) / 64 + nstash, IGMC_BLOCK, 0, stream, b, m, P,
+                 grad_scale, mult, 2.f, grad, nlin, nparts, stride, B, nstash, ctrl, bump_seq);
 }
 
 static void launch_tail_fin(const ModelDev& m, const BatchDev& b, const float* P, int B, float grad_scale, float mult, float* grad,
@@ -2379,8 +2392,12 @@
   hipemu::rt().co_stride = -1;
   hipemu::rt().co_block = 0;
 #endif
-  IGMC_PLAUNCH("k_tail_fin", k_tail_fin, 96 + m.L + nlin + 1, IGMC_BLOCK, (size_t)IGMC_TF_WORDS * sizeof(float), stream, b, m, P,
-               grad_scale, mult, 2.f, grad, arr_coef, at, nlin, nparts, stride, B, bump_seq, mute);
+  if (ts_inflight(nparts, stride, B) == IGMC_TS_NU_MIN)
+    IGMC_PLAUNCH("k_tail_fin", k_tail_fin<IGMC_TS_NU_MIN>, 96 + m.L + nlin + 1, IGMC_BLOCK, (size_t)IGMC_TF_WORDS * sizeof(float), stream,
+                 b, m, P, grad_scale, mult, 2.f, grad, arr_coef, at, nlin, nparts, stride, B, bump_seq, mute);
+  else
+    IGMC_PLAUNCH("k_tail_fin", k_tail_fin<IGMC_TS_NU_MAX>, 96 + m.L + nlin + 1, IGMC_BLOCK, (size_t)IGMC_TF_WORDS * sizeof(float), stream,
+                 b, m, P, grad_scale, mult, 2.f, grad, arr_coef, at, nlin, nparts, stride, B, bump_seq, mute);
 }
 
 static int launch_exchange(const ModelDev& m, int tail, const StepExchange* xch, float* grad, void* stream) {
@@ -2506,16 +2523,15 @@
   const int tables = sp.tail == IGMC_TAIL_TS;
   if (sp.family == IGMC_FAM_G2) {
     const int fold = sp.tail_fold && tables && adam && at.enabled && img && !xch;
-    const int stride = (sp.cs > 1) ? ((B + 7) & ~7) : IGMC_TS_BLOCKS;
+    const int stride = gs_ts_stride(sp, B), nparts = gs_ts_nparts(sp, B);
     const int bump_seq = igmc_launch_graph_step2(m, b, sp, Pc, B, 1, use_flags, inj_mask, seed, step, mult, grad_scale, out, stream,
                                                  fold ? 4 : 0, ctrl);
     if (fold) {
-      launch_tail_fin(m, b, Pc, B, grad_scale, mult, grad, ARR * arr_scale, at, 8 * ny, sp.grid, stride, bump_seq, stream);
+      launch_tail_fin(m, b, Pc, B, grad_scale, mult, grad, ARR * arr_scale, at, 8 * ny, nparts, stride, bump_seq, stream);
       if (img_emitted) *img_emitted = 1;
       return 0;
     }
-    launch_tail_ts(m, b, Pc, B, grad_scale, mult, grad, 8 * ny, sp.grid, (sp.cs > 1) ? ((B + 7) & ~7) : IGMC_TS_BLOCKS,
-                   tables ? 4 : 0, ctrl, bump_seq, stream);
+    launch_tail_ts(m, b, Pc, B, grad_scale, mult, grad, 8 * ny, nparts, stride, tables ? 4 : 0, ctrl, bump_seq, stream);
   } else {
     launch_conv_fwd(m, b, sp, Pc, B, 1, use_flags, stream);
     if (sp.dlts) {
diff --git a/igmc_amd/csrc/step_plan.h b/igmc_amd/csrc/step_plan.h
--- a/igmc_amd/csrc/step_plan.h
+++ b/igmc_amd/csrc/step_plan.h
@@ -12,6 +12,7 @@
   int dl_head;
   int fin_mode;
   int tail_fold;
+  int gs_tsum;
 };
 static int step_hook(const char* name, int unset) {
   const char* e = getenv(name);
@@ -29,6 +30,7 @@
   hk.dl_head = step_hook("IGMC_DL_HEAD", 1);
   hk.fin_mode = step_hook("IGMC_FIN_MODE", 1);
   hk.tail_fold = step_hook("IGMC_TAIL_FOLD", 1);
+  hk.gs_tsum = step_hook("IGMC_GS_TSUM", 0);
   return hk;
 }
 int igmc_dl_always() { return step_hook("IGMC_DL_ALWAYS", 0) == 1; }
@@ -139,6 +141,7 @@
     p->exchange_inside = fused && fts;
     p->tail_fold = fused && fts && hk.tail_fold != 0 && m.fold_w && m.L <= 32 && 4 * m.R <= IGMC_FOLD_NA;
     p->step_form = 1;
+    p->ts_tables = (p->cs > 1 && fused && hk.gs_tsum == 1) ? 1 : p->cs;
     return;
   }
   const int dlf1 = narrow && dl_fwd_eligible(hk, m, b, B), dlb1 = dlf1 && dl_bwd_eligible(hk, m, b, B);
diff --git a/igmc_amd/engine.py b/igmc_amd/engine.py
--- a/igmc_amd/engine.py
+++ b/igmc_amd/engine.py
@@ -257,6 +257,11 @@
         g = dict(zip(self.GEOMETRY_KEYS, [int(x) for x in out]))
         g['family'] = self.FAMILIES[g['family']]
         return g
+
+    def step_tail_tables(self, batch, B):
+        out = (C.c_int32 * 12)()
+        self.lib.call('igmc_model_step_geometry', self.handle, batch.handle, int(B), C.cast(out, C.c_void_p), 12)
+        return int(out[11])
 
     def adam_step(self, params, grad, exp_avg, exp_avg_sq, step, lr, beta1=0.9, beta2=0.999, eps=1e-8,
                   weight_decay=0.0, stream=None):
diff --git a/include/igmc_hip.h b/include/igmc_hip.h
--- a/include/igmc_hip.h
+++ b/include/igmc_hip.h
@@ -173,7 +173,7 @@
 int igmc_model_check(igmc_model* m, void* stream);
 int igmc_model_dense_path(const igmc_model* m, const igmc_batch* b, int B);
 int igmc_model_step_form(const igmc_model* m, const igmc_batch* b, int B);
-#define IGMC_GEOM_N 11
+#define IGMC_GEOM_N 12
 int igmc_model_step_geometry(const igmc_model* m, const igmc_batch* b, int B, int32_t* out, int n);
 int igmc_model_reset_exchange(igmc_model* m, void* stream);
 
```

Result: slower. 816,300 subgraphs/s (-1.0%).
